# Aatrick/LightDiffusion

Hardware: AMD Instinct MI355X
Metric: UNet denoise steps/sec at 512x512 (higher is better)
Workload: dtype f16 (fp32 accumulate); 1 GPU; SD1.5 512x512 UNet CFG step, euler_ancestral / normal-30, batch 8/GPU (UNet batch 16), latent 64x64; global_batch=8, parallelism=dp1 (replicas, RCCL cond broadcast), hip_graph=True, setup_before_warmup=hipGraph capture + one untimed schedule pass per workload

## Files before the change

include/ld_mi355x.h:

```cpp
#ifndef LD_MI355X_H
#define LD_MI355X_H

#include <stddef.h>
#include <stdint.h>

#ifdef __cplusplus
extern "C" {
#endif

#define LD_OK 0
#define LD_ERR_ARG 1
#define LD_ERR_SHAPE 2
#define LD_ERR_HIP 3
#define LD_ERR_STATE 4

#define LD_F16 0
#define LD_F32 1

const char* ld_version(void);
const char* ld_status_string(int status);

typedef struct {
    int in_channels, out_channels, model_channels;
    int num_levels;
    int channel_mult[8];
    int num_res_blocks[8];
    int transformer_depth[16];
    int transformer_depth_output[24];
    int transformer_depth_middle;
    int context_dim, num_heads;
} ld_unet_config;

typedef struct ld_unet ld_unet;

int ld_unet_create(const ld_unet_config* cfg, ld_unet** out);
void ld_unet_destroy(ld_unet* u);
int ld_unet_param_count(const ld_unet* u);
int ld_unet_param_info(const ld_unet* u, int index, const char** name, int* ndim, int64_t shape[4]);
int ld_unet_load_param(ld_unet* u, const char* name, const void* dev_src, int dtype, void* stream);
int ld_unet_reserve(ld_unet* u, int max_n, int max_h, int max_w, int max_ctx_tokens);
size_t ld_unet_workspace_bytes(const ld_unet* u);
size_t ld_unet_weight_bytes(const ld_unet* u);
int ld_unet_set_context(ld_unet* u, const void* ctx, int dtype, int n, int tokens, void* stream);
int ld_unet_forward(ld_unet* u, const float* x, const float* sigma, float* out, int n, int h, int w, int eps_only, void* stream);
int ld_unet_forward_pair(ld_unet* u, const float* x, const float* sigma, float* out, int nb, int h, int w, void* stream);
int ld_unet_profile(ld_unet* u, const float* x, const float* sigma, float* out, int n, int h, int w, void* stream, double ms[6],
                    double flops[6], int launches[6]);
int ld_unet_profile_pair(ld_unet* u, const float* x, const float* sigma, float* out, int nb, int h, int w, void* stream, double ms[6],
                         double flops[6], int launches[6]);
int ld_unet_profile_kernels(const ld_unet* u, char* buf, size_t buf_bytes);
int ld_unet_profile_launches(const ld_unet* u, char* buf, size_t buf_bytes);
int ld_unet_last_launches(const ld_unet* u);
double ld_unet_last_flops(const ld_unet* u);

typedef struct {
    int z_channels, ch, num_levels;
    int ch_mult[8];
    int num_res_blocks, out_ch;
    int with_encoder;
} ld_vae_config;

typedef struct ld_vae ld_vae;

int ld_vae_create(const ld_vae_config* cfg, ld_vae** out);
void ld_vae_destroy(ld_vae* v);
int ld_vae_param_count(const ld_vae* v);
int ld_vae_param_info(const ld_vae* v, int index, const char** name, int* ndim, int64_t shape[4]);
int ld_vae_load_param(ld_vae* v, const char* name, const void* dev_src, int dtype, void* stream);
int ld_vae_reserve(ld_vae* v, int max_b, int max_h, int max_w);
size_t ld_vae_workspace_bytes(const ld_vae* v);
size_t ld_vae_plan_bytes(ld_vae* v, int b, int h, int w);
int ld_vae_decode(ld_vae* v, const float* z, float* out, int b, int h, int w, void* stream);
int ld_vae_encode(ld_vae* v, const float* pixels_nchw, float* moments, int b, int h, int w, void* stream);
int ld_vae_profile(ld_vae* v, const float* z, float* out, int b, int h, int w, void* stream);
int ld_vae_profile_launches(const ld_vae* v, char* buf, size_t buf_bytes);
int ld_vae_last_launches(const ld_vae* v);
double ld_vae_last_flops(const ld_vae* v);

int ld_op_linear(const void* x, const void* w, const void* bias, const void* residual, void* y, int M, int N, int K,
                 float alpha, int act, void* ws, size_t ws_bytes, void* stream);
int ld_op_conv(const void* x1, int c1, const void* x2, int c2, int n, int h, int w, int hv, int wv, int stride, int ksize,
               const void* wt, const void* bias, const void* rowvec, const void* residual, void* y, int cout,
               void* ws, size_t ws_bytes, void* stream);
size_t ld_op_groupnorm_conv_ws_bytes(int c1, int c2, int n, int h, int w, int cout);
int ld_op_groupnorm_conv(const void* x1, int c1, const void* x2, int c2, int n, int h, int w, const void* gamma, const void* beta, float eps,
                         const void* wt, const void* bias, const void* rowvec, const void* residual, void* y, int cout, void* ws,
                         size_t ws_bytes, void* stream);
int ld_op_repack_conv(const void* src_oihw, int dtype, int cout, int cin, void* dst, void* stream);
size_t ld_op_conv_skip_ws_bytes(int c, int sc1, int sc2, int cout);
int ld_op_conv_skip(const void* x, int c, int n, int h, int w, const void* wt, const void* bias, const void* s1, int sc1, const void* s2, int sc2,
                    const void* wskip, const void* bskip, const void* rowvec, void* y, int cout, void* ws, size_t ws_bytes, void* stream);
int ld_op_upconv2x_fold(const void* wt, int cout, int cin, void* wfold, void* stream);
int ld_op_upconv2x(const void* x, int c, int n, int h, int w, int hv, int wv, const void* wt, const void* wfold, const void* bias, void* y, int cout,
                   void* ws, size_t ws_bytes, void* stream);
size_t ld_op_conv_gn_partials_floats(int n, int hw);
int ld_op_conv_gn_partials(const void* x, int c, int n, int h, int w, int hv, int wv, const void* wt, const void* bias,
                           const void* residual, void* y, int cout, float* part, int* chunks, void* ws, size_t ws_bytes, void* stream);
size_t ld_op_groupnorm_ws_bytes(int n, int hw);
int ld_op_groupnorm(const void* x1, int c1, const void* x2, int c2, int n, int hw, const void* gamma, const void* beta,
                    float eps, int silu, void* y, void* ws, void* stream);
int ld_op_layernorm(const void* x, const void* gamma, const void* beta, void* y, int rows, int c, float eps, void* stream);
int ld_op_attention(const void* q, int ldq, const void* k, int ldk, const void* vt, int ldvt, void* o, int ldo, int b,
                    int heads, int lq, int lk, int d, float scale, int causal, void* stream);
int ld_op_attention_rowv(const void* q, int ldq, const void* k, int ldk, const void* v, int ldv, void* o, int ldo, int b,
                         int heads, int lq, int lk, int d, float scale, int causal, void* stream);
int ld_op_softmax_rows(void* s, int rows, int cols, void* stream);
int ld_op_timestep_embed(const float* sigma, const float* log_sigmas, int n_sigmas, int n, int dim, void* out_f16, float* t_out,
                         void* stream);
int ld_op_cfg_combine(const float* den2, float* out, float cfg, size_t n_half, void* stream);
int ld_op_axpby(float* x, float a, const float* y, float b, const float* z, float c, size_t n, void* stream);
int ld_op_hook_check(const void* a, const void* b, size_t words_ab, const void* x, size_t half_words_x, const void* sigma, int half_sigma,
                     int* flags, int epoch, void* stream);

int ld_op_linear_ln(const void* x, const void* w_prod, const void* b_prod, const void* gamma, const void* beta, const void* w,
                    const void* bias, void* t_out, void* y, int M, int C, int N, float eps, void* ws, size_t ws_bytes, void* stream);
int ld_op_linear_ln_geglu(const void* x, const void* w_prod, const void* b_prod, const void* gamma, const void* beta, const void* w,
                          const void* bias, void* t_out, void* y, int M, int C, int N, float eps, void* ws, size_t ws_bytes, void* stream);
int ld_op_bislerp(const float* x, float* tmp, float* y, int n, int c, int h, int w, int h_new, int w_new, void* stream);
const char* ld_op_last_kernel(void);

#ifdef __cplusplus
}
#endif
#endif
```

lightdiffusion_amd/_lib.py:

```python
from __future__ import annotations

import ctypes as C
import os

_HERE = os.path.dirname(os.path.abspath(__file__))
LIB_PATH = os.environ.get("LD_MI355X_LIB") or os.path.join(_HERE, "libld_mi355x.so")

OK, ERR_ARG, ERR_SHAPE, ERR_HIP, ERR_STATE = 0, 1, 2, 3, 4
F16, F32 = 0, 1


class UNetConfig(C.Structure):
    _fields_ = [("in_channels", C.c_int), ("out_channels", C.c_int), ("model_channels", C.c_int), ("num_levels", C.c_int),
                ("channel_mult", C.c_int * 8), ("num_res_blocks", C.c_int * 8), ("transformer_depth", C.c_int * 16),
                ("transformer_depth_output", C.c_int * 24), ("transformer_depth_middle", C.c_int),
                ("context_dim", C.c_int), ("num_heads", C.c_int)]


class VAEConfig(C.Structure):
    _fields_ = [("z_channels", C.c_int), ("ch", C.c_int), ("num_levels", C.c_int), ("ch_mult", C.c_int * 8),
                ("num_res_blocks", C.c_int), ("out_ch", C.c_int), ("with_encoder", C.c_int)]


class LDError(RuntimeError):
    def __init__(self, status: int, where: str):
        self.status = status
        msg = lib().ld_status_string(status).decode() if _lib is not None else str(status)
        super().__init__(f"{where}: {msg} (status {status})")


_lib = None
_P, _I, _F, _Z = C.c_void_p, C.c_int, C.c_float, C.c_size_t

SIGNATURES = {
    "ld_version": (C.c_char_p, []),
    "ld_status_string": (C.c_char_p, [_I]),
    "ld_unet_create": (_I, [C.POINTER(UNetConfig), C.POINTER(_P)]),
    "ld_unet_destroy": (None, [_P]),
    "ld_unet_param_count": (_I, [_P]),
    "ld_unet_param_info": (_I, [_P, _I, C.POINTER(C.c_char_p), C.POINTER(_I), C.POINTER(C.c_int64)]),
    "ld_unet_load_param": (_I, [_P, C.c_char_p, _P, _I, _P]),
    "ld_unet_reserve": (_I, [_P, _I, _I, _I, _I]),
    "ld_unet_workspace_bytes": (_Z, [_P]),
    "ld_unet_weight_bytes": (_Z, [_P]),
    "ld_unet_set_context": (_I, [_P, _P, _I, _I, _I, _P]),
    "ld_unet_forward": (_I, [_P, _P, _P, _P, _I, _I, _I, _I, _P]),
    "ld_unet_forward_pair": (_I, [_P, _P, _P, _P, _I, _I, _I, _P]),
    "ld_unet_profile_pair": (_I, [_P, _P, _P, _P, _I, _I, _I, _P, C.POINTER(C.c_double), C.POINTER(C.c_double), C.POINTER(_I)]),
    "ld_unet_profile": (_I, [_P, _P, _P, _P, _I, _I, _I, _P, C.POINTER(C.c_double), C.POINTER(C.c_double), C.POINTER(_I)]),
    "ld_unet_profile_kernels": (_I, [_P, C.c_char_p, _Z]),
    "ld_unet_profile_launches": (_I, [_P, C.c_char_p, _Z]),
    "ld_unet_last_launches": (_I, [_P]),
    "ld_unet_last_flops": (C.c_double, [_P]),
    "ld_vae_create": (_I, [C.POINTER(VAEConfig), C.POINTER(_P)]),
    "ld_vae_destroy": (None, [_P]),
    "ld_vae_param_count": (_I, [_P]),
    "ld_vae_param_info": (_I, [_P, _I, C.POINTER(C.c_char_p), C.POINTER(_I), C.POINTER(C.c_int64)]),
    "ld_vae_load_param": (_I, [_P, C.c_char_p, _P, _I, _P]),
    "ld_vae_reserve": (_I, [_P, _I, _I, _I]),
    "ld_vae_workspace_bytes": (_Z, [_P]),
    "ld_vae_plan_bytes": (_Z, [_P, _I, _I, _I]),
    "ld_vae_decode": (_I, [_P, _P, _P, _I, _I, _I, _P]),
    "ld_vae_encode": (_I, [_P, _P, _P, _I, _I, _I, _P]),
    "ld_vae_profile": (_I, [_P, _P, _P, _I, _I, _I, _P]),
    "ld_vae_profile_launches": (_I, [_P, C.c_char_p, _Z]),
    "ld_vae_last_launches": (_I, [_P]),
    "ld_vae_last_flops": (C.c_double, [_P]),
    "ld_op_linear": (_I, [_P, _P, _P, _P, _P, _I, _I, _I, _F, _I, _P, _Z, _P]),
    "ld_op_conv": (_I, [_P, _I, _P, _I, _I, _I, _I, _I, _I, _I, _I, _P, _P, _P, _P, _P, _I, _P, _Z, _P]),
    "ld_op_groupnorm_conv_ws_bytes": (_Z, [_I, _I, _I, _I, _I, _I]),
    "ld_op_groupnorm_conv": (_I, [_P, _I, _P, _I, _I, _I, _I, _P, _P, _F, _P, _P, _P, _P, _P, _I, _P, _Z, _P]),
    "ld_op_repack_conv": (_I, [_P, _I, _I, _I, _P, _P]),
    "ld_op_upconv2x_fold": (_I, [_P, _I, _I, _P, _P]),
    "ld_op_upconv2x": (_I, [_P, _I, _I, _I, _I, _I, _I, _P, _P, _P, _P, _I, _P, _Z, _P]),
    "ld_op_conv_skip_ws_bytes": (_Z, [_I, _I, _I, _I]),
    "ld_op_conv_skip": (_I, [_P, _I, _I, _I, _I, _P, _P, _P, _I, _P, _I, _P, _P, _P, _P, _I, _P, _Z, _P]),
    "ld_op_groupnorm_ws_bytes": (_Z, [_I, _I]),
    "ld_op_groupnorm": (_I, [_P, _I, _P, _I, _I, _I, _P, _P, _F, _I, _P, _P, _P]),
    "ld_op_layernorm": (_I, [_P, _P, _P, _P, _I, _I, _F, _P]),
    "ld_op_attention": (_I, [_P, _I, _P, _I, _P, _I, _P, _I, _I, _I, _I, _I, _I, _F, _I, _P]),
    "ld_op_conv_gn_partials_floats": (_Z, [_I, _I]),
    "ld_op_conv_gn_partials": (_I, [_P, _I, _I, _I, _I, _I, _I, _P, _P, _P, _P, _I, _P, _P, _P, _Z, _P]),
    "ld_op_attention_rowv": (_I, [_P, _I, _P, _I, _P, _I, _P, _I, _I, _I, _I, _I, _I, _F, _I, _P]),
    "ld_op_softmax_rows": (_I, [_P, _I, _I, _P]),
    "ld_op_timestep_embed": (_I, [_P, _P, _I, _I, _I, _P, _P, _P]),
    "ld_op_cfg_combine": (_I, [_P, _P, _F, _Z, _P]),
    "ld_op_axpby": (_I, [_P, _F, _P, _F, _P, _F, _Z, _P]),
    "ld_op_hook_check": (_I, [_P, _P, _Z, _P, _Z, _P, _I, _P, _I, _P]),
    "ld_op_linear_ln": (_I, [_P, _P, _P, _P, _P, _P, _P, _P, _P, _I, _I, _I, _F, _P, _Z, _P]),
    "ld_op_linear_ln_geglu": (_I, [_P, _P, _P, _P, _P, _P, _P, _P, _P, _I, _I, _I, _F, _P, _Z, _P]),
    "ld_op_bislerp": (_I, [_P, _P, _P, _I, _I, _I, _I, _I, _I, _P]),
    "ld_op_last_kernel": (C.c_char_p, []),
}


def lib() -> C.CDLL:
    global _lib
    if _lib is None:
        if not os.path.exists(LIB_PATH):
            raise ImportError(f"{LIB_PATH} not found — build it with `python -c 'import __graft_entry__ as g; g.build()'` "
                              f"or `make -C lightdiffusion_amd/csrc`.  There is no CPU / PyTorch fallback for the hot path.")
        try:
            import torch
        except ImportError:
            pass
        l = C.CDLL(LIB_PATH)
        missing = []
        for name, (res, args) in SIGNATURES.items():
            if not hasattr(l, name):
                if not os.environ.get("LD_MI355X_LIB"):
                    raise AttributeError(f"{LIB_PATH} does not export {name}: header and library out of sync — rebuild it")
                missing.append(name)
                setattr(l, name, _missing_symbol(name))
                continue
            fn = getattr(l, name)
            fn.restype = res
            fn.argtypes = args
        l._ld_missing = tuple(missing)
        _lib = l
    return _lib


def _missing_symbol(name: str):
    def fail(*_a, **_k):
        raise RuntimeError(f"{LIB_PATH} (LD_MI355X_LIB) does not export {name}: it was built from a commit without this entry point")
    return fail


def check(status: int, where: str) -> None:
    if status != OK:
        raise LDError(status, where)
```

lightdiffusion_amd/csrc/capi.hip:

```cpp
#include <string>

#include "kernels.h"
#include "../../include/ld_mi355x.h"

namespace {
inline size_t align256(size_t v) { return (v + 255) / 256 * 256; }

thread_local std::string t_op_kernels;
inline void op_begin() { t_op_kernels.clear(); }
inline int noted(int st, const char* name) {
    if (name != nullptr && *name != '\0') {
        if (!t_op_kernels.empty()) t_op_kernels += ';';
        t_op_kernels += name;
    }
    return st;
}
inline int gemm_op(const GemmParams& p, hipStream_t s) { return noted(gemm_launch(p, s), gemm_last_kernel_name()); }
inline int gemm_op(const GemmParams& p, const GemmPlan& plan, hipStream_t s) { return noted(gemm_run(p, plan, s), gemm_last_kernel_name()); }

constexpr size_t kSyncBytes = LD_SYNC_INTS * sizeof(int);
inline size_t conv8_scratch_head(int cout, int cin) { return kSyncBytes + (conv8_weight_eligible(cout, cin) ? align256(conv8_weight_bytes(cout, cin)) : 0); }
inline void conv8_scratch(GemmParams& p, void* ws, size_t partial_bytes) {
    const int cin = p.C1 + p.C2;
    p.sync = (int*)ws;
    p.W8 = conv8_weight_eligible(p.N, cin) ? (const half_t*)((char*)ws + kSyncBytes) : nullptr;
    p.partial = (float*)((char*)ws + conv8_scratch_head(p.N, cin));
    p.partial_bytes = partial_bytes;
}
inline int conv8_scratch_op(const GemmParams& p, const GemmPlan& plan, const void* wt, hipStream_t stream) {
    if (plan.route == GR_CONV8) {
        if (hipMemsetAsync(p.sync, 0, kSyncBytes, stream) != hipSuccess) return LD_ERR_HIP;
        const int st = conv8_repack_launch((const half_t*)wt, p.N, p.C1 + p.C2, const_cast<half_t*>(p.W8), stream);
        if (st != LD_OK) return st;
    }
    return gemm_op(p, plan, stream);
}
inline int attn_op(const AttnParams& a, hipStream_t s) { return noted(attention_launch(a, s), attention_last_kernel_name()); }
}

extern "C" {

const char* ld_version(void) { return "ld_mi355x 0.1 (gfx950)"; }

const char* ld_op_last_kernel(void) { return t_op_kernels.c_str(); }

const char* ld_status_string(int s) {
    switch (s) {
        case LD_OK: return "ok";
        case LD_ERR_ARG: return "invalid argument";
        case LD_ERR_SHAPE: return "unsupported shape or alignment";
        case LD_ERR_HIP: return "HIP runtime error";
        case LD_ERR_STATE: return "invalid call order (weights / reserve / context missing)";
        default: return "unknown status";
    }
}

int ld_op_linear(const void* x, const void* w, const void* bias, const void* residual, void* y, int M, int N, int K, float alpha,
                 int act, void* ws, size_t ws_bytes, void* stream_) {
    op_begin();
    hipStream_t stream = (hipStream_t)stream_;
    GemmParams p;
    p.A = (const half_t*)x; p.lda = K;
    p.W = (const half_t*)w; p.ldw = K;
    p.M = M; p.N = N; p.K = K;
    p.alpha = alpha;
    p.bias_n = (const half_t*)bias;
    p.R = (const half_t*)residual;
    p.act = act;
    p.C = (half_t*)y;
    p.ldc = p.ldr = (act == 2 ? N / 2 : N);
    char* wsp = (char*)ws;
    if (act == 2) {
        if (bias == nullptr || (N & 15)) return LD_ERR_ARG;
        const int bn = gemm_pick_bn(N);
        if (N % bn) return LD_ERR_SHAPE;
        const size_t wb = align256((size_t)N * K * sizeof(half_t)), bb = align256((size_t)N * sizeof(half_t));
        if (ws == nullptr || ws_bytes < wb + bb) return LD_ERR_ARG;
        half_t* w2 = (half_t*)wsp;
        half_t* b2 = (half_t*)(wsp + wb);
        int st = repack_rows_launch(w, 0, N, K, w2, bn, stream);
        if (st != LD_OK) return st;
        st = repack_rows_launch(bias, 0, N, 1, b2, bn, stream);
        if (st != LD_OK) return st;
        p.W = w2;
        p.bias_n = b2;
        p.bn = bn;
        wsp += wb + bb;
        ws_bytes -= wb + bb;
    }
    p.partial = (float*)wsp;
    p.partial_bytes = ws ? ws_bytes : 0;
    if (ws == nullptr) p.partial = nullptr;
    return gemm_op(p, stream);
}

static int op_conv(const void* x1, int c1, const void* x2, int c2, int n, int h, int w, int hv, int wv, int stride, int ksize,
                   const void* wt, const void* bias, const void* rowvec, const void* residual, void* y, int cout, void* ws,
                   size_t ws_bytes, void* stream, float* gn_part, int* gn_chunks, const void* wup = nullptr) {
    if (stride < 1 || (ksize != 1 && ksize != 3)) return LD_ERR_ARG;
    GemmParams p;
    if (gn_part != nullptr) {
        const int HW = (ksize == 3 ? (hv - 1) / stride + 1 : hv) * (ksize == 3 ? (wv - 1) / stride + 1 : wv);
        p.gn_part = gn_part;
        p.gn_P = gn_num_chunks(n, HW);
        p.gn_HW = HW;
        p.gn_ppb = (HW + p.gn_P - 1) / p.gn_P;
        p.gn_part_done = gn_chunks;
    }
    p.conv = 1;
    p.ksize = ksize;
    p.A = (const half_t*)x1; p.A2 = (const half_t*)x2; p.C1 = c1; p.C2 = c2;
    p.Hs = h; p.Ws = w; p.Hv = hv; p.Wv = wv; p.stride = stride;
    p.Ho = ksize == 3 ? (hv - 1) / stride + 1 : hv;
    p.Wo = ksize == 3 ? (wv - 1) / stride + 1 : wv;
    p.K = ksize * ksize * (c1 + c2);
    p.W = (const half_t*)wt; p.ldw = p.K;
    p.Wup = (const half_t*)wup;
    p.M = n * p.Ho * p.Wo; p.N = cout;
    p.bias_n = (const half_t*)bias;
    p.rowvec = (const half_t*)rowvec; p.rows_per_vec = p.Ho * p.Wo; p.ldrv = cout;
    p.R = (const half_t*)residual; p.ldr = cout;
    p.C = (half_t*)y; p.ldc = cout;
    p.partial = (float*)ws;
    p.partial_bytes = ws ? ws_bytes : 0;
    const size_t head = conv8_scratch_head(cout, c1 + c2);
    if (ws != nullptr && ksize == 3 && conv8_weight_eligible(cout, c1 + c2) && ws_bytes > head + ((size_t)8 << 20)) {
        GemmParams c8 = p;
        conv8_scratch(c8, ws, ws_bytes - head);
        if (const GemmPlan plan = gemm_plan(c8); plan.route == GR_CONV8) return conv8_scratch_op(c8, plan, wt, (hipStream_t)stream);
    }
    return gemm_op(p, (hipStream_t)stream);
}

int ld_op_conv(const void* x1, int c1, const void* x2, int c2, int n, int h, int w, int hv, int wv, int stride, int ksize,
               const void* wt, const void* bias, const void* rowvec, const void* residual, void* y, int cout, void* ws,
               size_t ws_bytes, void* stream) {
    op_begin();
    return op_conv(x1, c1, x2, c2, n, h, w, hv, wv, stride, ksize, wt, bias, rowvec, residual, y, cout, ws, ws_bytes, stream, nullptr, nullptr);
}

int ld_op_upconv2x_fold(const void* wt, int cout, int cin, void* wfold, void* stream) {
    op_begin();
    return upconv_fold_launch((const half_t*)wt, cout, cin, (half_t*)wfold, (hipStream_t)stream);
}

int ld_op_upconv2x(const void* x, int c, int n, int h, int w, int hv, int wv, const void* wt, const void* wfold, const void* bias, void* y, int cout,
                   void* ws, size_t ws_bytes, void* stream) {
    op_begin();
    if (wfold == nullptr) return LD_ERR_ARG;
    return op_conv(x, c, nullptr, 0, n, h, w, hv, wv, 1, 3, wt, bias, nullptr, nullptr, y, cout, ws, ws_bytes, stream, nullptr, nullptr, wfold);
}

size_t ld_op_conv_gn_partials_floats(int n, int hw) {
    op_begin();
    return groupnorm_workspace_bytes(n, hw) / sizeof(float);
}

int ld_op_conv_gn_partials(const void* x, int c, int n, int h, int w, int hv, int wv, const void* wt, const void* bias, const void* residual,
                           void* y, int cout, float* part, int* chunks, void* ws, size_t ws_bytes, void* stream) {
    op_begin();
    if (part == nullptr || chunks == nullptr) return LD_ERR_ARG;
    *chunks = 0;
    return op_conv(x, c, nullptr, 0, n, h, w, hv, wv, 1, 3, wt, bias, nullptr, residual, y, cout, ws, ws_bytes, stream, part, chunks);
}

size_t ld_op_groupnorm_conv_ws_bytes(int c1, int c2, int n, int h, int w, int cout) {
    op_begin();
    const size_t C = (size_t)c1 + c2, HW = (size_t)h * w;
    return align256(groupnorm_workspace_bytes(n, (int)HW)) + 2 * align256((size_t)n * C * sizeof(float)) + align256((size_t)n * HW * C * sizeof(half_t)) +
           conv8_scratch_head(cout, c1 + c2) + ((size_t)96 << 20);
}

int ld_op_groupnorm_conv(const void* x1, int c1, const void* x2, int c2, int n, int h, int w, const void* gamma, const void* beta, float eps,
                         const void* wt, const void* bias, const void* rowvec, const void* residual, void* y, int cout, void* ws, size_t ws_bytes,
                         void* stream_) {
    op_begin();
    if (x1 == nullptr || gamma == nullptr || beta == nullptr || wt == nullptr || y == nullptr || ws == nullptr) return LD_ERR_ARG;
    if (ws_bytes < ld_op_groupnorm_conv_ws_bytes(c1, c2, n, h, w, cout)) return LD_ERR_ARG;
    hipStream_t stream = (hipStream_t)stream_;
    const int C = c1 + c2, HW = h * w;
    char* q = (char*)ws;
    float* part = (float*)q; q += align256(groupnorm_workspace_bytes(n, HW));
    float* scale = (float*)q; q += align256((size_t)n * C * sizeof(float));
    float* shift = (float*)q; q += align256((size_t)n * C * sizeof(float));
    half_t* g = (half_t*)q; q += align256((size_t)n * HW * C * sizeof(half_t));
    GemmParams p;
    p.conv = 1; p.ksize = 3;
    p.A = (const half_t*)x1; p.A2 = (const half_t*)x2; p.C1 = c1; p.C2 = c2;
    p.Hs = p.Hv = p.Ho = h; p.Ws = p.Wv = p.Wo = w; p.stride = 1;
    p.K = 9 * C; p.W = (const half_t*)wt; p.ldw = p.K;
    p.M = n * HW; p.N = cout;
    p.bias_n = (const half_t*)bias;
    p.rowvec = (const half_t*)rowvec; p.rows_per_vec = HW; p.ldrv = cout;
    p.R = (const half_t*)residual; p.ldr = cout;
    p.C = (half_t*)y; p.ldc = cout;
    conv8_scratch(p, q, (size_t)96 << 20);
    const GemmPlan fused = gemm_plan(p, true);
    if (fused.can_fuse_groupnorm) {
        int st = groupnorm_scale_shift_launch((const half_t*)x1, c1, (const half_t*)x2, c2, n, HW, (const half_t*)gamma, (const half_t*)beta, eps, part,
                                              scale, shift, stream);
        if (st != LD_OK) return st;
        p.gn_scale = scale; p.gn_shift = shift; p.gn_silu = 1;
        return gemm_op(p, fused, stream);
    }
    int st = groupnorm_launch((const half_t*)x1, c1, (const half_t*)x2, c2, n, HW, (const half_t*)gamma, (const half_t*)beta, eps, 1, g, part, stream);
    if (st != LD_OK) return st;
    p.A = g; p.A2 = nullptr; p.C1 = C; p.C2 = 0;
    return conv8_scratch_op(p, gemm_plan(p), (const half_t*)wt, stream);
}

size_t ld_op_conv_skip_ws_bytes(int c, int sc1, int sc2, int cout) {
    op_begin();
    return align256((size_t)cout * (9 * (size_t)c + sc1 + sc2) * sizeof(half_t)) + align256((size_t)cout * sizeof(half_t)) + ((size_t)96 << 20);
}

int ld_op_conv_skip(const void* x, int c, int n, int h, int w, const void* wt, const void* bias, const void* s1, int sc1, const void* s2, int sc2,
                    const void* wskip, const void* bskip, const void* rowvec, void* y, int cout, void* ws, size_t ws_bytes, void* stream_) {
    op_begin();
    if (x == nullptr || wt == nullptr || bias == nullptr || s1 == nullptr || wskip == nullptr || bskip == nullptr || y == nullptr || ws == nullptr) return LD_ERR_ARG;
    if (c <= 0 || sc1 <= 0 || sc2 < 0 || (sc2 > 0 && s2 == nullptr) || cout <= 0 || n <= 0 || h <= 0 || w <= 0) return LD_ERR_ARG;
    if (ws_bytes < ld_op_conv_skip_ws_bytes(c, sc1, sc2, cout)) return LD_ERR_ARG;
    hipStream_t stream = (hipStream_t)stream_;
    const int K9 = 9 * c, SC = sc1 + sc2;
    char* q = (char*)ws;
    half_t* wf = (half_t*)q; q += align256((size_t)cout * (K9 + SC) * sizeof(half_t));
    half_t* bf = (half_t*)q; q += align256((size_t)cout * sizeof(half_t));
    int st = skip_fold_launch((const half_t*)wt, (const half_t*)wskip, (const half_t*)bias, (const half_t*)bskip, cout, K9, SC, wf, bf, stream);
    if (st != LD_OK) return st;
    GemmParams p;
    p.conv = 1; p.ksize = 3;
    p.A = (const half_t*)x; p.C1 = c;
    p.Hs = p.Hv = p.Ho = h; p.Ws = p.Wv = p.Wo = w; p.stride = 1;
    p.S1 = (const half_t*)s1; p.SC1 = sc1; p.S2 = (const half_t*)s2; p.SC2 = sc2;
    p.K = K9 + SC; p.W = wf; p.ldw = p.K;
    p.M = n * h * w; p.N = cout;
    p.bias_n = bf;
    p.rowvec = (const half_t*)rowvec; p.rows_per_vec = h * w; p.ldrv = cout;
    p.C = (half_t*)y; p.ldc = cout;
    p.partial = (float*)q; p.partial_bytes = (size_t)96 << 20;
    return gemm_op(p, stream);
}

int ld_op_repack_conv(const void* src, int dtype, int cout, int cin, void* dst, void* stream) {
    op_begin();
    return repack_conv3x3_launch(src, dtype == LD_F32, cout, cin, (half_t*)dst, (hipStream_t)stream);
}

size_t ld_op_groupnorm_ws_bytes(int n, int hw) {
    op_begin();
    return groupnorm_workspace_bytes(n, hw);
}

int ld_op_groupnorm(const void* x1, int c1, const void* x2, int c2, int n, int hw, const void* gamma, const void* beta, float eps,
                    int silu, void* y, void* ws, void* stream) {
    op_begin();
    return groupnorm_launch((const half_t*)x1, c1, (const half_t*)x2, c2, n, hw, (const half_t*)gamma, (const half_t*)beta, eps,
                            silu, (half_t*)y, (float*)ws, (hipStream_t)stream);
}

int ld_op_layernorm(const void* x, const void* gamma, const void* beta, void* y, int rows, int c, float eps, void* stream) {
    op_begin();
    return layernorm_launch((const half_t*)x, (const half_t*)gamma, (const half_t*)beta, (half_t*)y, rows, c, eps, (hipStream_t)stream);
}

int ld_op_attention(const void* q, int ldq, const void* k, int ldk, const void* vt, int ldvt, void* o, int ldo, int b, int heads,
                    int lq, int lk, int d, float scale, int causal, void* stream) {
    op_begin();
    AttnParams a;
    a.Q = (const half_t*)q; a.ldq = ldq; a.sQ = (long long)lq * ldq;
    a.K = (const half_t*)k; a.ldk = ldk; a.sK = (long long)lk * ldk;
    a.Vt = (const half_t*)vt; a.ldvt = ldvt; a.sV = (long long)heads * d * ldvt;
    a.O = (half_t*)o; a.ldo = ldo; a.sO = (long long)lq * ldo;
    a.B = b; a.H = heads; a.Lq = lq; a.Lk = lk; a.d = d; a.scale = scale; a.causal = causal;
    return attn_op(a, (hipStream_t)stream);
}

int ld_op_attention_rowv(const void* q, int ldq, const void* k, int ldk, const void* v, int ldv, void* o, int ldo, int b, int heads,
                         int lq, int lk, int d, float scale, int causal, void* stream) {
    op_begin();
    const char *qb = (const char*)q, *kb = (const char*)k, *vb = (const char*)v;
    const long long rowb = (long long)ldq * 2;
    const bool fused = ldq == ldk && ldk == ldv && rowb > 0 && (kb - qb >= 0 ? kb - qb : qb - kb) < rowb && (vb - qb >= 0 ? vb - qb : qb - vb) < rowb;
    if (fused && lq != lk) return LD_ERR_SHAPE;
    AttnParams a;
    a.Q = (const half_t*)q; a.ldq = ldq; a.sQ = (long long)lq * ldq;
    a.K = (const half_t*)k; a.ldk = ldk; a.sK = (long long)lk * ldk;
    a.V = (const half_t*)v; a.ldv = ldv; a.sV = (long long)lk * ldv;
    a.O = (half_t*)o; a.ldo = ldo; a.sO = (long long)lq * ldo;
    a.B = b; a.H = heads; a.Lq = lq; a.Lk = lk; a.d = d; a.scale = scale; a.causal = causal;
    return attn_op(a, (hipStream_t)stream);
}

int ld_op_softmax_rows(void* s, int rows, int cols, void* stream) {
    op_begin();
    return softmax_rows_launch((half_t*)s, rows, cols, cols, (hipStream_t)stream);
}

int ld_op_timestep_embed(const float* sigma, const float* log_sigmas, int n_sigmas, int n, int dim, void* out, float* t_out, void* stream) {
    op_begin();
    return timestep_embed_launch(sigma, log_sigmas, n_sigmas, n, dim, (half_t*)out, t_out, (hipStream_t)stream);
}

int ld_op_cfg_combine(const float* den2, float* out, float cfg, size_t n_half, void* stream) {
    op_begin();
    return cfg_combine_launch(den2, out, cfg, n_half, (hipStream_t)stream);
}

int ld_op_hook_check(const void* a, const void* b, size_t words_ab, const void* x, size_t half_words_x, const void* sigma, int half_sigma,
                     int* flags, int epoch, void* stream) {
    op_begin();
    return hook_check_launch(a, b, words_ab, x, half_words_x, sigma, half_sigma, flags, epoch, (hipStream_t)stream);
}

int ld_op_axpby(float* x, float a, const float* y, float b, const float* z, float c, size_t n, void* stream) {
    op_begin();
    return axpby_launch(x, a, y, b, z, c, n, (hipStream_t)stream);
}

// ... 92 lines not shown
```

lightdiffusion_amd/csrc/gemm.h:

```cpp
#pragma once
#include "common.h"

struct GemmParams {
    const half_t* A = nullptr;
    const half_t* A2 = nullptr;
    int lda = 0;
    int conv = 0;
    int ksize = 3;
    int pad = -1;
    int Hs = 0, Ws = 0;
    int Hv = 0, Wv = 0;
    int Ho = 0, Wo = 0, stride = 1;
    int C1 = 0, C2 = 0;
    const half_t* S1 = nullptr;
    const half_t* S2 = nullptr;
    int SC1 = 0, SC2 = 0;
    const half_t* W = nullptr;
    int ldw = 0;
    int M = 0, N = 0, K = 0;
    int n_valid = 0;
    int batch = 1;
    long long sA = 0, sW = 0, sC = 0, sR = 0;
    float alpha = 1.0f;
    const half_t* bias_n = nullptr;
    const half_t* bias_m = nullptr;
    const half_t* rowvec = nullptr;
    int rows_per_vec = 1, ldrv = 0;
    const half_t* R = nullptr;
    int ldr = 0;
    int act = 0;
    half_t* C = nullptr;
    int ldc = 0;
    int bm = 0, bn = 0;
    int splitk = 0;
    int m_fastest = -1;
    int xcd_gm = 0;
    float* partial = nullptr;
    size_t partial_bytes = 0;
    float* stat_out = nullptr;
    int* stat_parts_out = nullptr;
    const float* ln_stat = nullptr;
    int ln_parts = 0;
    int ln_rows = 0;
    int ln_zrows = 0;
    float ln_inv_c = 0.f, ln_eps = 0.f;
    const float* ln_wsum = nullptr;
    int ln_swapped = 0;
    const float* gn_scale = nullptr;
    const float* gn_shift = nullptr;
    int gn_silu = 0;
    float* gn_part = nullptr;
    int gn_P = 0, gn_ppb = 0, gn_HW = 0;
    int* gn_part_done = nullptr;
    const half_t* W8 = nullptr;
    int* sync = nullptr;
    int c8_S = 0;
    const half_t* Wup = nullptr;
    int dbg = 0;
};

enum GemmRoute { GR_NONE = 0, GR_CONV8, GR_CONV6, GR_GEMM7, GR_GEMM5, GR_GEMM3, GR_GEMM4, GR_UPCONV };
enum GemmReduce { GRD_NONE = 0, GRD_PLAIN, GRD_GROUPNORM, GRD_UPCONV };
struct GemmPlan {
    int status = LD_OK;
    int route = GR_NONE;
    bool conv = false, geglu = false;
    bool gn = false, up = false;
    bool ln = false;
    bool deep = false, two_wg = false;
    int bm = 0, bn = 0, wc = 0;
    int splitk = 1, c8_S = 0;
    int m_fastest = 0, xcd_gm = 0;
    unsigned grid_x = 0, grid_z = 1;
    int reduce = GRD_NONE;
    int stat_parts = 0;
    int gn_chunks = 0;
    bool halo_tile = false;
    bool can_fuse_groupnorm = false;
    bool takes_skip_segment = false;
    const char* kernel = "";
};
GemmPlan gemm_plan(const GemmParams& p, bool gn_offer = false);
int gemm_run(const GemmParams& p, const GemmPlan& plan, hipStream_t stream);
inline int gemm_launch(const GemmParams& p, hipStream_t stream) { return gemm_run(p, gemm_plan(p), stream); }
const char* gemm_last_kernel_name();

bool conv8_plan(const GemmParams& p, int* S_out);
int conv8_launch(const GemmParams& p, int S, hipStream_t stream);
bool conv8_weight_eligible(int N, int Cin);
size_t conv8_weight_bytes(int N, int Cin);
int conv8_repack_launch(const half_t* w_okki, int N, int Cin, half_t* dst, hipStream_t stream);
int upconv_reduce_launch(const GemmParams& p, hipStream_t stream);
#define LD_SYNC_INTS 1024

static inline int gemm_pick_bn(int N) { return (N % 160 == 0) ? 160 : 128; }
```

lightdiffusion_amd/csrc/gemm.hip:

```cpp
#include <cstdlib>
#include <mutex>
#include <set>
#include <string>
#include <type_traits>
#include <vector>

#include "gemm.h"

namespace {

constexpr int BK = 64;
constexpr int NT = 256;

__device__ __forceinline__ void epilogue_store8(const GemmParams& p, int z, int m, int n_out, int n_bias, float (&v)[8]) {
    const bool hb = p.bias_n != nullptr && p.act != 2, hv = p.rowvec != nullptr, hr = p.R != nullptr;
    const uint4 rb = hb ? ld16(p.bias_n + n_bias) : zero16();
    const uint4 rv = hv ? ld16(p.rowvec + (long long)(m / p.rows_per_vec) * p.ldrv + n_out) : zero16();
    const uint4 rr = hr ? ld16(p.R + (long long)z * p.sR + (long long)m * p.ldr + n_out) : zero16();
    const float bm = p.bias_m != nullptr ? (float)p.bias_m[m] : 0.f;
    float b[8], e[8], r[8];
    unpack8(rb, b);
    unpack8(rv, e);
    unpack8(rr, r);
#pragma unroll
    for (int j = 0; j < 8; ++j) v[j] = v[j] + b[j] + bm + e[j];
    if (p.act == 1) {
#pragma unroll
        for (int j = 0; j < 8; ++j) v[j] = silu_f(v[j]);
    } else if (p.act == 3) {
#pragma unroll
        for (int j = 0; j < 8; ++j) v[j] = quick_gelu_f(v[j]);
    }
#pragma unroll
    for (int j = 0; j < 8; ++j) v[j] += r[j];
    st16(p.C + (long long)z * p.sC + (long long)m * p.ldc + n_out, pack8(v));
}

template <int BM, int BN>
struct EpiPre {
    static constexpr int CPR = BN / 8, EIT = (BM * CPR + NT - 1) / NT, GRP = EIT > 5 ? (EIT + 1) / 2 : EIT;
    uint4 r[GRP];
    bool fast;
    bool bias_done;
};
template <int BM, int BN>
__device__ __forceinline__ EpiPre<BM, BN> epi_prefetch_residual(const GemmParams& p, int z, int m0, int n0, int tid, bool bias_done) {
    EpiPre<BM, BN> e;
    e.bias_done = bias_done;
    constexpr int CPR = EpiPre<BM, BN>::CPR, GRP = EpiPre<BM, BN>::GRP;
    e.fast = (BM * CPR) % NT == 0 && m0 + BM <= p.M && n0 + BN <= p.N && p.act == 0 && p.bias_m == nullptr && bias_done;
#pragma unroll
    for (int k = 0; k < GRP; ++k) e.r[k] = zero16();
    if (e.fast && p.R != nullptr) {
        const half_t* Rb = p.R + (long long)z * p.sR + (long long)m0 * p.ldr + n0;
#pragma unroll
        for (int k = 0; k < GRP; ++k) {
            const int q = tid + k * NT;
            const int row = q / CPR, cc = q - row * CPR;
            e.r[k] = ld16(Rb + (long long)row * p.ldr + cc * 8);
        }
    }
    return e;
}

template <int BM, int BN>
__device__ __forceinline__ void epilogue_tile(const GemmParams& p, const half_t* Cs, int z, int m0, int n0, int tid, float* lds_scratch, const half_t* bias_s,
                                              const EpiPre<BM, BN>& pre) {
    constexpr int CLD = BN + 8;
    if (p.act == 2) {
        constexpr int CPR = BN / 16;
        constexpr int EIT = (BM * CPR + NT - 1) / NT;
        if ((BM * CPR) % NT == 0 && m0 + BM <= p.M && n0 + BN <= p.N && pre.bias_done) {
            half_t* Cb = p.C + (long long)z * p.sC + (long long)m0 * p.ldc + n0 / 2;
            const bool hr = p.R != nullptr;
            const half_t* Rb = hr ? p.R + (long long)z * p.sR + (long long)m0 * p.ldr + n0 / 2 : nullptr;
            uint4 rres[EIT], ca[EIT], cg[EIT];
#pragma unroll
            for (int it = 0; it < EIT; ++it) {
                const int q = tid + it * NT;
                const int row = q / CPR, cc = q - row * CPR;
                rres[it] = hr ? ld16(Rb + (long long)row * p.ldr + cc * 8) : zero16();
                ca[it] = ld16(Cs + row * CLD + cc * 8);
                cg[it] = ld16(Cs + row * CLD + BN / 2 + cc * 8);
            }
#pragma unroll
            for (int it = 0; it < EIT; ++it) {
                const int q = tid + it * NT;
                const int row = q / CPR, cc = q - row * CPR;
                float g[8];
                unpack8(cg[it], g);
                const unsigned aw[4] = {ca[it].x, ca[it].y, ca[it].z, ca[it].w};
                const f32x2 gp[4] = {{g[0], g[1]}, {g[2], g[3]}, {g[4], g[5]}, {g[6], g[7]}};
                unsigned ow[4];
                geglu8_staged(aw, gp, ow);
                uint4 packed = make_uint4(ow[0], ow[1], ow[2], ow[3]);
                if (hr) packed = add8h(packed, rres[it]);
                st16(Cb + (long long)row * p.ldc + cc * 8, packed);
            }
            return;
        }
        uint4 rba[EIT], rbg[EIT], rres[EIT];
#pragma unroll
        for (int it = 0; it < EIT; ++it) {
            const int q = tid + it * NT;
            const int row = q / CPR, cc = q - row * CPR;
            const int m = m0 + row, nv = n0 + cc * 8, ng = nv + BN / 2;
            const bool ok = q < BM * CPR && m < p.M && ng < p.N;
            rba[it] = (ok && !pre.bias_done) ? ld16(p.bias_n + nv) : zero16();
            rbg[it] = (ok && !pre.bias_done) ? ld16(p.bias_n + ng) : zero16();
            rres[it] = (ok && p.R != nullptr) ? ld16(p.R + (long long)z * p.sR + (long long)m * p.ldr + n0 / 2 + cc * 8) : zero16();
        }
#pragma unroll
        for (int it = 0; it < EIT; ++it) {
            const int q = tid + it * NT;
            const int row = q / CPR, cc = q - row * CPR;
            const int m = m0 + row, ng = n0 + cc * 8 + BN / 2;
            if (q < BM * CPR && m < p.M && ng < p.N) {
                float a[8], g[8], ba[8], bg[8], r[8];
                unpack8(ld16(Cs + row * CLD + cc * 8), a);
                unpack8(ld16(Cs + row * CLD + BN / 2 + cc * 8), g);
                unpack8(rba[it], ba);
                unpack8(rbg[it], bg);
                unpack8(rres[it], r);
#pragma unroll
                for (int j = 0; j < 8; ++j) a[j] = (a[j] + ba[j]) * gelu_f(g[j] + bg[j]) + r[j];
                st16(p.C + (long long)z * p.sC + (long long)m * p.ldc + n0 / 2 + cc * 8, pack8(a));
            }
        }
    } else {
        constexpr int CPR = BN / 8;
        constexpr int EIT = (BM * CPR + NT - 1) / NT;
        constexpr int GRP = EIT > 5 ? (EIT + 1) / 2 : EIT;
        const bool hb = p.bias_n != nullptr && !pre.bias_done, hv = p.rowvec != nullptr, hr = p.R != nullptr;
        if (pre.fast) {
            static_assert(GRP == EpiPre<BM, BN>::GRP, "group size");
            half_t* Cb = p.C + (long long)z * p.sC + (long long)m0 * p.ldc + n0;
            const half_t* Rb = hr ? p.R + (long long)z * p.sR + (long long)m0 * p.ldr + n0 : nullptr;
            uint4 rnext[GRP];
#pragma unroll
            for (int k = 0; k < GRP; ++k) rnext[k] = pre.r[k];
#pragma unroll
            for (int g0 = 0; g0 < EIT; g0 += GRP) {
                uint4 rv[GRP], rres[GRP], cv[GRP];
#pragma unroll
                for (int k = 0; k < GRP; ++k) rres[k] = rnext[k];
#pragma unroll
                for (int k = 0; k < GRP; ++k) {
                    if (g0 + GRP + k >= EIT) continue;
                    const int q = tid + (g0 + GRP + k) * NT;
                    const int row = q / CPR, cc = q - row * CPR;
                    rnext[k] = hr ? ld16(Rb + (long long)row * p.ldr + cc * 8) : zero16();
                }
#pragma unroll
                for (int k = 0; k < GRP; ++k) {
                    if (g0 + k >= EIT) continue;
                    const int q = tid + (g0 + k) * NT;
                    const int row = q / CPR, cc = q - row * CPR;
                    rv[k] = hv ? ld16(p.rowvec + (long long)((m0 + row) / p.rows_per_vec) * p.ldrv + n0 + cc * 8) : zero16();
                    cv[k] = ld16(Cs + row * CLD + cc * 8);
                }
#pragma unroll
                for (int k = 0; k < GRP; ++k) {
                    if (g0 + k >= EIT) continue;
                    const int q = tid + (g0 + k) * NT;
                    const int row = q / CPR, cc = q - row * CPR;
                    uint4 packed = cv[k];
                    if (hv) packed = add8h(packed, rv[k]);
                    if (hr) packed = add8h(packed, rres[k]);
                    st16(Cb + (long long)row * p.ldc + cc * 8, packed);
                    if (lds_scratch != nullptr) {
                        const half2v one2 = {(half_t)1.f, (half_t)1.f};
                        const half2v h0 = __builtin_bit_cast(half2v, packed.x), h1 = __builtin_bit_cast(half2v, packed.y);
                        const half2v h2 = __builtin_bit_cast(half2v, packed.z), h3 = __builtin_bit_cast(half2v, packed.w);
                        float s1 = __builtin_amdgcn_fdot2(h1, one2, __builtin_amdgcn_fdot2(h0, one2, 0.f, false), false);
                        float s2 = __builtin_amdgcn_fdot2(h1, h1, __builtin_amdgcn_fdot2(h0, h0, 0.f, false), false);
                        s1 = __builtin_amdgcn_fdot2(h3, one2, __builtin_amdgcn_fdot2(h2, one2, s1, false), false);
                        s2 = __builtin_amdgcn_fdot2(h3, h3, __builtin_amdgcn_fdot2(h2, h2, s2, false), false);
                        *reinterpret_cast<float2*>(lds_scratch + q * 2) = make_float2(s1, s2);
                    }
                }
            }
            if (lds_scratch != nullptr) {
                __syncthreads();
                if (tid < BM) {
                    float s1 = 0.f, s2 = 0.f;
#pragma unroll 4
                    for (int c = 0; c < CPR; ++c) {
                        const float2 t = *reinterpret_cast<const float2*>(lds_scratch + (tid * CPR + c) * 2);
                        s1 += t.x;
// ... 1896 lines not shown
                for (int j = 0; j < 8; ++j) {
                    a[j] += base[nv + j];
                    g[j] += base[ng + j];
                }
            }
            float ba[8], bg[8];
            unpack8(ld16(p.bias_n + nv), ba);
            unpack8(ld16(p.bias_n + ng), bg);
#pragma unroll
            for (int j = 0; j < 8; ++j) v[j] = (a[j] + ba[j]) * gelu_f(g[j] + bg[j]);
            epilogue_store8(p, 0, m, no, 0, v);
        } else {
            const int n = cc * 8;
#pragma unroll
            for (int j = 0; j < 8; ++j) v[j] = 0.f;
            const float* base = p.partial + (long long)m * p.N + n;
            const long long slab = (long long)p.M * p.N;
            int s = 0;
            for (; s + 4 <= p.splitk; s += 4) {
                f32x4 x0[4], x1[4];
#pragma unroll
                for (int u = 0; u < 4; ++u) {
                    x0[u] = *reinterpret_cast<const f32x4*>(base + (s + u) * slab);
                    x1[u] = *reinterpret_cast<const f32x4*>(base + (s + u) * slab + 4);
                }
#pragma unroll
                for (int u = 0; u < 4; ++u)
#pragma unroll
                    for (int j = 0; j < 4; ++j) {
                        v[j] += x0[u][j];
                        v[4 + j] += x1[u][j];
                    }
            }
            for (; s < p.splitk; ++s) {
                const f32x4 x0 = *reinterpret_cast<const f32x4*>(base + s * slab), x1 = *reinterpret_cast<const f32x4*>(base + s * slab + 4);
#pragma unroll
                for (int j = 0; j < 4; ++j) {
                    v[j] += x0[j];
                    v[4 + j] += x1[j];
                }
            }
            epilogue_store8(p, 0, m, n, n, v);
        }
    }
}

__global__ __launch_bounds__(256) void splitk_reduce_gn_kernel(const GemmParams p) {
    __shared__ float csum[2048], csq[2048];
    const int C = p.N, cpg = C / 32;
    const int CS = C / 4, CHS = CS >> 3;
    const int n = blockIdx.y, pc = blockIdx.x, slab = blockIdx.z, tid = threadIdx.x;
    const int rows_par = 256 / CHS;
    const int cc = tid % CHS, prow = tid / CHS;
    const int c0 = slab * CS + cc * 8;
    const int p_begin = pc * p.gn_ppb, p_end = min(p.gn_HW, p_begin + p.gn_ppb);
    const long long slab_stride = (long long)p.M * p.N;
    if (prow < rows_par) {
        float s[8], ss[8];
#pragma unroll
        for (int j = 0; j < 8; ++j) s[j] = ss[j] = 0.f;
        for (int pix = p_begin + prow; pix < p_end; pix += rows_par) {
            const int m = n * p.gn_HW + pix;
            const float* base = p.partial + (long long)m * p.N + c0;
            float v[8];
#pragma unroll
            for (int j = 0; j < 8; ++j) v[j] = 0.f;
            int sp = 0;
            for (; sp + 4 <= p.splitk; sp += 4) {
                f32x4 x0[4], x1[4];
#pragma unroll
                for (int u = 0; u < 4; ++u) {
                    x0[u] = *reinterpret_cast<const f32x4*>(base + (sp + u) * slab_stride);
                    x1[u] = *reinterpret_cast<const f32x4*>(base + (sp + u) * slab_stride + 4);
                }
#pragma unroll
                for (int u = 0; u < 4; ++u)
#pragma unroll
                    for (int j = 0; j < 4; ++j) {
                        v[j] += x0[u][j];
                        v[4 + j] += x1[u][j];
                    }
            }
            for (; sp < p.splitk; ++sp) {
                const f32x4 x0 = *reinterpret_cast<const f32x4*>(base + sp * slab_stride), x1 = *reinterpret_cast<const f32x4*>(base + sp * slab_stride + 4);
#pragma unroll
                for (int j = 0; j < 4; ++j) {
                    v[j] += x0[j];
                    v[4 + j] += x1[j];
                }
            }
            epilogue_store8(p, 0, m, c0, c0, v);
            float f[8];
            unpack8(pack8(v), f);
#pragma unroll
            for (int j = 0; j < 8; ++j) {
                s[j] += f[j];
                ss[j] += f[j] * f[j];
            }
        }
#pragma unroll
        for (int j = 0; j < 8; ++j) {
            csum[prow * CS + cc * 8 + j] = s[j];
            csq[prow * CS + cc * 8 + j] = ss[j];
        }
    }
    __syncthreads();
    {
        const int g = tid >> 5, sub = tid & 31;
        const int cnt = rows_par * cpg;
        float a = 0.f, b = 0.f;
        for (int i = sub; i < cnt; i += 32) {
            const int pr = i / cpg, c = g * cpg + (i - pr * cpg);
            a += csum[pr * CS + c];
            b += csq[pr * CS + c];
        }
#pragma unroll
        for (int o = 1; o < 32; o <<= 1) {
            a += __shfl_xor(a, o, 64);
            b += __shfl_xor(b, o, 64);
        }
        if (sub == 0) {
            float* o = p.gn_part + (((long long)n * p.gn_P + pc) * 32 + slab * 8 + g) * 2;
            o[0] = a;
            o[1] = b;
        }
    }
}

constexpr int V4_MAX_BLOCKS = 256;

thread_local const char* t_last_kernel = "";

const char* plan_kernel_name(const GemmPlan& pl) {
    typedef unsigned long long u64;
    const u64 key = (u64)pl.route | (u64)pl.reduce << 3 | (u64)pl.conv << 5 | (u64)pl.geglu << 6 | (u64)pl.gn << 7 | (u64)pl.up << 8 | (u64)pl.ln << 9 |
                    (u64)pl.deep << 10 | (u64)pl.two_wg << 11 | (u64)pl.bm << 12 | (u64)pl.bn << 24 | (u64)pl.wc << 36;
    thread_local std::vector<std::pair<u64, const char*>> seen;
    for (const auto& e : seen)
        if (e.first == key) return e.second;
    const std::string tile = std::to_string(pl.bm) + "," + std::to_string(pl.bn);
    std::string s;
    switch (pl.route) {
        case GR_UPCONV: s = "upconv_kernel<256,320>"; break;
        case GR_CONV8: s = "conv8_kernel<W" + std::to_string(pl.wc) + (pl.up ? ",up>" : ">"); break;
        case GR_CONV6:
            s = "conv6_kernel<W" + std::to_string(pl.wc) + ",halo" + (pl.gn ? "+groupnorm" : "") +
                (pl.bn == V5_BN ? "" : "," + std::to_string(pl.bn) + (pl.bm == V5_BM ? "" : "x" + std::to_string(pl.bm))) + (pl.up ? ",up" : "") + ">";
            break;
        case GR_GEMM7: s = std::string("gemm7_kernel<256,K320,") + (pl.geglu ? "geglu" : "plain") + (pl.ln ? ",ln>" : ">"); break;
        case GR_GEMM5: s = std::string("gemm5_kernel<256,320,") + (pl.conv ? "conv" : pl.geglu ? "geglu" : pl.ln ? "lnfold" : "plain") + ">"; break;
        case GR_GEMM4: s = "gemm4_kernel<" + tile + (pl.conv ? ",conv" : ",plain") + (pl.two_wg ? ",2wg>" : ">"); break;
        default: s = "gemm3_kernel<" + tile + (pl.conv ? ",conv" : ",plain") + (pl.deep ? ",deep>" : ">"); break;
    }
    if (pl.reduce != GRD_NONE) s += pl.reduce == GRD_GROUPNORM ? "+splitk_reduce_gn_kernel" : pl.reduce == GRD_UPCONV ? "+upconv_reduce_kernel" : "+splitk_reduce_kernel";
    static std::mutex mu; static std::set<std::string> pool;
    std::lock_guard<std::mutex> lock(mu);
    const char* name = pool.insert(s).first->c_str();
    seen.push_back({key, name});
    return name;
}

template <int BM, int BN>
void launch_cfg(const GemmParams& p, const GemmPlan& pl, dim3 grid, hipStream_t s) {
    if (pl.route == GR_GEMM4) {
        if constexpr (BM == 64 && BN == 64) {
            if (pl.two_wg) {
                if (!pl.conv) hipLaunchKernelGGL((gemm4_kernel<64, 64, false, 4, 4>), grid, dim3(2 * NT), 0, s, p);
                else hipLaunchKernelGGL((gemm4_kernel<64, 64, true, 4, 4>), grid, dim3(2 * NT), 0, s, p);
                return;
            }
        }
        hipLaunchKernelGGL((gemm4_kernel<BM, BN, false>), grid, dim3(2 * NT), 0, s, p);
    } else if (pl.conv) {
        if constexpr (BM == 64 && BN == 160) {
            if (pl.deep) {
                hipLaunchKernelGGL((gemm3_kernel<BM, BN, true, 4>), grid, dim3(NT), 0, s, p);
                return;
            }
        }
        hipLaunchKernelGGL((gemm3_kernel<BM, BN, true, 2>), grid, dim3(NT), 0, s, p);
    } else {
        hipLaunchKernelGGL((gemm3_kernel<BM, BN, false, 2>), grid, dim3(NT), 0, s, p);
    }
}

template <int W, bool GN, int BN, int BM, bool UP>
void launch_conv6_w(const GemmParams& p, dim3 grid, hipStream_t s) { hipLaunchKernelGGL((conv6_kernel<W, GN, BN, BM, UP>), grid, dim3(512), 0, s, p); }
template <bool GN, int BN = V5_BN, int BM = V5_BM, bool UP = false>
void launch_conv6(int wc, const GemmParams& p, dim3 grid, hipStream_t s) {
    if constexpr (BN == V5_BN) {
        if (wc == 16) return launch_conv6_w<16, GN, BN, BM, UP>(p, grid, s);
        if (wc == 32) return launch_conv6_w<32, GN, BN, BM, UP>(p, grid, s);
    }
    if constexpr (BN == V5_BN || (BN == 256 && !GN)) {
        if (wc == 64) return launch_conv6_w<64, GN, BN, BM, UP>(p, grid, s);
    }
    launch_conv6_w<128, GN, BN, BM, UP>(p, grid, s);
}

}

#ifdef LD_AB_BUILD
static int g_force_bm = 0, g_force_sk = 0;
static int g_shape_ovr[5] = {0, 0, 0, 0, 0};
extern "C" void ld_debug_gemm_shape_override(int M, int N, int K, int bm, int splitk) {
    g_shape_ovr[0] = M; g_shape_ovr[1] = N; g_shape_ovr[2] = K; g_shape_ovr[3] = bm; g_shape_ovr[4] = splitk;
}
extern "C" void ld_debug_gemm_override(int bm, int splitk) {
    g_force_bm = bm;
    g_force_sk = splitk;
}
#endif

const char* gemm_last_kernel_name() { return t_last_kernel; }

static void plan_reduce(const GemmParams& p, GemmPlan* pl) {
    if (pl->splitk <= 1) return;
    const bool gn = p.gn_part != nullptr && p.act != 2 && p.batch == 1 && p.gn_P > 0 && p.gn_HW > 0 && p.M % p.gn_HW == 0 && p.N % 32 == 0 && p.N <= 8192 && p.N >= 256 &&
                    p.ldc == p.N && (p.N / 4) % 8 == 0 && p.N / 32 <= 256;
    pl->reduce = gn ? GRD_GROUPNORM : GRD_PLAIN;
    if (gn) pl->gn_chunks = p.gn_P;
}

static bool upconv_plan(const GemmParams& p, GemmPlan* out) {
    if (!(p.conv && p.ksize == 3 && p.stride == 1 && p.pad == 1 && p.Hv == 2 * p.Hs && p.Wv == 2 * p.Ws && p.Ho == p.Hv && p.Wo == p.Wv && p.C2 == 0 &&
          p.SC1 == 0 && p.C1 % V5_BK == 0 && p.N % V5_BN == 0 && p.n_valid == p.N && p.bm == 0 && p.bn == 0 && p.splitk == 0 && p.batch == 1 && p.act == 0 &&
          p.alpha == 1.0f && p.rowvec == nullptr && p.R == nullptr && p.bias_m == nullptr && p.stat_out == nullptr && p.ln_stat == nullptr && p.ldc == p.N))
        return false;
    if ((long long)p.M * 4 > 0x7fffffffll) return false;
    if (p.M / (p.Ho * p.Wo) <= 2) return false;
    const int Ms = p.M / 4, K = 4 * p.C1;
    const long long tiles = (long long)((Ms + V5_BM - 1) / V5_BM) * (4 * p.N / V5_BN);
    int sk = 1;
    if (tiles < 192 && p.partial != nullptr) {
        sk = (int)((256 + tiles - 1) / tiles);
        const int cap = K / 640 < 1 ? 1 : K / 640;
        if (sk > cap) sk = cap;
        while (sk > 1 && (size_t)sk * Ms * 4 * p.N * sizeof(float) > p.partial_bytes) --sk;
    }
    out->bm = V5_BM; out->bn = V5_BN; out->splitk = sk; out->up = true;
    out->grid_x = (unsigned)(tiles * sk); out->grid_z = 1;
    out->reduce = sk > 1 ? GRD_UPCONV : GRD_NONE;
    return true;
}

static bool v6_plan(const GemmParams& p, bool gn, GemmPlan* out) {
    const bool same = p.Hv == p.Hs && p.Wv == p.Ws;
    const bool up = p.Hv == 2 * p.Hs && p.Wv == 2 * p.Ws;
    if (!(p.conv && p.ksize == 3 && p.stride == 1 && (p.pad < 0 || p.pad == 1) && (same || up) && p.Ho == p.Hv && p.Wo == p.Wv &&
          p.C1 % 32 == 0 && p.C2 % 32 == 0 && p.bm == 0 && p.bn == 0 && p.splitk == 0 && p.batch == 1 && p.act != 2))
        return false;
    if (up && (p.C2 != 0 || gn)) return false;
    if (p.SC1 > 0) return false;
    const int wc = (p.Wo == 16 || p.Wo == 32 || p.Wo == 64 || p.Wo == 128) ? p.Wo : (p.Wo > 128 && p.Wo % 128 == 0) ? 128 : 0;
    if (wc == 0) return false;
    int bn = 0, bm = V5_BM;
    if (p.N % V5_BN == 0) {
        bn = V5_BN;
    } else if (p.N % 256 == 0 && wc >= 64 && (!gn || (p.N == 256 && wc == 128 && !up))) {
        bn = 256;
    } else if (p.N % 128 == 0 && wc == 128 && !up && (!gn || p.N == 128)) {
        bn = 128;
        bm = 512;
    } else if (p.N == 32 && wc == 128 && !gn && !up) {
        bn = 32;
        bm = 512;
    } else {
        return false;
    }
    if (p.Ho % (bm / wc) != 0 || p.M % bm != 0) return false;
    const long long tm = p.M / bm;
    const long long t6 = tm * (p.N / bn);
    const int NS = (p.C1 + p.C2) / 32;
    int sk6 = 1;
    if (t6 < 192 && p.partial != nullptr && p.K >= 8640) {
        sk6 = (int)((256 + t6 - 1) / t6);
        const int cap = p.K / 2560;
        if (sk6 > cap) sk6 = cap;
        if (sk6 > NS) sk6 = NS;
        while (sk6 > 1 && (size_t)sk6 * p.M * p.N * sizeof(float) > p.partial_bytes) --sk6;
    }
#ifdef LD_AB_BUILD
    if (p.partial != nullptr && bn == V5_BN) {
        static const char* names[4] = {"LD_V6_SK_W16", "LD_V6_SK_W32", "LD_V6_SK_W64", "LD_V6_SK_W128"};
        const char* e = getenv(names[wc == 16 ? 0 : wc == 32 ? 1 : wc == 64 ? 2 : 3]);
        if (e != nullptr) {
            int want = atoi(e);
            if (want < 1) want = 1;
            if (want > NS) want = NS;
            while (want > 1 && (size_t)want * p.M * p.N * sizeof(float) > p.partial_bytes) --want;
            sk6 = want;
        }
    }
#endif
    out->splitk = sk6; out->bn = bn; out->bm = bm; out->wc = wc; out->up = up;
    out->grid_x = (unsigned)(t6 * sk6);
    return t6 * sk6 >= 192;
}

GemmPlan gemm_plan(const GemmParams& pin, bool gn_offer) {
    GemmPlan pl;
    GemmParams p = pin;
    const bool gn = gn_offer || p.gn_scale != nullptr;
    const auto fail = [](int st) { GemmPlan f; f.status = st; return f; };
    const auto done = [&pl](int route) { pl.route = route; pl.kernel = plan_kernel_name(pl); return pl; };
#ifdef LD_AB_BUILD
    if (g_force_bm) p.bm = g_force_bm;
    if (g_force_sk) p.splitk = g_force_sk;
    if (g_shape_ovr[0] == p.M && g_shape_ovr[1] == p.N && g_shape_ovr[2] == p.K && p.batch == 1 && !gn) {
        p.bm = g_shape_ovr[3];
        p.splitk = g_shape_ovr[4];
    }
#endif
    if (p.M <= 0 || p.N <= 0 || p.K <= 0 || p.A == nullptr || p.W == nullptr || p.C == nullptr) return fail(LD_ERR_ARG);
    if ((p.N & 7) || (p.K & 7) || (p.ldw & 7) || (p.ldc & 7)) return fail(LD_ERR_SHAPE);
    if (p.conv) {
        const int Cin = p.C1 + p.C2;
        if (p.ksize != 1 && p.ksize != 3) return fail(LD_ERR_ARG);
        if (p.pad < 0) p.pad = p.ksize >> 1;
        if (p.SC1 < 0 || p.SC2 < 0 || (p.SC1 == 0 && p.SC2 != 0)) return fail(LD_ERR_ARG);
        if (Cin <= 0 || (p.C1 % 64) || (p.C2 % 64) || (p.SC1 % 64) || (p.SC2 % 64) || p.K != p.ksize * p.ksize * Cin + p.SC1 + p.SC2) return fail(LD_ERR_SHAPE);
        if (p.SC1 > 0) {
            if (p.S1 == nullptr || (p.SC2 > 0 && p.S2 == nullptr)) return fail(LD_ERR_ARG);
            if (p.stride != 1 || p.Hv != p.Hs || p.Wv != p.Ws || p.Ho != p.Hv || p.Wo != p.Wv || p.pad != p.ksize / 2 || p.SC1 > 32768 || p.SC2 > 32768) return fail(LD_ERR_SHAPE);
        }
        if (p.C1 > 32768 || p.C2 > 32768) return fail(LD_ERR_SHAPE);
        if (p.C2 > 0 && p.A2 == nullptr) return fail(LD_ERR_ARG);
        if (p.M % (p.Ho * p.Wo)) return fail(LD_ERR_SHAPE);
        if (p.batch != 1) return fail(LD_ERR_ARG);
    } else if (p.lda & 7) {
        return fail(LD_ERR_SHAPE);
    }
    if (p.act == 2 && (p.bias_n == nullptr || (p.N & 15))) return fail(LD_ERR_ARG);
    if (p.R != nullptr && (p.ldr & 7)) return fail(LD_ERR_SHAPE);
    if (p.n_valid <= 0 || p.n_valid > p.N) p.n_valid = p.N;
    pl.conv = p.conv != 0; pl.geglu = p.act == 2;

    if (!gn && conv8_plan(p, &pl.c8_S)) {
        pl.wc = p.Wo; pl.up = p.Hv == 2 * p.Hs;
        if (p.gn_part != nullptr) pl.gn_chunks = p.Wo * p.Wo / 16;
        return done(GR_CONV8);
    }
    if (p.Wup != nullptr && !gn && upconv_plan(p, &pl)) return done(GR_UPCONV);
    if (GemmPlan v6 = pl; v6_plan(p, gn, &v6)) {
        pl = v6;
        const int bn6 = pl.bn, wc = pl.wc;
        if (gn) {
            if ((p.gn_scale != nullptr && p.gn_shift == nullptr) || pl.up) return fail(LD_ERR_ARG);
            if (bn6 != V5_BN && (wc != 128 || p.N != bn6 || !((bn6 == 256 && pl.bm == V5_BM) || (bn6 == 128 && pl.bm == 512)))) return fail(LD_ERR_ARG);
            pl.can_fuse_groupnorm = bn6 != V5_BN || p.N == V5_BN;
            if (gn_offer && !pl.can_fuse_groupnorm) return fail(LD_ERR_ARG);
            pl.gn = true;
        }
        if (pl.splitk == 1 && p.gn_part != nullptr) {
            const int cpg = p.N / 32, tiles_img = (p.Ho / (pl.bm / wc)) * (p.Wo / wc);
            const bool ok = (bn6 == 256 || bn6 == 128) && p.N % 32 == 0 && (p.N == 128 || cpg % 8 == 0) && bn6 % cpg == 0 && p.act == 0;
            if (ok) pl.gn_chunks = tiles_img;
        }
        plan_reduce(p, &pl);
        pl.halo_tile = true;
        return done(GR_CONV6);
    }
    if (gn) return fail(LD_ERR_ARG);
    pl.takes_skip_segment = p.conv && p.ksize == 3 && p.stride == 1 && p.Hv == p.Hs && p.Wv == p.Ws && p.SC1 == 0;
    if (!p.conv && p.K == V7_K && p.batch == 1 && !p.ln_swapped && p.bias_m == nullptr && p.rowvec == nullptr && p.bm == 0 && (p.bn == 0 || p.bn == 160) &&
        p.splitk == 0 && (p.n_valid <= 0 || p.n_valid >= p.N) && p.N % (p.act == 2 ? 160 : V7_NB) == 0 && (p.M + V7_BM - 1) / V7_BM >= 192 &&
        (p.act == 0 || (p.act == 2 && p.bias_n != nullptr && p.stat_out == nullptr && p.R == nullptr))) {
        pl.stat_parts = p.N / V7_NB;
        pl.grid_x = (unsigned)((p.M + V7_BM - 1) / V7_BM); pl.ln = p.ln_stat != nullptr;
        return done(GR_GEMM7);
    }
    {
        const bool conv3 = p.conv && p.ksize == 3;
        const bool shape_ok = !p.ln_swapped && p.bm == 0 && (p.bn == 0 || p.bn == 160) && p.N % V5_BN == 0 && p.K % V5_BK == 0 &&
                              p.K >= (p.act == 2 ? 1280 : conv3 ? 640 : 2560) && (p.n_valid == p.N || p.n_valid <= 0 || p.n_valid > p.N) &&
                              p.splitk == 0 && p.M >= 1024;
        const int tm5 = (p.M + V5_BM - 1) / V5_BM, tn5 = p.N / V5_BN;
        if (shape_ok && (long long)tm5 * tn5 * p.batch >= 192 && !(p.act == 2 && p.stat_out != nullptr)) {
            pl.ln = p.ln_stat != nullptr || p.stat_out != nullptr;
            if (p.conv && (pl.ln || p.act == 2)) return fail(LD_ERR_ARG);
            pl.stat_parts = 2 * tn5;
            pl.bm = V5_BM; pl.bn = V5_BN;
            pl.grid_x = (unsigned)(tm5 * tn5); pl.grid_z = (unsigned)p.batch;
            pl.xcd_gm = p.xcd_gm;
            if (!p.conv) {
                pl.xcd_gm = 0;
                if (p.batch == 1 && (tm5 * tn5) % 8 == 0 && p.M % V5_BM == 0) {
                    double best = 0;
                    for (int gm = 1; gm <= 8; gm <<= 1) {
                        const int gn5 = 8 / gm;
                        if (tm5 % gm || tn5 % gn5) continue;
                        const double cost = (double)p.M * gn5 + (double)p.N * gm;
                        if (pl.xcd_gm == 0 || cost < best) {
                            best = cost;
                            pl.xcd_gm = gm;
                        }
                    }
                }
            }
            return done(GR_GEMM5);
        }
    }
    int bn = p.bn ? p.bn : gemm_pick_bn(p.N);
    constexpr int skinny_max = 256;
    const bool skinny_ok = !p.conv && p.act != 2 && p.bn == 0 && p.bm == 0 && (p.N % 64) == 0;
    if (skinny_ok) {
        const long long t160 = (long long)((p.M + 63) / 64) * ((p.N + bn - 1) / bn) * p.batch;
        if (t160 <= skinny_max && (p.N + bn - 1) / bn <= 8) bn = 64;
    }
    bool skinny_conv1 = false;
    if (p.conv && p.ksize == 1 && p.act == 0 && p.bn == 0 && p.bm == 0 && p.splitk == 0 && p.batch == 1 && (p.N % 64) == 0 && p.SC1 == 0) {
        const long long t64 = (long long)((p.M + 63) / 64) * (p.N / 64);
        if (t64 > 128 && t64 <= 512 && p.K >= 1280 && p.K <= 3200) {
            bn = 64;
            skinny_conv1 = true;
        }
    }
    if (bn != 128 && bn != 160 && bn != 64) return fail(LD_ERR_ARG);
    if (p.act == 2 && (p.N % bn)) return fail(LD_ERR_SHAPE);
    const int tiles_n = (p.N + bn - 1) / bn;
    const int KT = (p.K + BK - 1) / BK;
    const int tiles128 = ((p.M + 127) / 128) * tiles_n * p.batch;
    const bool can_split = p.batch == 1 && p.partial != nullptr;
    const int sk_cap = p.K / 640 < 1 ? 1 : (p.K / 640 > 16 ? 16 : p.K / 640);
    int bm = p.bm, sk = p.splitk;
    if (bm == 0) {
        if (tiles128 >= 512) bm = 128;
        else if (p.K >= 4096 && can_split && (tiles128 >= 128 || (p.K >= 8192 && tiles128 >= 64))) bm = 128;
        else if (!p.conv && tiles128 >= 256) bm = 128;
        else bm = 64;
    }
    if (bn == 64) bm = 64;
    if (skinny_conv1) sk = 1;
    if (bm != 64 && bm != 128) return fail(LD_ERR_ARG);
    const int tiles = ((p.M + bm - 1) / bm) * tiles_n;
    const bool deep = p.conv && bm == 64 && bn == 160 && p.batch == 1 && p.splitk == 0 && (tiles <= 32 || (tiles >= 256 && tiles < 512));
    if (sk == 0) {
        sk = 1;
        if (can_split && tiles * p.batch < 512) {
            sk = ((deep ? 256 : 512) + tiles - 1) / tiles;
            if (sk > sk_cap) sk = sk_cap;
        }
    }
    if (sk > 1) {
        if (p.batch != 1 || p.partial == nullptr) return fail(LD_ERR_ARG);
        while (sk > 1 && (size_t)sk * p.M * p.N * sizeof(float) > p.partial_bytes) --sk;
        if (sk > KT) sk = KT;
    }
    if (p.stat_out != nullptr || p.ln_stat != nullptr) {
        if (p.act == 2 && p.stat_out != nullptr) return fail(LD_ERR_ARG);
        sk = 1;
        pl.stat_parts = tiles_n;
    }
    if (sk < 1) sk = 1;
    pl.bm = bm; pl.bn = bn; pl.splitk = sk;
    pl.grid_x = (unsigned)(tiles * sk); pl.grid_z = (unsigned)p.batch;
    pl.m_fastest = p.m_fastest;
    if (p.m_fastest < 0) {
        const int tiles_m = (p.M + bm - 1) / bm;
        pl.m_fastest = (!p.conv && p.batch == 1 && tiles_m >= 2 && tiles_m <= 8 && (long long)p.N * p.K * 2 >= (8ll << 20)) ? 1 : 0;
    }
    plan_reduce(p, &pl);
    const long long blocks = (long long)tiles * sk * p.batch;
    {
        const bool plain_2wg = bn == 64 && !p.conv && blocks > V4_MAX_BLOCKS && blocks <= 512 && p.K >= 640;
        const bool conv1_2wg = bn == 64 && p.conv && p.ksize == 1 && sk <= 1 && (long long)tiles * p.batch <= 512;
        pl.two_wg = plain_2wg || conv1_2wg;
        if (pl.two_wg) return done(GR_GEMM4);
    }
    if (!p.conv && blocks <= V4_MAX_BLOCKS) return done(GR_GEMM4);
    pl.deep = deep;
    return done(GR_GEMM3);
}

int gemm_run(const GemmParams& pin, const GemmPlan& pl, hipStream_t stream) {
    t_last_kernel = "";
    if (pl.status != LD_OK) return pl.status;
    if (pl.gn != (pin.gn_scale != nullptr) || (pl.gn && pin.gn_shift == nullptr)) return LD_ERR_ARG;
    GemmParams p = pin;
    if (p.stat_parts_out != nullptr) *p.stat_parts_out = pl.stat_parts;
    if (p.gn_part_done != nullptr) *p.gn_part_done = pl.gn_chunks;
    if (p.conv && p.pad < 0) p.pad = p.ksize >> 1;
    if (p.n_valid <= 0 || p.n_valid > p.N) p.n_valid = p.N;
    const dim3 grid(pl.grid_x, 1, pl.grid_z);
    t_last_kernel = pl.kernel;
    switch (pl.route) {
        case GR_CONV8:
            if (const int st = conv8_launch(p, pl.c8_S, stream); st != LD_OK) return st;
            break;
        case GR_CONV6:
            p.splitk = pl.splitk;
            if (pl.bn != 32) p.n_valid = p.N;
            if (pl.splitk == 1 && p.gn_part != nullptr) {
                if (pl.gn_chunks > 0) p.gn_P = pl.gn_chunks;
                else p.gn_part = nullptr;
            }
            if (pl.gn) {
                if (pl.bn == 256) launch_conv6<true, 256>(pl.wc, p, grid, stream);
                else if (pl.bn == 128) launch_conv6<true, 128, 512>(pl.wc, p, grid, stream);
                else launch_conv6<true>(pl.wc, p, grid, stream);
            } else if (pl.bn == 128) {
                launch_conv6<false, 128, 512>(pl.wc, p, grid, stream);
            } else if (pl.bn == 32) {
                launch_conv6<false, 32, 512>(pl.wc, p, grid, stream);
            } else if (pl.bn == 256) {
                if (pl.up) launch_conv6<false, 256, V5_BM, true>(pl.wc, p, grid, stream);
                else launch_conv6<false, 256>(pl.wc, p, grid, stream);
            } else {
                if (pl.up) launch_conv6<false, V5_BN, V5_BM, true>(pl.wc, p, grid, stream);
                else launch_conv6<false>(pl.wc, p, grid, stream);
            }
            break;
        case GR_UPCONV: {
            p.W = p.Wup; p.K = 4 * p.C1; p.ldw = p.K; p.M = pin.M / 4; p.N = 4 * pin.N; p.n_valid = p.N;
            p.splitk = pl.splitk; p.bn = 160; p.xcd_gm = 0;
            hipLaunchKernelGGL((gemm5_kernel<true, 0, true>), grid, dim3(512), 0, stream, p);
            if (pl.reduce == GRD_UPCONV) {
                if (const int st = upconv_reduce_launch(p, stream); st != LD_OK) return st;
            }
            return hipGetLastError() == hipSuccess ? LD_OK : LD_ERR_HIP;
        }
        case GR_GEMM7:
            if (pl.geglu && pl.ln) hipLaunchKernelGGL((gemm7_kernel<true, true>), grid, dim3(512), 0, stream, p);
            else if (pl.geglu) hipLaunchKernelGGL((gemm7_kernel<true, false>), grid, dim3(512), 0, stream, p);
            else if (pl.ln) hipLaunchKernelGGL((gemm7_kernel<false, true>), grid, dim3(512), 0, stream, p);
            else hipLaunchKernelGGL((gemm7_kernel<false, false>), grid, dim3(512), 0, stream, p);
            break;
        case GR_GEMM5:
            p.splitk = 1; p.bn = 160; p.xcd_gm = pl.xcd_gm;
            if (pl.conv) hipLaunchKernelGGL((gemm5_kernel<true, 0>), grid, dim3(512), 0, stream, p);
            else if (pl.geglu) hipLaunchKernelGGL((gemm5_kernel<false, 2>), grid, dim3(512), 0, stream, p);
            else if (pl.ln) hipLaunchKernelGGL((gemm5_kernel<false, 1>), grid, dim3(512), 0, stream, p);
            else hipLaunchKernelGGL((gemm5_kernel<false, 0>), grid, dim3(512), 0, stream, p);
            break;
        default:
            p.splitk = pl.splitk; p.bn = pl.bn; p.m_fastest = pl.m_fastest;
            if (pl.bn == 64) launch_cfg<64, 64>(p, pl, grid, stream);
            else if (pl.bm == 128 && pl.bn == 160) launch_cfg<128, 160>(p, pl, grid, stream);
            else if (pl.bm == 128 && pl.bn == 128) launch_cfg<128, 128>(p, pl, grid, stream);
            else if (pl.bm == 64 && pl.bn == 160) launch_cfg<64, 160>(p, pl, grid, stream);
            else launch_cfg<64, 128>(p, pl, grid, stream);
            break;
    }
    if (pl.reduce == GRD_GROUPNORM) {
        hipLaunchKernelGGL(splitk_reduce_gn_kernel, dim3(p.gn_P, p.M / p.gn_HW, 4), dim3(256), 0, stream, p);
    } else if (pl.reduce == GRD_PLAIN) {
        const int out_n = p.act == 2 ? p.N / 2 : p.N;
        const long long total = (long long)p.M * (out_n / 8);
        int blocks = (int)((total + 255) / 256);
        if (blocks > 2048) blocks = 2048;
        hipLaunchKernelGGL(splitk_reduce_kernel, dim3(blocks), dim3(256), 0, stream, p, pl.route == GR_CONV6 ? 160 : pl.bn);
    }
    return hipGetLastError() == hipSuccess ? LD_OK : LD_ERR_HIP;
}
```

lightdiffusion_amd/csrc/norm.hip:

```cpp
#include "kernels.h"

namespace {

constexpr int GN_THREADS = 256;
__host__ __device__ inline int gn_slabs(int C) { return C >= 256 ? 4 : C >= 128 ? 2 : 1; }

struct GnArgs {
    const half_t* x1;
    const half_t* x2;
    int C1, C2, HW, P, ppb;
    int Pstat;
    int slabs;
    float* partial;
    const half_t* gamma;
    const half_t* beta;
    half_t* y;
    float eps;
    int silu;
};

__device__ __forceinline__ const half_t* gn_src(const GnArgs& a, int n, int pix, int c) {
    return c < a.C1 ? a.x1 + ((long long)n * a.HW + pix) * a.C1 + c
                    : a.x2 + ((long long)n * a.HW + pix) * a.C2 + (c - a.C1);
}
// ... 34 lines not shown
            float v[8];
            unpack8(ld16(src), v);
#pragma unroll
            for (int j = 0; j < 8; ++j) {
                s[j] += v[j];
                ss[j] += v[j] * v[j];
            }
        }
#pragma unroll
        for (int j = 0; j < 8; ++j) {
            csum[prow * CS + cc * 8 + j] = s[j];
            csq[prow * CS + cc * 8 + j] = ss[j];
        }
    }
    __syncthreads();
    {
        const int g = tid / lpg, sub = tid - g * lpg;
        const int cnt = rows_par * cpg;
        float s = 0.f, ss = 0.f;
        for (int i = sub; i < cnt; i += lpg) {
            const int pr = i / cpg, c = g * cpg + (i - pr * cpg);
            s += csum[pr * CS + c];
            ss += csq[pr * CS + c];
        }
        for (int o = 1; o < lpg; o <<= 1) {
            s += __shfl_xor(s, o, 64);
            ss += __shfl_xor(ss, o, 64);
        }
        if (sub == 0) {
            float* o = a.partial + (((long long)n * a.P + pc) * 32 + slab * gps + g) * 2;
            o[0] = s;
            o[1] = ss;
        }
    }
}

__global__ __launch_bounds__(GN_THREADS) void gn_apply_kernel(const GnArgs a) {
    __shared__ float mean[32], rstd[32];
    const int C = a.C1 + a.C2, cpg = C / 32;
    const int CS = C / a.slabs, CHS = CS >> 3;
    const int gps = 32 / a.slabs, lpg = GN_THREADS / gps;
    const int n = blockIdx.y, pc = blockIdx.x, slab = blockIdx.z, tid = threadIdx.x;
    {
        const int g = tid / lpg, sub = tid - g * lpg;
        float s = 0.f, ss = 0.f;
        const float* pp = a.partial + ((long long)n * a.Pstat * 32 + slab * gps + g) * 2;
        for (int i = sub; i < a.Pstat; i += 4 * lpg) {
            float2 v[4];
#pragma unroll
            for (int u = 0; u < 4; ++u) {
                const int iu = i + u * lpg;
                v[u] = *reinterpret_cast<const float2*>(pp + (long long)(iu < a.Pstat ? iu : sub) * 64);
                if (iu >= a.Pstat) v[u] = make_float2(0.f, 0.f);
            }
#pragma unroll
            for (int u = 0; u < 4; ++u) {
                s += v[u].x;
                ss += v[u].y;
            }
        }
        for (int o = 1; o < lpg; o <<= 1) {
            s += __shfl_xor(s, o, 64);
            ss += __shfl_xor(ss, o, 64);
        }
        if (sub == 0) {
            const float cnt = (float)cpg * (float)a.HW;
            const float mu = s / cnt;
            const float var = fmaxf(ss / cnt - mu * mu, 0.f);
            mean[g] = mu;
            rstd[g] = rsqrtf(var + a.eps);
        }
    }
    __syncthreads();
    const int rows_par = GN_THREADS / CHS;
    const int cc = tid % CHS, prow = tid / CHS;
    if (prow >= rows_par) return;
    const int c0 = slab * CS + cc * 8;
    const int p_begin = pc * a.ppb, p_end = min(a.HW, p_begin + a.ppb);
    float ga[8], be[8], sc[8], sh[8];
    unpack8(ld16(a.gamma + c0), ga);
    unpack8(ld16(a.beta + c0), be);
#pragma unroll
    for (int j = 0; j < 8; ++j) {
        const int g = (cc * 8 + j) / cpg;
        sc[j] = rstd[g] * ga[j];
        sh[j] = be[j] - mean[g] * sc[j];
    }
    const half_t* src = gn_src(a, n, p_begin + prow, c0);
    const long long pstep = (long long)rows_par * (c0 < a.C1 ? a.C1 : a.C2);
    half_t* dst = a.y + ((long long)n * a.HW + p_begin + prow) * C + c0;
    const long long dstep = (long long)rows_par * C;
    auto norm8 = [&](uint4 raw) {
        float v[8];
        unpack8(raw, v);
#pragma unroll
        for (int j = 0; j < 8; ++j) {
            v[j] = v[j] * sc[j] + sh[j];
            if (a.silu) v[j] = silu_f(v[j]);
        }
        return pack8(v);
    };
    int pix = p_begin + prow;
    for (; pix + 3 * rows_par < p_end; pix += 4 * rows_par, src += 4 * pstep, dst += 4 * dstep) {
        uint4 r[4];
#pragma unroll
        for (int u = 0; u < 4; ++u) r[u] = ld16(src + u * pstep);
#pragma unroll
        for (int u = 0; u < 4; ++u) st16(dst + u * dstep, norm8(r[u]));
    }
    for (; pix < p_end; pix += rows_par, src += pstep, dst += dstep) st16(dst, norm8(ld16(src)));
}

__global__ __launch_bounds__(GN_THREADS) void gn_finalize_kernel(const GnArgs a, float* __restrict__ scale, float* __restrict__ shift) {
    __shared__ float mean[32], rstd[32];
    const int C = a.C1 + a.C2, cpg = C / 32, CS = C / a.slabs;
    const int gps = 32 / a.slabs, lpg = GN_THREADS / gps;
    const int n = blockIdx.x, slab = blockIdx.y, tid = threadIdx.x;
    {
        const int g = tid / lpg, sub = tid - g * lpg;
        float s = 0.f, ss = 0.f;
        const float* pp = a.partial + ((long long)n * a.Pstat * 32 + slab * gps + g) * 2;
        for (int i = sub; i < a.Pstat; i += 4 * lpg) {
            float2 v[4];
#pragma unroll
            for (int u = 0; u < 4; ++u) {
                const int iu = i + u * lpg;
                v[u] = *reinterpret_cast<const float2*>(pp + (long long)(iu < a.Pstat ? iu : sub) * 64);
                if (iu >= a.Pstat) v[u] = make_float2(0.f, 0.f);
            }
#pragma unroll
            for (int u = 0; u < 4; ++u) {
                s += v[u].x;
                ss += v[u].y;
            }
        }
        for (int o = 1; o < lpg; o <<= 1) {
            s += __shfl_xor(s, o, 64);
            ss += __shfl_xor(ss, o, 64);
        }
        if (sub == 0) {
            const float cnt = (float)cpg * (float)a.HW;
            const float mu = s / cnt;
            const float var = fmaxf(ss / cnt - mu * mu, 0.f);
            mean[g] = mu;
            rstd[g] = rsqrtf(var + a.eps);
        }
    }
    __syncthreads();
    for (int c = tid; c < CS; c += GN_THREADS) {
        const int g = c / cpg, cg = slab * CS + c;
        const float sc = rstd[g] * (float)a.gamma[cg];
        scale[(long long)n * C + cg] = sc;
        shift[(long long)n * C + cg] = (float)a.beta[cg] - mean[g] * sc;
    }
}

__global__ __launch_bounds__(256) void layernorm_kernel(const half_t* __restrict__ x, const half_t* __restrict__ gamma,
                                                         const half_t* __restrict__ beta, half_t* __restrict__ y,
                                                         int rows, int C, float eps) {
    const int lane = threadIdx.x & 63;
    const int row = blockIdx.x * 4 + (threadIdx.x >> 6);
    if (row >= rows) return;
    const int CH = C >> 3;
    float v[4][8];
    float s = 0.f;
#pragma unroll
    for (int i = 0; i < 4; ++i) {
        const int cc = lane + i * 64;
        if (cc < CH) {
            unpack8(ld16(x + (long long)row * C + cc * 8), v[i]);
#pragma unroll
            for (int j = 0; j < 8; ++j) s += v[i][j];
        }
    }
    const float mu = wave_sum(s) / (float)C;
    float ss = 0.f;
#pragma unroll
    for (int i = 0; i < 4; ++i) {
        const int cc = lane + i * 64;
        if (cc < CH) {
#pragma unroll
            for (int j = 0; j < 8; ++j) {
                const float d = v[i][j] - mu;
                ss += d * d;
            }
        }
    }
    const float rs = rsqrtf(wave_sum(ss) / (float)C + eps);
#pragma unroll
    for (int i = 0; i < 4; ++i) {
        const int cc = lane + i * 64;
        if (cc < CH) {
            float ga[8], be[8];
            unpack8(ld16(gamma + cc * 8), ga);
            unpack8(ld16(beta + cc * 8), be);
#pragma unroll
            for (int j = 0; j < 8; ++j) v[i][j] = (v[i][j] - mu) * rs * ga[j] + be[j];
            st16(y + (long long)row * C + cc * 8, pack8(v[i]));
        }
    }
}

__global__ __launch_bounds__(256) void softmax_rows_kernel(half_t* __restrict__ s, int cols, int valid, long long ld) {
    __shared__ float red[4];
    half_t* row = s + (long long)blockIdx.x * ld;
    const int tid = threadIdx.x, lane = tid & 63, wid = tid >> 6;
    const int CH = cols >> 3;
    float mx = -INFINITY;
    for (int c = tid; c < CH; c += 256) {
        float v[8];
        unpack8(ld16(row + c * 8), v);
#pragma unroll
        for (int j = 0; j < 8; ++j) mx = fmaxf(mx, c * 8 + j < valid ? v[j] : -INFINITY);
    }
    mx = wave_max(mx);
    if (lane == 0) red[wid] = mx;
    __syncthreads();
    mx = fmaxf(fmaxf(red[0], red[1]), fmaxf(red[2], red[3]));
    __syncthreads();
    float sum = 0.f;
    for (int c = tid; c < CH; c += 256) {
        float v[8];
        unpack8(ld16(row + c * 8), v);
#pragma unroll
        for (int j = 0; j < 8; ++j) sum += c * 8 + j < valid ? __expf(v[j] - mx) : 0.f;
    }
    sum = wave_sum(sum);
    if (lane == 0) red[wid] = sum;
    __syncthreads();
    const float inv = 1.0f / (red[0] + red[1] + red[2] + red[3]);
    for (int c = tid; c < CH; c += 256) {
        float v[8];
        unpack8(ld16(row + c * 8), v);
#pragma unroll
        for (int j = 0; j < 8; ++j) v[j] = c * 8 + j < valid ? __expf(v[j] - mx) * inv : 0.f;
        st16(row + c * 8, pack8(v));
    }
}

}

size_t groupnorm_workspace_bytes(int n_img, int HW) {
    int P = gn_num_chunks(n_img, HW);
    const int p8 = HW / 16 < 256 ? HW / 16 : 256;
    if (p8 > P) P = p8;
    if (HW / 256 > P) P = HW / 256;
    return (size_t)n_img * P * 32 * 2 * sizeof(float);
}

int groupnorm_stats_launch(const half_t* x1, int C1, const half_t* x2, int C2, int n_img, int HW, float* partial, hipStream_t stream) {
    const int C = C1 + C2;
    if (x1 == nullptr || partial == nullptr) return LD_ERR_ARG;
    if (C % 32 || C1 % 8 || C2 % 8 || C > 8192 || C1 <= 0 || (C2 > 0 && x2 == nullptr)) return LD_ERR_SHAPE;
    GnArgs a;
    a.x1 = x1; a.x2 = x2; a.C1 = C1; a.C2 = C2; a.HW = HW;
    a.P = a.Pstat = gn_num_chunks(n_img, HW);
    a.ppb = (HW + a.P - 1) / a.P;
    a.partial = partial; a.gamma = nullptr; a.beta = nullptr; a.y = nullptr; a.eps = 0.f; a.silu = 0;
    a.slabs = gn_slabs(C);
    hipLaunchKernelGGL(gn_stats_kernel, dim3(a.P, n_img, a.slabs), dim3(GN_THREADS), 0, stream, a);
    return hipGetLastError() == hipSuccess ? LD_OK : LD_ERR_HIP;
}

int groupnorm_launch(const half_t* x1, int C1, const half_t* x2, int C2, int n_img, int HW, const half_t* gamma,
                     const half_t* beta, float eps, int silu, half_t* y, float* partial, hipStream_t stream, int stats_ready) {
    const int C = C1 + C2;
    if (x1 == nullptr || y == nullptr || partial == nullptr || gamma == nullptr || beta == nullptr) return LD_ERR_ARG;
    if (C % 32 || C1 % 8 || C2 % 8 || C > 8192 || C1 <= 0 || (C2 > 0 && x2 == nullptr)) return LD_ERR_SHAPE;
    GnArgs a;
    a.x1 = x1; a.x2 = x2; a.C1 = C1; a.C2 = C2; a.HW = HW;
    a.P = gn_num_chunks(n_img, HW);
    a.Pstat = stats_ready > 0 ? stats_ready : a.P;
    a.ppb = (HW + a.P - 1) / a.P;
    a.partial = partial; a.gamma = gamma; a.beta = beta; a.y = y; a.eps = eps; a.silu = silu;
    a.slabs = gn_slabs(C);
    dim3 grid(a.P, n_img, a.slabs);
    if (!stats_ready) hipLaunchKernelGGL(gn_stats_kernel, grid, dim3(GN_THREADS), 0, stream, a);
    hipLaunchKernelGGL(gn_apply_kernel, grid, dim3(GN_THREADS), 0, stream, a);
    return hipGetLastError() == hipSuccess ? LD_OK : LD_ERR_HIP;
}

int groupnorm_scale_shift_launch(const half_t* x1, int C1, const half_t* x2, int C2, int n_img, int HW, const half_t* gamma, const half_t* beta,
                                 float eps, float* partial, float* scale, float* shift, hipStream_t stream, int stats_ready) {
    const int C = C1 + C2;
    if (x1 == nullptr || partial == nullptr || gamma == nullptr || beta == nullptr || scale == nullptr || shift == nullptr) return LD_ERR_ARG;
    if (C % 32 || C1 % 8 || C2 % 8 || C > 8192 || C1 <= 0 || (C2 > 0 && x2 == nullptr)) return LD_ERR_SHAPE;
    GnArgs a;
    a.x1 = x1; a.x2 = x2; a.C1 = C1; a.C2 = C2; a.HW = HW;
    a.P = gn_num_chunks(n_img, HW);
    a.Pstat = stats_ready > 0 ? stats_ready : a.P;
    a.ppb = (HW + a.P - 1) / a.P;
    a.partial = partial; a.gamma = gamma; a.beta = beta; a.y = nullptr; a.eps = eps; a.silu = 0;
    a.slabs = gn_slabs(C);
    if (!stats_ready) hipLaunchKernelGGL(gn_stats_kernel, dim3(a.P, n_img, a.slabs), dim3(GN_THREADS), 0, stream, a);
    hipLaunchKernelGGL(gn_finalize_kernel, dim3(n_img, a.slabs), dim3(GN_THREADS), 0, stream, a, scale, shift);
    return hipGetLastError() == hipSuccess ? LD_OK : LD_ERR_HIP;
}

int layernorm_launch(const half_t* x, const half_t* gamma, const half_t* beta, half_t* y, int rows, int C, float eps,
                     hipStream_t stream) {
    if (x == nullptr || y == nullptr || gamma == nullptr || beta == nullptr) return LD_ERR_ARG;
    if (C % 8 || C > 2048 || rows <= 0) return LD_ERR_SHAPE;
    hipLaunchKernelGGL(layernorm_kernel, dim3((rows + 3) / 4), dim3(256), 0, stream, x, gamma, beta, y, rows, C, eps);
    return hipGetLastError() == hipSuccess ? LD_OK : LD_ERR_HIP;
}

int softmax_rows_launch(half_t* s, int rows, int cols, long long ld, hipStream_t stream, int valid) {
    if (s == nullptr || rows <= 0 || cols % 8 || ld % 8 || valid > cols) return LD_ERR_SHAPE;
    hipLaunchKernelGGL(softmax_rows_kernel, dim3(rows), dim3(256), 0, stream, s, cols, valid > 0 ? valid : cols, ld);
    return hipGetLastError() == hipSuccess ? LD_OK : LD_ERR_HIP;
}
```

lightdiffusion_amd/csrc/runtime.h:

```cpp
#pragma once
#include <cstdio>
#include <cstdlib>
#include <string>
#include <unordered_map>
#include <vector>

#include "kernels.h"

enum ParamKind { PK_VEC = 0, PK_MAT = 1, PK_CONV3 = 2, PK_GEGLU_W = 3, PK_GEGLU_B = 4 };

struct ParamSlot {
    std::string name;
    int ndim = 0;
    int64_t shape[4] = {0, 0, 0, 0};
    int kind = PK_VEC;
    int geglu_bn = 0;
    size_t elems = 0, offset = 0;
    bool loaded = false;
};

struct ParamTable {
    std::vector<ParamSlot> slots;
    std::unordered_map<std::string, int> index;
    size_t bytes = 0;
// ... 46 lines not shown
            case PK_GEGLU_B: st = repack_rows_launch(src, f32, (int)s.shape[0], 1, dst, s.geglu_bn, stream); break;
            case PK_MAT: st = repack_rows_launch(src, f32, (int)s.shape[0], (int)(s.elems / s.shape[0]), dst, 0, stream); break;
            default: st = repack_rows_launch(src, f32, 1, (int)s.elems, dst, 0, stream); break;
        }
        if (st == LD_OK) s.loaded = true;
        return st;
    }
};

struct Arena {
    char* base = nullptr;
    size_t cap = 0, off = 0, peak = 0;
    void* alloc(size_t bytes) {
        off = (off + 255) / 256 * 256;
        void* p = base + off;
        off += bytes;
        if (off > peak) peak = off;
        return p;
    }
    half_t* halfs(size_t n) { return reinterpret_cast<half_t*>(alloc(n * sizeof(half_t))); }
    size_t mark() const { return off; }
    void release(size_t m) { off = m; }
};

enum KClass { KC_CONV3 = 0, KC_GEMM = 1, KC_ATTN = 2, KC_GNORM = 3, KC_LNORM = 4, KC_MISC = 5, KC_COUNT = 6 };

struct Timing {
    std::vector<hipEvent_t> ev;
    std::vector<int> cls;
    std::vector<std::string> desc;
    std::vector<const char*> kname;
    std::vector<double> kflops;
    struct PerKernel {
        double ms = 0, flops = 0;
        int launches = 0;
    };
    std::vector<std::pair<std::string, PerKernel>> per_kernel;
    struct Launch {
        const char* what = "";
        long long a = 0, b = 0, d = 0, e = 0;
        float us = 0.f;
    };
    std::vector<Launch> rec;
    bool verbose = false;
    size_t used = 0;
    double ms[KC_COUNT] = {0}, flops[KC_COUNT] = {0};
    int launches[KC_COUNT] = {0};
    hipEvent_t next() {
        if (used == ev.size()) {
            hipEvent_t e;
            (void)hipEventCreate(&e);
            ev.push_back(e);
        }
        return ev[used++];
    }
    void reset() {
        used = 0;
        cls.clear();
        desc.clear();
        kname.clear();
        kflops.clear();
        per_kernel.clear();
        rec.clear();
        verbose = getenv("LD_PROFILE_DUMP") != nullptr;
        for (int i = 0; i < KC_COUNT; ++i) ms[i] = flops[i] = 0, launches[i] = 0;
    }
    void collect() {
        for (size_t i = 0; i + 1 < used; i += 2) {
            float t = 0.f;
            (void)hipEventElapsedTime(&t, ev[i], ev[i + 1]);
            ms[cls[i / 2]] += t;
            const char* kn = i / 2 < kname.size() && kname[i / 2] ? kname[i / 2] : "?";
            size_t j = 0;
            while (j < per_kernel.size() && per_kernel[j].first != kn) ++j;
            if (j == per_kernel.size()) per_kernel.push_back({kn, PerKernel()});
            per_kernel[j].second.ms += t;
            per_kernel[j].second.flops += i / 2 < kflops.size() ? kflops[i / 2] : 0.0;
            per_kernel[j].second.launches += 1;
            if (i / 2 < rec.size()) rec[i / 2].us = t * 1e3f;
            if (verbose && i / 2 < desc.size()) fprintf(stderr, "[ld_profile] %8.1f us  %s  %s\n", t * 1e3, desc[i / 2].c_str(), kn);
        }
    }
    void destroy() {
        for (hipEvent_t e : ev) (void)hipEventDestroy(e);
        ev.clear();
    }
    int format_launches(char* buf, size_t buf_bytes) const {
        if (buf == nullptr || buf_bytes == 0) return LD_ERR_ARG;
        size_t off = 0;
        buf[0] = 0;
        for (size_t i = 0; i < rec.size(); ++i) {
            const Launch& r = rec[i];
            const int w = snprintf(buf + off, buf_bytes - off, "%s\t%lld\t%lld\t%lld\t%lld\t%.0f\t%.2f\t%s\n", r.what, r.a, r.b, r.d, r.e,
                                   i < kflops.size() ? kflops[i] : 0.0, r.us, i < kname.size() && kname[i] ? kname[i] : "?");
            if (w < 0 || (size_t)w >= buf_bytes - off) return LD_ERR_ARG;
            off += (size_t)w;
        }
        return LD_OK;
    }
};

struct Exec {
    Timing* timing = nullptr;
    hipStream_t stream = nullptr;
    bool dry = false;
    Arena* arena = nullptr;
    int status = LD_OK;
    int launches = 0;
    double flops = 0.0;
    float* splitk_ws = nullptr;
    size_t splitk_bytes = 0;
    int* sync_ws = nullptr;

    void note(int st) {
        if (st != LD_OK && status == LD_OK) status = st;
    }
    bool overflow() const { return !dry && arena->peak > arena->cap; }

    void t_begin(int c, double fl, int nl, const char* what = "", long long a = 0, long long b = 0, long long d = 0, long long e = 0) {
        if (timing == nullptr || dry) return;
        timing->cls.push_back(c);
        if (timing->verbose) {
            char buf[160];
            snprintf(buf, sizeof buf, "%-10s %8lld %6lld %6lld %4lld  %.2f GFLOP", what, a, b, d, e, fl * 1e-9);
            timing->desc.push_back(buf);
        }
        timing->flops[c] += fl;
        timing->launches[c] += nl;
        timing->kflops.push_back(fl);
        Timing::Launch r;
        r.what = what;
        r.a = a; r.b = b; r.d = d; r.e = e;
        timing->rec.push_back(r);
        (void)hipEventRecord(timing->next(), stream);
    }
    void t_end(const char* kernel_name = "misc") {
        if (timing == nullptr || dry) return;
        (void)hipEventRecord(timing->next(), stream);
        timing->kname.push_back(kernel_name);
    }

    void with_scratch(GemmParams& p) const {
        if (p.batch != 1) return;
        p.partial = splitk_ws; p.partial_bytes = splitk_bytes; p.sync = sync_ws;
    }
    void gemm(GemmParams p, const GemmPlan* plan = nullptr) {
        const double fl = 2.0 * p.M * (double)p.N * p.K * p.batch;
        flops += fl;
        with_scratch(p);
        launches += 1;
        if (dry || status != LD_OK) return;
        t_begin(p.conv && p.ksize == 3 ? KC_CONV3 : KC_GEMM, fl, 1, p.conv ? (p.ksize == 3 ? "conv3" : "conv1") : (p.act == 2 ? "geglu" : "gemm"),
                p.M, p.N, p.K, p.batch);
        note(plan != nullptr ? gemm_run(p, *plan, stream) : gemm_launch(p, stream));
        t_end(gemm_last_kernel_name());
    }
    bool conv_takes_skip_segment(GemmParams p) const {
        with_scratch(p);
        return gemm_plan(p).takes_skip_segment;
    }
    void groupnorm(const half_t* x1, int C1, const half_t* x2, int C2, int n, int HW, const half_t* g, const half_t* b, float eps,
                   int silu, half_t* y, float* ready = nullptr, int ready_P = 0) {
        const size_t m = arena->mark();
        if (ready_P <= 0) ready = nullptr;
        float* ws = ready != nullptr ? ready : reinterpret_cast<float*>(arena->alloc(groupnorm_workspace_bytes(n, HW)));
        const int nl = ready != nullptr ? 1 : 2;
        launches += nl;
        t_begin(KC_GNORM, 0.0, nl, "groupnorm", n, HW, C1 + C2, silu);
        if (!dry && status == LD_OK) note(groupnorm_launch(x1, C1, x2, C2, n, HW, g, b, eps, silu, y, ws, stream, ready != nullptr ? ready_P : 0));
        t_end(ready != nullptr ? "gn_apply_kernel" : "gn_stats_kernel+gn_apply_kernel");
        arena->release(m);
    }
    void gn_silu_conv(GemmParams p, int n_img, int HW, const half_t* gamma, const half_t* beta, float eps, half_t* g, float* ready = nullptr, int ready_P = 0) {
        with_scratch(p);
        if (ready_P <= 0) ready = nullptr;
        const GemmPlan fused = gemm_plan(p, true);
        if (fused.can_fuse_groupnorm) {
            const int C = p.C1 + p.C2;
            const size_t m = arena->mark();
            float* ws = ready != nullptr ? ready : reinterpret_cast<float*>(arena->alloc(groupnorm_workspace_bytes(n_img, HW)));
            float* scale = reinterpret_cast<float*>(arena->alloc((size_t)n_img * C * sizeof(float)));
            float* shift = reinterpret_cast<float*>(arena->alloc((size_t)n_img * C * sizeof(float)));
            const int nl = ready != nullptr ? 1 : 2;
            launches += nl;
            t_begin(KC_GNORM, 0.0, nl, "gn_stats", n_img, HW, C, 1);
            if (!dry && status == LD_OK)
                note(groupnorm_scale_shift_launch(p.A, p.C1, p.A2, p.C2, n_img, HW, gamma, beta, eps, ws, scale, shift, stream, ready != nullptr ? ready_P : 0));
            t_end(ready != nullptr ? "gn_finalize_kernel" : "gn_stats_kernel+gn_finalize_kernel");
            p.gn_scale = scale;
            p.gn_shift = shift;
            p.gn_silu = 1;
            gemm(p, &fused);
            arena->release(m);
            return;
        }
        groupnorm(p.A, p.C1, p.A2, p.C2, n_img, HW, gamma, beta, eps, 1, g, ready, ready_P);
        p.A = g;
        p.A2 = nullptr;
        p.C1 = p.C1 + p.C2;
        p.C2 = 0;
        gemm(p);
    }
    void attention(const AttnParams& p) {
        const double fl = 4.0 * p.B * p.H * (double)p.Lq * p.Lk * p.d;
        flops += fl;
        launches += 1;
        t_begin(KC_ATTN, fl, 1, "attention", (long long)p.B * p.H, p.Lq, p.Lk, p.d);
        if (!dry && status == LD_OK) note(attention_launch(p, stream));
        t_end(attention_last_kernel_name());
    }
};
```

lightdiffusion_amd/csrc/unet.hip:

```cpp
#include <cstring>

#include "runtime.h"
#include "../../include/ld_mi355x.h"

namespace {

struct ResW {
    std::string prefix;
    int cin = 0, cout = 0, emb_off = 0;
    int gn1_g, gn1_b, c1_w, c1_b, emb_w, emb_b, gn2_g, gn2_b, c2_w, c2_b, sk_w = -1, sk_b = -1;
    size_t f_c2_w = 0, f_c2_b = 0;
};
struct StW {
    int c = 0, bn = 0, ctx_slot = 0;
    size_t f_qk_w = 0, f_q2_w = 0, f_ff1_w = 0, f_qk_b = 0, f_q2_b = 0, f_ff1_b = 0, f_qk_s = 0, f_q2_s = 0,
           f_ff1_s = 0;
    size_t f_mo_w = 0, f_mo_b = 0;
    int gn_g, gn_b, pin_w, pin_b, ln1_g, ln1_b, q1_w, k1_w, v1_w, o1_w, o1_b, ln2_g, ln2_b, q2_w, k2_w, v2_w, o2_w, o2_b, ln3_g,
        ln3_b, ff1_w, ff1_b, ff2_w, ff2_b, pout_w, pout_b;
};
struct ConvW {
    int cin = 0, cout = 0, w = -1, b = -1;
    long long f_up = -1;
};
enum LayerKind { L_CONV_IN, L_RES, L_ST, L_DOWN, L_UP };
struct Layer {
    int kind, idx;
};
struct Feat {
    half_t* p;
    int C, H, W;
    float* gn = nullptr;
    int gnP = 0;
};

}

struct ld_unet {
    ld_unet_config cfg;
    ParamTable pt;
    std::vector<ResW> res;
    std::vector<StW> st;
    std::vector<ConvW> convs;
    std::vector<std::vector<Layer>> in_blocks, out_blocks;
    std::vector<Layer> mid_block;
    int te0_w, te0_b, te2_w, te2_b, outn_g, outn_b, outc_w, outc_b;
    int emb_total = 0, ted = 0;
    Arena arena;
    char* ws_base = nullptr;
    size_t ws_bytes = 0;
    float* splitk_ws = nullptr;
    size_t splitk_bytes = 0;
    float* log_sigmas = nullptr;
    int max_n = 0, max_h = 0, max_w = 0, max_tok = 0;
    half_t* ctx16 = nullptr;
    std::vector<half_t*> ctx_k, ctx_vt;
    int ctx_n = 0, ctx_tok = 0, ctx_tpad = 0;
    int plan_n = 0, plan_h = 0, plan_w = 0, plan_pair = 0;
    int last_launches = 0;
    double last_flops = 0.0;
    int* sync_ws = nullptr;
    struct W8 { int slot, N, Cin; size_t off; };
    std::vector<W8> w8_list;
    std::vector<long long> w8_of_slot;
    char* w8_base = nullptr;
    size_t w8_bytes = 0;
    const half_t* w8(int slot) const {
        return (w8_base != nullptr && slot >= 0 && slot < (int)w8_of_slot.size() && w8_of_slot[slot] >= 0) ? reinterpret_cast<const half_t*>(w8_base + w8_of_slot[slot]) : nullptr;
    }
    void want_w8(int slot, int N, int Cin) {
        if (!conv8_weight_eligible(N, Cin)) return;
        w8_list.push_back({slot, N, Cin, w8_bytes});
        w8_bytes += (conv8_weight_bytes(N, Cin) + 255) / 256 * 256;
    }
    Timing timing;
    bool want_timing = false;
    char* fold_base = nullptr;
    size_t fold_bytes = 0;
    bool fold_dirty = true;
};

namespace {

std::string S(const char* fmt, int a = 0, int b = 0) {
    char buf[160];
    snprintf(buf, sizeof buf, fmt, a, b);
    return buf;
}

int add_res(ld_unet* u, const std::string& p, int cin, int cout) {
    ParamTable& t = u->pt;
    ResW r;
    r.prefix = p;
    r.cin = cin;
    r.cout = cout;
    r.gn1_g = t.add(p + ".in_layers.0.weight", PK_VEC, {cin});
    r.gn1_b = t.add(p + ".in_layers.0.bias", PK_VEC, {cin});
    r.c1_w = t.add(p + ".in_layers.2.weight", PK_CONV3, {cout, cin, 3, 3});
    r.c1_b = t.add(p + ".in_layers.2.bias", PK_VEC, {cout});
    u->want_w8(r.c1_w, cout, cin);
    r.gn2_g = t.add(p + ".out_layers.0.weight", PK_VEC, {cout});
    r.gn2_b = t.add(p + ".out_layers.0.bias", PK_VEC, {cout});
    r.c2_w = t.add(p + ".out_layers.3.weight", PK_CONV3, {cout, cout, 3, 3});
    r.c2_b = t.add(p + ".out_layers.3.bias", PK_VEC, {cout});
    u->want_w8(r.c2_w, cout, cout);
    if (cin != cout) {
        r.sk_w = t.add(p + ".skip_connection.weight", PK_MAT, {cout, cin, 1, 1});
        r.sk_b = t.add(p + ".skip_connection.bias", PK_VEC, {cout});
        size_t& fb = u->fold_bytes;
        r.f_c2_w = fb;
        fb += ((size_t)cout * (9 * cout + cin) * sizeof(half_t) + 255) / 256 * 256;
        r.f_c2_b = fb;
        fb += ((size_t)cout * sizeof(half_t) + 255) / 256 * 256;
    }
    r.emb_off = u->emb_total;
    u->emb_total += cout;
    u->res.push_back(r);
    return (int)u->res.size() - 1;
}

int add_st(ld_unet* u, const std::string& p, int c) {
    ParamTable& t = u->pt;
    const int ctx = u->cfg.context_dim;
    StW s;
    s.c = c;
    s.bn = gemm_pick_bn(8 * c);
    s.ctx_slot = (int)u->st.size();
    s.gn_g = t.add(p + ".norm.weight", PK_VEC, {c});
    s.gn_b = t.add(p + ".norm.bias", PK_VEC, {c});
    s.pin_w = t.add(p + ".proj_in.weight", PK_MAT, {c, c, 1, 1});
    s.pin_b = t.add(p + ".proj_in.bias", PK_VEC, {c});
    const std::string b = p + ".transformer_blocks.0";
    s.ln1_g = t.add(b + ".norm1.weight", PK_VEC, {c});
    s.ln1_b = t.add(b + ".norm1.bias", PK_VEC, {c});
    s.q1_w = t.add(b + ".attn1.to_q.weight", PK_MAT, {c, c});
    s.k1_w = t.add(b + ".attn1.to_k.weight", PK_MAT, {c, c}, 16);
    s.v1_w = t.add(b + ".attn1.to_v.weight", PK_MAT, {c, c}, 16);
    s.o1_w = t.add(b + ".attn1.to_out.0.weight", PK_MAT, {c, c});
    s.o1_b = t.add(b + ".attn1.to_out.0.bias", PK_VEC, {c});
    s.ln2_g = t.add(b + ".norm2.weight", PK_VEC, {c});
    s.ln2_b = t.add(b + ".norm2.bias", PK_VEC, {c});
    s.q2_w = t.add(b + ".attn2.to_q.weight", PK_MAT, {c, c});
    s.k2_w = t.add(b + ".attn2.to_k.weight", PK_MAT, {c, ctx});
    s.v2_w = t.add(b + ".attn2.to_v.weight", PK_MAT, {c, ctx});
    s.o2_w = t.add(b + ".attn2.to_out.0.weight", PK_MAT, {c, c});
    s.o2_b = t.add(b + ".attn2.to_out.0.bias", PK_VEC, {c});
    s.ln3_g = t.add(b + ".norm3.weight", PK_VEC, {c});
    s.ln3_b = t.add(b + ".norm3.bias", PK_VEC, {c});
    s.ff1_w = t.add(b + ".ff.net.0.proj.weight", PK_GEGLU_W, {8 * c, c}, 256, s.bn);
    s.ff1_b = t.add(b + ".ff.net.0.proj.bias", PK_GEGLU_B, {8 * c}, 256, s.bn);
    s.ff2_w = t.add(b + ".ff.net.2.weight", PK_MAT, {c, 4 * c});
    s.ff2_b = t.add(b + ".ff.net.2.bias", PK_VEC, {c});
    s.pout_w = t.add(p + ".proj_out.weight", PK_MAT, {c, c, 1, 1});
    s.pout_b = t.add(p + ".proj_out.bias", PK_VEC, {c});
    {
        size_t& fb = u->fold_bytes;
        auto take = [&](size_t bytes) {
            const size_t o = fb;
            fb += (bytes + 255) / 256 * 256;
            return o;
        };
        const size_t C = (size_t)c;
        s.f_qk_w = take(3 * C * C * sizeof(half_t));
        s.f_q2_w = take(C * C * sizeof(half_t));
        s.f_ff1_w = take(8 * C * C * sizeof(half_t));
        s.f_qk_b = take(3 * C * sizeof(half_t));
        s.f_q2_b = take(C * sizeof(half_t));
        s.f_ff1_b = take(8 * C * sizeof(half_t));
        s.f_qk_s = take(3 * C * sizeof(float));
        s.f_q2_s = take(C * sizeof(float));
        s.f_ff1_s = take(8 * C * sizeof(float));
        s.f_mo_w = take(5 * C * C * sizeof(half_t));
        s.f_mo_b = take(C * sizeof(half_t));
    }
    u->st.push_back(s);
    return (int)u->st.size() - 1;
}

int add_conv(ld_unet* u, const std::string& p, int cin, int cout) {
    ConvW c;
    c.cin = cin;
    c.cout = cout;
    c.w = u->pt.add(p + ".weight", PK_CONV3, {cout, cin, 3, 3});
    c.b = u->pt.add(p + ".bias", PK_VEC, {cout});
    u->convs.push_back(c);
    return (int)u->convs.size() - 1;
}

int build(ld_unet* u) {
    const ld_unet_config& c = u->cfg;
    if (c.num_levels < 1 || c.num_levels > 8 || c.model_channels % 32 || c.num_heads < 1) return LD_ERR_ARG;
    const int mc = c.model_channels;
    u->ted = mc * 4;
    ParamTable& t = u->pt;
    u->te0_w = t.add("time_embed.0.weight", PK_MAT, {u->ted, mc});
    u->te0_b = t.add("time_embed.0.bias", PK_VEC, {u->ted});
    u->te2_w = t.add("time_embed.2.weight", PK_MAT, {u->ted, u->ted});
    u->te2_b = t.add("time_embed.2.bias", PK_VEC, {u->ted});
    u->in_blocks.push_back({{L_CONV_IN, add_conv(u, "input_blocks.0.0", c.in_channels, mc)}});
    int ch = mc, idx = 1, td = 0;
    std::vector<int> chans{mc};
    for (int lvl = 0; lvl < c.num_levels; ++lvl) {
        for (int r = 0; r < c.num_res_blocks[lvl]; ++r) {
            std::vector<Layer> L;
            L.push_back({L_RES, add_res(u, S("input_blocks.%d.0", idx), ch, c.channel_mult[lvl] * mc)});
            ch = c.channel_mult[lvl] * mc;
            if (c.transformer_depth[td++] > 0) L.push_back({L_ST, add_st(u, S("input_blocks.%d.1", idx), ch)});
            u->in_blocks.push_back(L);
            chans.push_back(ch);
            ++idx;
        }
        if (lvl != c.num_levels - 1) {
            u->in_blocks.push_back({{L_DOWN, add_conv(u, S("input_blocks.%d.0.op", idx), ch, ch)}});
            chans.push_back(ch);
            ++idx;
        }
    }
    u->mid_block.push_back({L_RES, add_res(u, "middle_block.0", ch, ch)});
    if (c.transformer_depth_middle > 0) u->mid_block.push_back({L_ST, add_st(u, "middle_block.1", ch)});
    u->mid_block.push_back({L_RES, add_res(u, "middle_block.2", ch, ch)});
    int n_out = 0;
    for (int lvl = 0; lvl < c.num_levels; ++lvl) n_out += c.num_res_blocks[lvl] + 1;
    int tdo = n_out;
    idx = 0;
    for (int lvl = c.num_levels - 1; lvl >= 0; --lvl) {
        for (int i = 0; i <= c.num_res_blocks[lvl]; ++i) {
            const int ich = chans.back();
            chans.pop_back();
            std::vector<Layer> L;
            L.push_back({L_RES, add_res(u, S("output_blocks.%d.0", idx), ch + ich, mc * c.channel_mult[lvl])});
            ch = mc * c.channel_mult[lvl];
            int j = 1;
            if (c.transformer_depth_output[--tdo] > 0) {
                L.push_back({L_ST, add_st(u, S("output_blocks.%d.%d", idx, j), ch)});
                ++j;
            }
            if (lvl && i == c.num_res_blocks[lvl]) {
                L.push_back({L_UP, add_conv(u, S("output_blocks.%d.%d.conv", idx, j), ch, ch)});
                u->want_w8(u->convs.back().w, ch, ch);
                u->convs.back().f_up = (long long)u->fold_bytes;
                u->fold_bytes += (16 * (size_t)ch * ch * sizeof(half_t) + 255) / 256 * 256;
            }
            u->out_blocks.push_back(L);
            ++idx;
        }
    }
    u->outn_g = t.add("out.0.weight", PK_VEC, {ch});
    u->outn_b = t.add("out.0.bias", PK_VEC, {ch});
    u->outc_w = t.add("out.2.weight", PK_CONV3, {c.out_channels, mc, 3, 3});
    u->outc_b = t.add("out.2.bias", PK_VEC, {c.out_channels});
    for (size_t i = 0; i < u->res.size(); ++i)
        u->res[i].emb_w = t.add(u->res[i].prefix + ".emb_layers.1.weight", PK_MAT, {u->res[i].cout, u->ted}, i == 0 ? 256 : 16);
    for (size_t i = 0; i < u->res.size(); ++i)
        u->res[i].emb_b = t.add(u->res[i].prefix + ".emb_layers.1.bias", PK_VEC, {u->res[i].cout}, i == 0 ? 256 : 16);
    return t.finalize();
}

struct Run {
    ld_unet* u;
    Exec ex;
    int n;
    int n_alloc = 0;
    bool pair_pending = false;
    const half_t* emb_all;
    half_t* P(int slot) const { return u->pt.ptr(slot); }
    int na() const { return n_alloc > 0 ? n_alloc : n; }
    void dup(void* base, size_t half_bytes) {
        ex.launches += 1;
        ex.t_begin(KC_MISC, 0.0, 1, "dup", (long long)half_bytes, 0, 0, 1);
        if (!ex.dry && ex.status == LD_OK &&
            hipMemcpyAsync(static_cast<char*>(base) + half_bytes, base, half_bytes, hipMemcpyDeviceToDevice, ex.stream) != hipSuccess)
            ex.note(LD_ERR_HIP);
        ex.t_end("hipMemcpyAsync(pair)");
    }

    void want_stats(GemmParams& p, float* buf, int HW, int* done) {
        p.gn_part = buf;
        p.gn_P = gn_num_chunks(n, HW);
        p.gn_HW = HW;
        p.gn_ppb = (HW + p.gn_P - 1) / p.gn_P;
        p.gn_part_done = done;
    }

    half_t* conv3(const half_t* x1, int C1, const half_t* x2, int C2, int Hs, int Ws, int Hv, int Wv, int stride, int wslot, int bslot,
                  int cout, const half_t* rowvec, int ldrv, const half_t* R, half_t* out, int* Ho_, int* Wo_, int ksize = 3, float* stats = nullptr,
                  int* stats_done = nullptr, const half_t* wup = nullptr) {
        const int Ho = ksize == 3 ? (Hv - 1) / stride + 1 : Hv, Wo = ksize == 3 ? (Wv - 1) / stride + 1 : Wv;
        GemmParams p;
        p.conv = 1;
        p.ksize = ksize;
        p.A = x1; p.A2 = x2; p.C1 = C1; p.C2 = C2;
        p.Hs = Hs; p.Ws = Ws; p.Hv = Hv; p.Wv = Wv; p.Ho = Ho; p.Wo = Wo; p.stride = stride;
        p.W = P(wslot); p.ldw = ksize * ksize * (C1 + C2);
        p.W8 = ksize == 3 ? u->w8(wslot) : nullptr;
        p.Wup = wup;
        p.M = n * Ho * Wo; p.N = cout; p.K = ksize * ksize * (C1 + C2);
        p.bias_n = P(bslot);
        p.rowvec = rowvec; p.rows_per_vec = Ho * Wo; p.ldrv = ldrv;
        p.R = R; p.ldr = cout;
        p.C = out; p.ldc = cout;
        if (stats != nullptr) want_stats(p, stats, Ho * Wo, stats_done);
        ex.gemm(p);
        if (Ho_) *Ho_ = Ho;
        if (Wo_) *Wo_ = Wo;
        return out;
    }

    void linear(const half_t* x, int lda, int wslot, int bslot, const half_t* R, half_t* y, int M, int N, int K, int act = 0, int bn = 0) {
        GemmParams p;
        p.A = x; p.lda = lda;
        p.W = P(wslot); p.ldw = K;
        p.M = M; p.N = N; p.K = K;
        p.bias_n = bslot >= 0 ? P(bslot) : nullptr;
        p.R = R; p.ldr = (act == 2 ? N / 2 : N);
        p.act = act; p.bn = bn;
        p.C = y; p.ldc = (act == 2 ? N / 2 : N);
        ex.gemm(p);
    }

    Feat resblock(const ResW& r, const half_t* x1, int C1, const half_t* x2, int C2, int H, int W, float* in_stats = nullptr, int in_P = 0) {
        Arena& ar = *ex.arena;
        const size_t M = (size_t)na() * H * W;
        half_t* out = ar.halfs(M * r.cout);
        float* gno = reinterpret_cast<float*>(ar.alloc(groupnorm_workspace_bytes(na(), H * W)));
        int gno_done = 0;
        if (C2 != 0) in_stats = nullptr;
        const size_t mk = ar.mark();
        auto conv_params = [&](const half_t* a1, int c1, const half_t* a2, int c2, int wslot, int bslot, const half_t* rowvec, int ldrv, const half_t* R,
                               half_t* dst) {
            GemmParams p;
            p.conv = 1; p.ksize = 3;
            p.A = a1; p.A2 = a2; p.C1 = c1; p.C2 = c2;
            p.Hs = H; p.Ws = W; p.Hv = H; p.Wv = W; p.Ho = H; p.Wo = W; p.stride = 1;
            p.W = P(wslot); p.ldw = 9 * (c1 + c2);
            p.W8 = u->w8(wslot);
            p.M = n * H * W; p.N = r.cout; p.K = 9 * (c1 + c2);
            p.bias_n = P(bslot);
            p.rowvec = rowvec; p.rows_per_vec = H * W; p.ldrv = ldrv;
            p.R = R; p.ldr = r.cout;
            p.C = dst; p.ldc = r.cout;
            return p;
        };
        half_t* g1 = ar.halfs(M * r.cin);
        half_t* h1 = ar.halfs(M * r.cout);
        const half_t* skip = x1;
        bool fold_skip = false;
        if (r.sk_w >= 0) {
            fold_skip = u->fold_base != nullptr && ex.conv_takes_skip_segment(conv_params(h1, r.cout, nullptr, 0, r.c2_w, r.c2_b, nullptr, 0, nullptr, out));
            half_t* sk = (!fold_skip || ex.dry) ? ar.halfs(M * r.cout) : nullptr;
            if (!fold_skip) {
                conv3(x1, C1, x2, C2, H, W, H, W, 1, r.sk_w, r.sk_b, r.cout, nullptr, 0, nullptr, sk, nullptr, nullptr, 1);
                skip = sk;
            }
        }
        float* gnp = reinterpret_cast<float*>(ar.alloc(groupnorm_workspace_bytes(na(), H * W)));
        int gnp_done = 0;
        {
            GemmParams c1 = conv_params(x1, C1, x2, C2, r.c1_w, r.c1_b, emb_all + r.emb_off, u->emb_total, nullptr, h1);
            want_stats(c1, gnp, H * W, &gnp_done);
            ex.gn_silu_conv(c1, n, H * W, P(r.gn1_g), P(r.gn1_b), 1e-5f, g1, in_stats, in_P);
        }
        half_t* g2 = g1;
        if (r.cout > r.cin) g2 = ar.halfs(M * r.cout);
        {
            GemmParams c2 = conv_params(h1, r.cout, nullptr, 0, r.c2_w, r.c2_b, nullptr, 0, skip, out);
            if (fold_skip) {
                c2.S1 = x1; c2.SC1 = C1; c2.S2 = x2; c2.SC2 = C2;
                c2.W = reinterpret_cast<const half_t*>(u->fold_base + r.f_c2_w);
                c2.K = 9 * r.cout + r.cin; c2.ldw = c2.K;
                c2.bias_n = reinterpret_cast<const half_t*>(u->fold_base + r.f_c2_b);
                c2.R = nullptr;
                c2.W8 = nullptr;
            }
            want_stats(c2, gno, H * W, &gno_done);
            ex.gn_silu_conv(c2, n, H * W, P(r.gn2_g), P(r.gn2_b), 1e-5f, g2, gnp_done ? gnp : nullptr, gnp_done);
        }
        ar.release(mk);
        return {out, r.cout, H, W, gno_done ? gno : nullptr, gno_done};
    }

    Feat transformer(const StW& s, const half_t* x, int H, int W, float* in_stats = nullptr, int in_P = 0) {
        Arena& ar = *ex.arena;
        const int C = s.c, L = H * W, heads = u->cfg.num_heads, d = C / heads;
        int M = n * L;
        const size_t Ma = (size_t)na() * L;
        half_t* out = ar.halfs(Ma * C);
        float* gno = reinterpret_cast<float*>(ar.alloc(groupnorm_workspace_bytes(na(), L)));
        int gno_done = 0;
        const size_t mk = ar.mark();
        half_t* g = ar.halfs(Ma * C);
        ex.groupnorm(x, C, nullptr, 0, n, L, P(s.gn_g), P(s.gn_b), 1e-6f, 0, g, in_stats, in_P);
        half_t* t = ar.halfs(Ma * C);
        half_t* qkv = ar.halfs(Ma * 3 * C);
        half_t* ao = ar.halfs(Ma * C);
        half_t* ff = nullptr;
        float* stat = reinterpret_cast<float*>(ar.alloc((size_t)((C + 63) / 64) * Ma * 2 * sizeof(float)));
        int parts = 0;
        char* fb = u->fold_base;
        auto producer = [&](const half_t* x_, int lda, int wslot, int bslot, const half_t* R, int K) {
            GemmParams p;
            p.A = x_; p.lda = lda;
            p.W = P(wslot); p.ldw = K;
            p.M = M; p.N = C; p.K = K;
            p.bias_n = P(bslot);
            p.R = R; p.ldr = C;
            p.C = t; p.ldc = C;
            p.stat_out = stat;
            p.stat_parts_out = &parts;
            ex.gemm(p);
        };
        auto ln_args = [&](GemmParams& p, size_t wsum_off) {
            p.ln_stat = stat; p.ln_parts = parts; p.ln_rows = M;
            p.ln_inv_c = 1.0f / (float)C; p.ln_eps = 1e-5f;
            p.ln_wsum = reinterpret_cast<const float*>(fb + wsum_off);
        };
        producer(g, C, s.pin_w, s.pin_b, nullptr, C);
        {
            GemmParams p;
            p.A = t; p.lda = C;
            p.W = reinterpret_cast<const half_t*>(fb + s.f_qk_w); p.ldw = C;
            p.M = M; p.N = 3 * C; p.K = C;
            p.C = qkv; p.ldc = 3 * C;
            p.bias_n = reinterpret_cast<const half_t*>(fb + s.f_qk_b);
            ln_args(p, s.f_qk_s);
            ex.gemm(p);
        }
        {
            AttnParams a;
            a.Q = qkv; a.ldq = 3 * C; a.sQ = (long long)L * 3 * C;
            a.K = qkv + C; a.ldk = 3 * C; a.sK = (long long)L * 3 * C;
            a.V = qkv + 2 * C; a.ldv = 3 * C; a.sV = (long long)L * 3 * C;
            a.O = ao; a.ldo = C; a.sO = (long long)L * C;
            a.B = n; a.H = heads; a.Lq = L; a.Lk = L; a.d = d;
            a.scale = 1.0f / sqrtf((float)d);
            ex.attention(a);
        }
        const bool split_here = pair_pending;
        producer(ao, C, s.o1_w, s.o1_b, t, C);
        half_t* q2 = qkv;
        {
            GemmParams p;
            p.A = t; p.lda = C;
            p.W = reinterpret_cast<const half_t*>(fb + s.f_q2_w); p.ldw = C;
            p.M = M; p.N = C; p.K = C;
            p.C = q2; p.ldc = C;
            p.bias_n = reinterpret_cast<const half_t*>(fb + s.f_q2_b);
            ln_args(p, s.f_q2_s);
            ex.gemm(p);
        }
        if (split_here) {
            const size_t hb = (size_t)M * C * sizeof(half_t);
            DupArgs da;
            da.count = 3;
            da.base[0] = reinterpret_cast<char*>(t); da.base[1] = reinterpret_cast<char*>(q2); da.base[2] = reinterpret_cast<char*>(const_cast<half_t*>(x));
            da.bytes[0] = da.bytes[1] = da.bytes[2] = hb;
            ex.launches += 1;
            ex.t_begin(KC_MISC, 0.0, 1, "dup3", (long long)hb, 0, 0, 1);
            if (!ex.dry && ex.status == LD_OK) ex.note(dup_halves_launch(da, ex.stream));
            ex.t_end("dup_halves_kernel");
            pair_pending = false;
            n = n_alloc;
            M = n * L;
        }
        {
            const int Tp = u->ctx_tpad;
            AttnParams a;
            a.Q = q2; a.ldq = C; a.sQ = (long long)L * C;
            a.K = u->ctx_k[s.ctx_slot]; a.ldk = C; a.sK = (long long)Tp * C;
            a.Vt = u->ctx_vt[s.ctx_slot]; a.ldvt = Tp; a.sV = (long long)C * Tp;
            a.O = ao; a.ldo = C; a.sO = (long long)L * C;
            a.B = n; a.H = heads; a.Lq = L; a.Lk = u->ctx_tok; a.d = d;
            a.scale = 1.0f / sqrtf((float)d);
            ex.attention(a);
        }
        producer(ao, C, s.o2_w, s.o2_b, t, C);
        ff = ar.halfs(Ma * 4 * C);
        {
            GemmParams p;
            p.A = t; p.lda = C;
            p.W = reinterpret_cast<const half_t*>(fb + s.f_ff1_w); p.ldw = C;
            p.M = M; p.N = 8 * C; p.K = C;
            p.bias_n = reinterpret_cast<const half_t*>(fb + s.f_ff1_b);
            p.act = 2; p.bn = s.bn;
            p.C = ff; p.ldc = 4 * C; p.ldr = 4 * C;
            ln_args(p, s.f_ff1_s);
            ex.gemm(p);
        }
        {
            GemmParams p;
            p.conv = 1; p.ksize = 1;
            p.A = ff; p.A2 = t; p.C1 = 4 * C; p.C2 = C;
            p.Hs = p.Hv = p.Ho = H; p.Ws = p.Wv = p.Wo = W; p.stride = 1;
            p.W = reinterpret_cast<const half_t*>(fb + s.f_mo_w); p.ldw = 5 * C;
            p.M = M; p.N = C; p.K = 5 * C;
            p.bias_n = reinterpret_cast<const half_t*>(fb + s.f_mo_b);
            p.R = x; p.ldr = C;
            p.C = out; p.ldc = C;
            want_stats(p, gno, L, &gno_done);
            ex.gemm(p);
        }
        ar.release(mk);
        return {out, C, H, W, gno_done ? gno : nullptr, gno_done};
    }
};

int fold_layernorms(ld_unet* u, hipStream_t stream) {
    for (const StW& s : u->st) {
        const int C = s.c;
        char* fb = u->fold_base;
        auto H = [&](size_t off) { return reinterpret_cast<half_t*>(fb + off); };
        auto F = [&](size_t off) { return reinterpret_cast<float*>(fb + off); };
        const half_t* P_q1 = u->pt.ptr(s.q1_w);
        int st = ln_fold_launch(P_q1, 3 * C, C, u->pt.ptr(s.ln1_g), u->pt.ptr(s.ln1_b), nullptr, H(s.f_qk_w), H(s.f_qk_b), F(s.f_qk_s), stream);
        if (st == LD_OK) st = ln_fold_launch(u->pt.ptr(s.q2_w), C, C, u->pt.ptr(s.ln2_g), u->pt.ptr(s.ln2_b), nullptr, H(s.f_q2_w), H(s.f_q2_b), F(s.f_q2_s), stream);
        if (st == LD_OK) st = ln_fold_launch(u->pt.ptr(s.ff1_w), 8 * C, C, u->pt.ptr(s.ln3_g), u->pt.ptr(s.ln3_b), u->pt.ptr(s.ff1_b), H(s.f_ff1_w), H(s.f_ff1_b), F(s.f_ff1_s), stream);
        if (st == LD_OK) st = mlp_out_fold_launch(u->pt.ptr(s.pout_w), u->pt.ptr(s.ff2_w), u->pt.ptr(s.ff2_b), u->pt.ptr(s.pout_b), C, H(s.f_mo_w), H(s.f_mo_b), stream);
        if (st != LD_OK) return st;
    }
    for (const ResW& r : u->res) {
        if (r.sk_w < 0) continue;
        const int st = skip_fold_launch(u->pt.ptr(r.c2_w), u->pt.ptr(r.sk_w), u->pt.ptr(r.c2_b), u->pt.ptr(r.sk_b), r.cout, 9 * r.cout, r.cin,
                                        reinterpret_cast<half_t*>(u->fold_base + r.f_c2_w), reinterpret_cast<half_t*>(u->fold_base + r.f_c2_b), stream);
        if (st != LD_OK) return st;
    }
    for (const ConvW& c : u->convs) {
        if (c.f_up < 0) continue;
        const int st = upconv_fold_launch(u->pt.ptr(c.w), c.cout, c.cin, reinterpret_cast<half_t*>(u->fold_base + c.f_up), stream);
        if (st != LD_OK) return st;
    }
    u->fold_dirty = false;
    return LD_OK;
}

int derive_conv8_weights(ld_unet* u, hipStream_t stream) {
    for (const ld_unet::W8& w : u->w8_list) {
        const int st = conv8_repack_launch(u->pt.ptr(w.slot), w.N, w.Cin, reinterpret_cast<half_t*>(u->w8_base + w.off), stream);
        if (st != LD_OK) return st;
    }
    return LD_OK;
}

int run_forward(ld_unet* u, bool dry, const float* x, const float* sigma, float* out, int n, int h, int w, int eps_only, hipStream_t stream,
                size_t* dry_peak = nullptr, bool pair = false) {
    if (!dry && u->fold_dirty) {
        if (u->w8_base != nullptr) {
            const int st = derive_conv8_weights(u, stream);
            if (st != LD_OK) return st;
        }
        {
            const int st = fold_layernorms(u, stream);
            if (st != LD_OK) return st;
        }
        u->fold_dirty = false;
    }
    if (pair && (n & 1)) return LD_ERR_SHAPE;
    Run R;
    R.u = u;
    R.n = n;
    R.n_alloc = n;
    Exec& ex = R.ex;
    ex.stream = stream;
    ex.dry = dry;
    Arena plan;
    ex.arena = dry ? &plan : &u->arena;
    ex.splitk_ws = u->splitk_ws;
    ex.splitk_bytes = u->splitk_bytes;
    ex.sync_ws = u->sync_ws;
    if (u->want_timing && !dry) {
        u->timing.reset();
        ex.timing = &u->timing;
    }
    Arena& ar = *ex.arena;
    ar.release(0);
    const ld_unet_config& c = u->cfg;
    const int mc = c.model_channels, ted = u->ted;
    const int in_mod = pair ? n / 2 : 0;
    if (pair) R.pair_pending = true;

    half_t* temb = ar.halfs((size_t)n * mc);
    ex.launches += 1;
    ex.t_begin(KC_MISC, 0.0, 1);
    if (!dry) ex.note(timestep_embed_launch(sigma, u->log_sigmas, 1000, n, mc, temb, nullptr, stream, in_mod));
    ex.t_end("timestep_embed_kernel");
    half_t* e1 = ar.halfs((size_t)n * ted);
    R.linear(temb, mc, u->te0_w, u->te0_b, nullptr, e1, n, ted, mc, 1);
    half_t* semb = ar.halfs((size_t)n * ted);
    R.linear(e1, ted, u->te2_w, u->te2_b, nullptr, semb, n, ted, ted, 1);
    half_t* emb_all = ar.halfs((size_t)n * u->emb_total);
    R.linear(semb, ted, u->res[0].emb_w, u->res[0].emb_b, nullptr, emb_all, n, u->emb_total, ted);
    R.emb_all = emb_all;

    auto run_layers = [&](const std::vector<Layer>& layers, Feat f, const half_t* x2, int C2, int outH, int outW) -> Feat {
        for (const Layer& L : layers) {
            switch (L.kind) {
                case L_RES: {
                    f = R.resblock(u->res[L.idx], f.p, f.C, x2, C2, f.H, f.W, f.gn, f.gnP);
                    x2 = nullptr;
                    C2 = 0;
                    break;
                }
                case L_ST: f = R.transformer(u->st[L.idx], f.p, f.H, f.W, f.gn, f.gnP); break;
                case L_DOWN: {
                    const ConvW& cw = u->convs[L.idx];
                    const int Ho = (f.H - 1) / 2 + 1, Wo = (f.W - 1) / 2 + 1;
                    if (R.pair_pending) {
                        R.dup(const_cast<half_t*>(f.p), (size_t)R.n * f.H * f.W * f.C * sizeof(half_t));
                        R.pair_pending = false;
                        R.n = n;
                    }
                    half_t* o = ar.halfs((size_t)n * Ho * Wo * cw.cout);
                    float* gno = reinterpret_cast<float*>(ar.alloc(groupnorm_workspace_bytes(n, Ho * Wo)));
                    int gno_done = 0;
                    R.conv3(f.p, f.C, nullptr, 0, f.H, f.W, f.H, f.W, 2, cw.w, cw.b, cw.cout, nullptr, 0, nullptr, o, nullptr, nullptr, 3, gno, &gno_done);
                    f = {o, cw.cout, Ho, Wo, gno_done ? gno : nullptr, gno_done};
                    break;
                }
                case L_UP: {
                    const ConvW& cw = u->convs[L.idx];
                    const int Hv = outH > 0 ? outH : f.H * 2, Wv = outW > 0 ? outW : f.W * 2;
                    half_t* o = ar.halfs((size_t)n * Hv * Wv * cw.cout);
                    const half_t* wup = (u->fold_base != nullptr && cw.f_up >= 0) ? reinterpret_cast<const half_t*>(u->fold_base + cw.f_up) : nullptr;
                    R.conv3(f.p, f.C, nullptr, 0, f.H, f.W, Hv, Wv, 1, cw.w, cw.b, cw.cout, nullptr, 0, nullptr, o, nullptr, nullptr, 3, nullptr, nullptr, wup);
                    f = {o, cw.cout, Hv, Wv};
                    break;
                }
                default: break;
            }
        }
        return f;
    };

    std::vector<Feat> hs;
    Feat f{nullptr, 0, h, w};
    {
        const ConvW& cw = u->convs[u->in_blocks[0][0].idx];
        half_t* o = ar.halfs((size_t)n * h * w * mc);
        if (R.pair_pending) R.n = n / 2;
        SmallConvInArgs a;
        a.x = x; a.scale_sigma = sigma; a.w = u->pt.ptr(cw.w); a.b = u->pt.ptr(cw.b); a.y = o;
        a.N = R.n; a.Cin = c.in_channels; a.H = h; a.W = w; a.Cout = mc;
        if (R.pair_pending) a.dup_off = (long long)R.n * h * w * mc;
        ex.launches += 1;
        ex.flops += 2.0 * R.n * h * w * mc * 9.0 * c.in_channels;
        ex.t_begin(KC_MISC, 2.0 * R.n * h * w * mc * 9.0 * c.in_channels, 1);
        if (!dry) ex.note(small_conv_in_launch(a, stream));
        ex.t_end("small_conv_in_kernel");
        f = {o, mc, h, w};
        hs.push_back(f);
    }
    for (size_t b = 1; b < u->in_blocks.size(); ++b) {
        f = run_layers(u->in_blocks[b], f, nullptr, 0, 0, 0);
        if (R.pair_pending && b == 1) {
            R.dup(const_cast<half_t*>(f.p), (size_t)R.n * f.H * f.W * f.C * sizeof(half_t));
            R.pair_pending = false;
            R.n = n;
            f.gn = nullptr;
            f.gnP = 0;
        }
        hs.push_back(f);
    }
    if (R.pair_pending) {
        R.pair_pending = false;
        R.n = n;
    }
    f = run_layers(u->mid_block, f, nullptr, 0, 0, 0);
    for (size_t b = 0; b < u->out_blocks.size(); ++b) {
        const Feat skip = hs.back();
        hs.pop_back();
        if (skip.H != f.H || skip.W != f.W) ex.note(LD_ERR_SHAPE);
        const int oh = hs.empty() ? 0 : hs.back().H, ow = hs.empty() ? 0 : hs.back().W;
        f = run_layers(u->out_blocks[b], f, skip.p, skip.C, oh, ow);
    }
    {
        half_t* g = ar.halfs((size_t)n * f.H * f.W * f.C);
        ex.groupnorm(f.p, f.C, nullptr, 0, n, f.H * f.W, u->pt.ptr(u->outn_g), u->pt.ptr(u->outn_b), 1e-5f, 1, g, f.gn, f.gnP);
        SmallConvOutArgs a;
        a.x = g; a.w = u->pt.ptr(u->outc_w); a.b = u->pt.ptr(u->outc_b);
        a.N = n; a.H = f.H; a.W = f.W; a.Cin = f.C; a.Cout = c.out_channels;
        a.mode = eps_only ? 2 : 0;
        a.x_in = x; a.sigma = sigma; a.out = out; a.in_mod = in_mod;
        ex.launches += 1;
        ex.flops += 2.0 * n * f.H * f.W * f.C * 9.0 * c.out_channels;
        ex.t_begin(KC_MISC, 2.0 * n * f.H * f.W * f.C * 9.0 * c.out_channels, 1);
        if (!dry) ex.note(small_conv_out_launch(a, stream));
        ex.t_end("small_conv_out_kernel");
    }
    u->last_launches = ex.launches;
    u->last_flops = ex.flops;
    if (dry_peak) *dry_peak = ar.peak;
    return ex.status;
}

}

extern "C" {

int ld_unet_create(const ld_unet_config* cfg, ld_unet** out) {
    if (cfg == nullptr || out == nullptr) return LD_ERR_ARG;
    ld_unet* u = new ld_unet();
    u->cfg = *cfg;
    const int st = build(u);
    if (st != LD_OK) {
        u->pt.destroy();
        delete u;
        return st;
    }
    std::vector<float> ls(1000);
    {
        const double b0 = sqrt(0.00085), b1 = sqrt(0.012);
        double ac = 1.0;
        for (int i = 0; i < 1000; ++i) {
            const double sb = b0 + (b1 - b0) * (double)i / 999.0;
            ac *= 1.0 - sb * sb;
            ls[i] = (float)log(sqrt((1.0 - ac) / ac));
        }
    }
    u->w8_of_slot.assign(u->pt.slots.size(), -1);
    for (const ld_unet::W8& w : u->w8_list) u->w8_of_slot[w.slot] = (long long)w.off;
    if (u->w8_bytes > 0 && hipMalloc((void**)&u->w8_base, u->w8_bytes) != hipSuccess) u->w8_base = nullptr;
    if (u->fold_bytes > 0 && hipMalloc((void**)&u->fold_base, u->fold_bytes) != hipSuccess) {
        u->pt.destroy();
        delete u;
        return LD_ERR_HIP;
    }
    if (hipMalloc((void**)&u->sync_ws, LD_SYNC_INTS * sizeof(int)) != hipSuccess || hipMemset(u->sync_ws, 0, LD_SYNC_INTS * sizeof(int)) != hipSuccess ||
        hipMalloc((void**)&u->log_sigmas, 1000 * sizeof(float)) != hipSuccess ||
        hipMemcpy(u->log_sigmas, ls.data(), 1000 * sizeof(float), hipMemcpyHostToDevice) != hipSuccess) {
        u->pt.destroy();
        delete u;
        return LD_ERR_HIP;
    }
    *out = u;
    return LD_OK;
}

void ld_unet_destroy(ld_unet* u) {
    if (u == nullptr) return;
    u->pt.destroy();
    u->timing.destroy();
    if (u->ws_base) (void)hipFree(u->ws_base);
    if (u->log_sigmas) (void)hipFree(u->log_sigmas);
    if (u->sync_ws) (void)hipFree(u->sync_ws);
    if (u->w8_base) (void)hipFree(u->w8_base);
    if (u->fold_base) (void)hipFree(u->fold_base);
    delete u;
}

int ld_unet_param_count(const ld_unet* u) { return u ? (int)u->pt.slots.size() : 0; }

int ld_unet_param_info(const ld_unet* u, int i, const char** name, int* ndim, int64_t shape[4]) {
    if (u == nullptr || i < 0 || i >= (int)u->pt.slots.size()) return LD_ERR_ARG;
    const ParamSlot& s = u->pt.slots[i];
    if (name) *name = s.name.c_str();
    if (ndim) *ndim = s.ndim;
    if (shape)
        for (int k = 0; k < 4; ++k) shape[k] = s.shape[k];
    return LD_OK;
}

int ld_unet_load_param(ld_unet* u, const char* name, const void* src, int dtype, void* stream) {
    if (u == nullptr || name == nullptr) return LD_ERR_ARG;
    u->fold_dirty = true;
    return u->pt.load(name, src, dtype, (hipStream_t)stream);
}

size_t ld_unet_workspace_bytes(const ld_unet* u) { return u ? u->ws_bytes : 0; }
size_t ld_unet_weight_bytes(const ld_unet* u) { return u ? u->pt.bytes + (u->fold_base ? u->fold_bytes : 0) + (u->w8_base ? u->w8_bytes : 0) : 0; }

int ld_unet_reserve(ld_unet* u, int max_n, int max_h, int max_w, int max_tok) {
    if (u == nullptr || max_n < 1 || max_h < 1 || max_w < 1 || max_tok < 1) return LD_ERR_ARG;
    if (u->ws_base) {
        (void)hipFree(u->ws_base);
        u->ws_base = nullptr;
    }
    u->arena = Arena();
    u->plan_n = u->plan_h = u->plan_w = u->plan_pair = 0;
    u->ctx_tok = max_tok;
    u->ctx_tpad = (max_tok + 7) & ~7;
    u->ctx_k.assign(u->st.size(), nullptr);
    u->ctx_vt.assign(u->st.size(), nullptr);
    size_t peak = 0;
    int st = run_forward(u, true, nullptr, nullptr, nullptr, max_n, max_h, max_w, 0, nullptr, &peak);
    if (st != LD_OK) return st;
    if (!(max_n & 1)) {
        size_t peak2 = 0;
        st = run_forward(u, true, nullptr, nullptr, nullptr, max_n, max_h, max_w, 0, nullptr, &peak2, true);
        if (st != LD_OK) return st;
        if (peak2 > peak) peak = peak2;
    }
    const size_t act = (peak + 4095) / 4096 * 4096;
    const size_t tpad = (size_t)u->ctx_tpad;
    size_t ctxb = ((size_t)max_n * tpad * u->cfg.context_dim * sizeof(half_t) + 255) / 256 * 256;
    for (const StW& s : u->st) ctxb += 2 * (((size_t)max_n * tpad * s.c * sizeof(half_t) + 255) / 256 * 256);
    u->splitk_bytes = (size_t)96 << 20;
    u->ws_bytes = act + ctxb + u->splitk_bytes + 4096;
    if (hipMalloc((void**)&u->ws_base, u->ws_bytes) != hipSuccess) {
        u->ws_base = nullptr;
        return LD_ERR_HIP;
    }
    char* p = u->ws_base;
    u->arena.base = p;
    u->arena.cap = act;
    u->arena.off = u->arena.peak = 0;
    p += act;
    u->splitk_ws = reinterpret_cast<float*>(p);
    p += u->splitk_bytes;
    u->ctx16 = reinterpret_cast<half_t*>(p);
    p += ((size_t)max_n * tpad * u->cfg.context_dim * sizeof(half_t) + 255) / 256 * 256;
    for (size_t i = 0; i < u->st.size(); ++i) {
        const size_t b = ((size_t)max_n * tpad * u->st[i].c * sizeof(half_t) + 255) / 256 * 256;
// ... 127 lines not shown
```

lightdiffusion_amd/ops.py:

```python
from __future__ import annotations

import math
from typing import Optional

import torch

from ._lib import F16, F32, check, lib


def _stream() -> int:
    return torch.cuda.current_stream().cuda_stream


def _p(t: Optional[torch.Tensor]) -> Optional[int]:
    if t is None:
        return None
    assert t.is_cuda and t.is_contiguous(), "device-resident contiguous tensors only"
    return t.data_ptr()


def last_kernel() -> str:
    return lib().ld_op_last_kernel().decode()


_WS = {}


def _ws(nbytes: int, device) -> torch.Tensor:
    d = torch.device(device)
    idx = d.index if d.index is not None else torch.cuda.current_device()
    n = max(nbytes, 256)
    if torch.cuda.is_current_stream_capturing():
        return torch.empty(n, dtype=torch.uint8, device=device)
    key = (idx, torch.cuda.current_stream(idx).cuda_stream)
    buf = _WS.get(key)
    if buf is None or buf.numel() < n:
        buf = torch.empty(n, dtype=torch.uint8, device=device)
        _WS[key] = buf
    return buf[:n]


def linear(x: torch.Tensor, weight: torch.Tensor, bias: Optional[torch.Tensor] = None, residual: Optional[torch.Tensor] = None,
           act: str = "none", alpha: float = 1.0) -> torch.Tensor:
    code = {"none": 0, "silu": 1, "geglu": 2, "quick_gelu": 3}[act]
    K = x.shape[-1]
    N = weight.shape[0]
    M = x.numel() // K
    y = torch.empty(*x.shape[:-1], N // 2 if code == 2 else N, dtype=torch.float16, device=x.device)
    ws = _ws(64 << 20, x.device)
    check(lib().ld_op_linear(_p(x), _p(weight), _p(bias), _p(residual), _p(y), M, N, K, alpha, code, _p(ws), ws.numel(), _stream()),
          "ld_op_linear")
    return y


def linear_ln(x: torch.Tensor, w_prod: torch.Tensor, b_prod: Optional[torch.Tensor], gamma: torch.Tensor, beta: torch.Tensor,
              weight: torch.Tensor, bias: Optional[torch.Tensor], eps: float = 1e-5):
    M, C = x.shape
    N = weight.shape[0]
    t = torch.empty(M, C, dtype=torch.float16, device=x.device)
    y = torch.empty(M, N, dtype=torch.float16, device=x.device)
    ws = _ws(2 * N * C + 8 * N + 8 * ((C + 63) // 64) * M + 4096, x.device)
    check(lib().ld_op_linear_ln(_p(x), _p(w_prod), _p(b_prod), _p(gamma), _p(beta), _p(weight), _p(bias), _p(t), _p(y), M, C, N, eps,
                                _p(ws), ws.numel(), _stream()), "ld_op_linear_ln")
    return t, y


def linear_ln_geglu(x: torch.Tensor, w_prod: torch.Tensor, b_prod: Optional[torch.Tensor], gamma: torch.Tensor, beta: torch.Tensor,
                    weight: torch.Tensor, bias: torch.Tensor, eps: float = 1e-5):
    M, C = x.shape
    N = weight.shape[0]
    t = torch.empty(M, C, dtype=torch.float16, device=x.device)
    y = torch.empty(M, N // 2, dtype=torch.float16, device=x.device)
    ws = _ws(4 * N * C + 12 * N + 8 * ((C + 63) // 64) * M + 4096, x.device)
    check(lib().ld_op_linear_ln_geglu(_p(x), _p(w_prod), _p(b_prod), _p(gamma), _p(beta), _p(weight), _p(bias), _p(t), _p(y), M, C, N, eps,
                                      _p(ws), ws.numel(), _stream()), "ld_op_linear_ln_geglu")
    return t, y


def repack_conv_weight(w_oihw: torch.Tensor) -> torch.Tensor:
    O, I, kh, kw = w_oihw.shape
    w_oihw = w_oihw.contiguous()
    out = torch.empty(O, kh * kw * I, dtype=torch.float16, device=w_oihw.device)
    if kh == 3:
        check(lib().ld_op_repack_conv(_p(w_oihw), F32 if w_oihw.dtype == torch.float32 else F16, O, I, _p(out), _stream()),
              "ld_op_repack_conv")
    else:
        out.copy_(w_oihw.reshape(O, I))
    return out


def conv2d(x: torch.Tensor, w_packed: torch.Tensor, bias: Optional[torch.Tensor], ksize: int = 3, stride: int = 1,
           x2: Optional[torch.Tensor] = None, out_hw: Optional[tuple] = None, rowvec: Optional[torch.Tensor] = None,
           residual: Optional[torch.Tensor] = None) -> torch.Tensor:
    n, h, w, c1 = x.shape
    c2 = 0 if x2 is None else x2.shape[-1]
    hv, wv = (h, w) if out_hw is None else out_hw
    cout = w_packed.shape[0]
    ho = (hv - 1) // stride + 1 if ksize == 3 else hv
    wo = (wv - 1) // stride + 1 if ksize == 3 else wv
    y = torch.empty(n, ho, wo, cout, dtype=torch.float16, device=x.device)
    ws = _ws(192 << 20, x.device)
    check(lib().ld_op_conv(_p(x), c1, _p(x2), c2, n, h, w, hv, wv, stride, ksize, _p(w_packed), _p(bias), _p(rowvec), _p(residual),
                           _p(y), cout, _p(ws), ws.numel(), _stream()), "ld_op_conv")
    return y


def upconv2x_fold(w_packed: torch.Tensor) -> torch.Tensor:
    O = w_packed.shape[0]
    I = w_packed.shape[1] // 9
    out = torch.empty(4, O, 4 * I, dtype=torch.float16, device=w_packed.device)
    check(lib().ld_op_upconv2x_fold(_p(w_packed), O, I, _p(out), _stream()), "ld_op_upconv2x_fold")
    return out


def upconv2x(x: torch.Tensor, w_packed: torch.Tensor, w_fold: torch.Tensor, bias: Optional[torch.Tensor], out_hw: Optional[tuple] = None) -> torch.Tensor:
    n, h, w, c = x.shape
    hv, wv = (2 * h, 2 * w) if out_hw is None else out_hw
    cout = w_packed.shape[0]
    y = torch.empty(n, hv, wv, cout, dtype=torch.float16, device=x.device)
    ws = _ws(192 << 20, x.device)
    check(lib().ld_op_upconv2x(_p(x), c, n, h, w, hv, wv, _p(w_packed), _p(w_fold), _p(bias), _p(y), cout, _p(ws), ws.numel(), _stream()),
          "ld_op_upconv2x")
    return y


def conv2d_skip(x: torch.Tensor, w_packed: torch.Tensor, bias: torch.Tensor, s1: torch.Tensor, s2: Optional[torch.Tensor], w_skip: torch.Tensor,
                b_skip: torch.Tensor, rowvec: Optional[torch.Tensor] = None) -> torch.Tensor:
    n, h, w, c = x.shape
    sc1 = s1.shape[-1]
    sc2 = 0 if s2 is None else s2.shape[-1]
    cout = w_packed.shape[0]
    y = torch.empty(n, h, w, cout, dtype=torch.float16, device=x.device)
    ws = _ws(lib().ld_op_conv_skip_ws_bytes(c, sc1, sc2, cout), x.device)
    check(lib().ld_op_conv_skip(_p(x), c, n, h, w, _p(w_packed), _p(bias), _p(s1), sc1, _p(s2), sc2, _p(w_skip), _p(b_skip), _p(rowvec), _p(y), cout,
                                _p(ws), ws.numel(), _stream()), "ld_op_conv_skip")
    return y


def conv2d_gn_partials(x: torch.Tensor, w_packed: torch.Tensor, bias: Optional[torch.Tensor], out_hw: Optional[tuple] = None,
                       residual: Optional[torch.Tensor] = None):
    import ctypes
    n, h, w, c = x.shape
    hv, wv = (h, w) if out_hw is None else out_hw
    cout = w_packed.shape[0]
    y = torch.empty(n, hv, wv, cout, dtype=torch.float16, device=x.device)
    part = torch.zeros(lib().ld_op_conv_gn_partials_floats(n, hv * wv), dtype=torch.float32, device=x.device)
    chunks = ctypes.c_int(0)
    ws = _ws(192 << 20, x.device)
    check(lib().ld_op_conv_gn_partials(_p(x), c, n, h, w, hv, wv, _p(w_packed), _p(bias), _p(residual), _p(y), cout, _p(part), ctypes.byref(chunks),
                                       _p(ws), ws.numel(), _stream()), "ld_op_conv_gn_partials")
    if chunks.value == 0:
        return y, None
    return y, part[: n * chunks.value * 64].view(n, chunks.value, 32, 2)


def group_norm_silu_conv2d(x: torch.Tensor, gamma: torch.Tensor, beta: torch.Tensor, eps: float, w_packed: torch.Tensor,
                           bias: Optional[torch.Tensor], x2: Optional[torch.Tensor] = None, rowvec: Optional[torch.Tensor] = None,
                           residual: Optional[torch.Tensor] = None) -> torch.Tensor:
    n, h, w, c1 = x.shape
    c2 = 0 if x2 is None else x2.shape[-1]
    cout = w_packed.shape[0]
    y = torch.empty(n, h, w, cout, dtype=torch.float16, device=x.device)
    ws = _ws(lib().ld_op_groupnorm_conv_ws_bytes(c1, c2, n, h, w, cout), x.device)
    check(lib().ld_op_groupnorm_conv(_p(x), c1, _p(x2), c2, n, h, w, _p(gamma), _p(beta), eps, _p(w_packed), _p(bias), _p(rowvec), _p(residual),
                                     _p(y), cout, _p(ws), ws.numel(), _stream()), "ld_op_groupnorm_conv")
    return y


def group_norm(x: torch.Tensor, gamma: torch.Tensor, beta: torch.Tensor, eps: float, silu: bool = False,
               x2: Optional[torch.Tensor] = None) -> torch.Tensor:
    n, c1 = x.shape[0], x.shape[-1]
    hw = x.numel() // (n * c1)
    c2 = 0 if x2 is None else x2.shape[-1]
    y = torch.empty(*x.shape[:-1], c1 + c2, dtype=torch.float16, device=x.device)
    ws = _ws(lib().ld_op_groupnorm_ws_bytes(n, hw), x.device)
    check(lib().ld_op_groupnorm(_p(x), c1, _p(x2), c2, n, hw, _p(gamma), _p(beta), eps, int(silu), _p(y), _p(ws), _stream()),
          "ld_op_groupnorm")
    return y


def layer_norm(x: torch.Tensor, gamma: torch.Tensor, beta: torch.Tensor, eps: float = 1e-5) -> torch.Tensor:
    c = x.shape[-1]
    y = torch.empty_like(x)
    check(lib().ld_op_layernorm(_p(x), _p(gamma), _p(beta), _p(y), x.numel() // c, c, eps, _stream()), "ld_op_layernorm")
    return y


def attention(q: torch.Tensor, k: torch.Tensor, v: torch.Tensor, heads: int, causal: bool = False) -> torch.Tensor:
    b, lq, c = q.shape
    lk = k.shape[1]
    d = c // heads
    lkp = (lk + 7) // 8 * 8
    vt = torch.zeros(b, c, lkp, dtype=torch.float16, device=q.device)
    vt[:, :, :lk] = v.transpose(1, 2)
    o = torch.empty_like(q)
    check(lib().ld_op_attention(_p(q), c, _p(k.contiguous()), c, _p(vt), lkp, _p(o), c, b, heads, lq, lk, d, 1.0 / math.sqrt(d), int(causal), _stream()),
          "ld_op_attention")
    return o


def attention_qkv(qkv: torch.Tensor, heads: int, causal: bool = False) -> torch.Tensor:
    b, l, c3 = qkv.shape
    c = c3 // 3
    d = c // heads
    o = torch.empty(b, l, c, dtype=torch.float16, device=qkv.device)
    base = qkv.data_ptr()
    check(lib().ld_op_attention_rowv(base, c3, base + 2 * c, c3, base + 4 * c, c3, _p(o), c, b, heads, l, l, d, 1.0 / math.sqrt(d), int(causal),
                                     _stream()), "ld_op_attention_rowv")
    return o


def attention_rowv(q: torch.Tensor, k: torch.Tensor, v: torch.Tensor, heads: int, causal: bool = False) -> torch.Tensor:
    b, lq, c = q.shape
    lk = k.shape[1]
    d = c // heads
    o = torch.empty_like(q)
    check(lib().ld_op_attention_rowv(_p(q), c, _p(k.contiguous()), c, _p(v.contiguous()), c, _p(o), c, b, heads, lq, lk, d, 1.0 / math.sqrt(d), int(causal),
                                     _stream()), "ld_op_attention_rowv")
    return o


def softmax_rows_(s: torch.Tensor) -> torch.Tensor:
    cols = s.shape[-1]
    check(lib().ld_op_softmax_rows(_p(s), s.numel() // cols, cols, _stream()), "ld_op_softmax_rows")
    return s


def timestep_embed(sigma: torch.Tensor, log_sigmas: torch.Tensor, dim: int):
    n = sigma.numel()
    out = torch.empty(n, dim, dtype=torch.float16, device=sigma.device)
    t = torch.empty(n, dtype=torch.float32, device=sigma.device)
    check(lib().ld_op_timestep_embed(_p(sigma), _p(log_sigmas), log_sigmas.numel(), n, dim, _p(out), _p(t), _stream()),
          "ld_op_timestep_embed")
    return out, t


def cfg_combine(den2: torch.Tensor, cfg: float) -> torch.Tensor:
    half = den2.shape[0] // 2
    out = torch.empty_like(den2[:half])
    check(lib().ld_op_cfg_combine(_p(den2), _p(out), float(cfg), out.numel(), _stream()), "ld_op_cfg_combine")
    return out


def axpby_(x: torch.Tensor, a: float, y: Optional[torch.Tensor] = None, b: float = 0.0, z: Optional[torch.Tensor] = None,
           c: float = 0.0) -> torch.Tensor:
    check(lib().ld_op_axpby(_p(x), float(a), _p(y), float(b), _p(z), float(c), x.numel(), _stream()), "ld_op_axpby")
    return x


def bislerp(samples: torch.Tensor, width: int, height: int) -> torch.Tensor:
    x = samples.float().contiguous()
    n, c, h, w = x.shape
    tmp = torch.empty(n, c, h, width, dtype=torch.float32, device=x.device)
    y = torch.empty(n, c, height, width, dtype=torch.float32, device=x.device)
    check(lib().ld_op_bislerp(_p(x), _p(tmp), _p(y), n, c, h, w, height, width, _stream()), "ld_op_bislerp")
    return y.to(samples.dtype)


import torch.nn as nn


def _to_f16_cl(x: torch.Tensor) -> torch.Tensor:
    return x.to(torch.float16).contiguous(memory_format=torch.channels_last)


class _NoInit:
    def reset_parameters(self):
        return None


class Linear(_NoInit, nn.Module):
    def __init__(self, in_features, out_features, bias=True, device=None, dtype=None):
        super().__init__()
        self.in_features, self.out_features = in_features, out_features
        self.weight = nn.Parameter(torch.empty(out_features, in_features, device=device, dtype=dtype), requires_grad=False)
        self.bias = nn.Parameter(torch.empty(out_features, device=device, dtype=dtype), requires_grad=False) if bias else None

    def forward(self, x):
        w = self.weight.to(x.device, torch.float16)
        b = None if self.bias is None else self.bias.to(x.device, torch.float16)
        return linear(x.to(torch.float16).contiguous(), w.contiguous(), b).to(x.dtype)


class Conv2d(_NoInit, nn.Module):
    def __init__(self, in_channels, out_channels, kernel_size, stride=1, padding=0, dilation=1, groups=1, bias=True,
                 padding_mode="zeros", device=None, dtype=None):
        super().__init__()
        k = kernel_size if isinstance(kernel_size, int) else kernel_size[0]
        st = stride if isinstance(stride, int) else stride[0]
        pd = padding if isinstance(padding, int) else padding[0]
        if k not in (1, 3) or pd != k // 2 or dilation not in (1, (1, 1)) or groups != 1 or padding_mode != "zeros":
            raise NotImplementedError("MI355X Conv2d: kernel 1 or 3 with padding k//2, no dilation / groups (all the SD1.x UNet and VAE use)")
        self.in_channels, self.out_channels, self.kernel_size, self.stride, self.padding = in_channels, out_channels, (k, k), (st, st), (pd, pd)
        self.weight = nn.Parameter(torch.empty(out_channels, in_channels, k, k, device=device, dtype=dtype), requires_grad=False)
        self.bias = nn.Parameter(torch.empty(out_channels, device=device, dtype=dtype), requires_grad=False) if bias else None
        self._packed = None

    def _weights(self, device):
        key = (self.weight.data_ptr(), self.weight._version, str(device))
        if self._packed is None or self._packed[0] != key:
            wp = repack_conv_weight(self.weight.detach().to(device))
            b = torch.zeros(self.out_channels, dtype=torch.float16, device=device) if self.bias is None else self.bias.detach().to(device, torch.float16)
            self._packed = (key, wp, b.contiguous())
        return self._packed[1], self._packed[2]

    def forward(self, x):
# ... 53 lines not shown
```

Baseline: 61.40 steps/s.

## Fuse split-K reduce with GroupNorm apply for next-layer normalized input

```diff
diff --git a/include/ld_mi355x.h b/include/ld_mi355x.h
--- a/include/ld_mi355x.h
+++ b/include/ld_mi355x.h
@@ -90,6 +90,10 @@
 size_t ld_op_conv_skip_ws_bytes(int c, int sc1, int sc2, int cout);
 int ld_op_conv_skip(const void* x, int c, int n, int h, int w, const void* wt, const void* bias, const void* s1, int sc1, const void* s2, int sc2,
                     const void* wskip, const void* bskip, const void* rowvec, void* y, int cout, void* ws, size_t ws_bytes, void* stream);
+int ld_op_conv_gn_finish(const void* x1, int c1, const void* x2, int c2, int n, int h, int w, int ksize, const void* wt, const void* bias,
+                         const void* rowvec, const void* residual, const void* s1, int sc1, const void* s2, int sc2, const void* gamma,
+                         const void* beta, float eps, int silu, const void* gn_x2, int gn_c2, void* y, void* yn, int cout, float* part, int* chunks,
+                         int* applied, int offer, void* ws, size_t ws_bytes, void* stream);
 int ld_op_upconv2x_fold(const void* wt, int cout, int cin, void* wfold, void* stream);
 int ld_op_upconv2x(const void* x, int c, int n, int h, int w, int hv, int wv, const void* wt, const void* wfold, const void* bias, void* y, int cout,
                    void* ws, size_t ws_bytes, void* stream);
diff --git a/lightdiffusion_amd/_lib.py b/lightdiffusion_amd/_lib.py
--- a/lightdiffusion_amd/_lib.py
+++ b/lightdiffusion_amd/_lib.py
@@ -80,6 +80,7 @@
     "ld_op_layernorm": (_I, [_P, _P, _P, _P, _I, _I, _F, _P]),
     "ld_op_attention": (_I, [_P, _I, _P, _I, _P, _I, _P, _I, _I, _I, _I, _I, _I, _F, _I, _P]),
     "ld_op_conv_gn_partials_floats": (_Z, [_I, _I]),
+    "ld_op_conv_gn_finish": (_I, [_P, _I, _P, _I, _I, _I, _I, _I, _P, _P, _P, _P, _P, _I, _P, _I, _P, _P, _F, _I, _P, _I, _P, _P, _I, _P, _P, _P, _I, _P, _Z, _P]),
     "ld_op_conv_gn_partials": (_I, [_P, _I, _I, _I, _I, _I, _I, _P, _P, _P, _P, _I, _P, _P, _P, _Z, _P]),
     "ld_op_attention_rowv": (_I, [_P, _I, _P, _I, _P, _I, _P, _I, _I, _I, _I, _I, _I, _F, _I, _P]),
     "ld_op_softmax_rows": (_I, [_P, _I, _I, _P]),
diff --git a/lightdiffusion_amd/csrc/capi.hip b/lightdiffusion_amd/csrc/capi.hip
--- a/lightdiffusion_amd/csrc/capi.hip
+++ b/lightdiffusion_amd/csrc/capi.hip
@@ -164,6 +164,50 @@
     return op_conv(x, c, nullptr, 0, n, h, w, hv, wv, 1, 3, wt, bias, nullptr, residual, y, cout, ws, ws_bytes, stream, part, chunks);
 }
 
+int ld_op_conv_gn_finish(const void* x1, int c1, const void* x2, int c2, int n, int h, int w, int ksize, const void* wt, const void* bias,
+                         const void* rowvec, const void* residual, const void* s1, int sc1, const void* s2, int sc2, const void* gamma,
+                         const void* beta, float eps, int silu, const void* gn_x2, int gn_c2, void* y, void* yn, int cout, float* part, int* chunks,
+                         int* applied, int offer, void* ws, size_t ws_bytes, void* stream_) {
+    op_begin();
+    if (part == nullptr || chunks == nullptr || applied == nullptr || gamma == nullptr || beta == nullptr || yn == nullptr || ws == nullptr) return LD_ERR_ARG;
+    if ((ksize != 1 && ksize != 3) || gn_c2 < 0 || (gn_c2 > 0 && gn_x2 == nullptr)) return LD_ERR_ARG;
+    hipStream_t stream = (hipStream_t)stream_;
+    const int HW = h * w;
+    if (ws_bytes < groupnorm_workspace_bytes(n, HW)) return LD_ERR_ARG;
+    *chunks = 0;
+    *applied = 0;
+    GemmParams p;
+    p.gn_part = part;
+    p.gn_P = gn_num_chunks(n, HW);
+    p.gn_HW = HW;
+    p.gn_ppb = (HW + p.gn_P - 1) / p.gn_P;
+    p.gn_part_done = chunks;
+    p.conv = 1;
+    p.ksize = ksize;
+    p.A = (const half_t*)x1; p.A2 = (const half_t*)x2; p.C1 = c1; p.C2 = c2;
+    p.Hs = p.Hv = p.Ho = h; p.Ws = p.Wv = p.Wo = w; p.stride = 1;
+    p.S1 = (const half_t*)s1; p.SC1 = sc1; p.S2 = (const half_t*)s2; p.SC2 = sc2;
+    p.K = ksize * ksize * (c1 + c2) + sc1 + sc2;
+    p.W = (const half_t*)wt; p.ldw = p.K;
+    p.M = n * HW; p.N = cout;
+    p.bias_n = (const half_t*)bias;
+    p.rowvec = (const half_t*)rowvec; p.rows_per_vec = HW; p.ldrv = cout;
+    p.R = (const half_t*)residual; p.ldr = cout;
+    p.C = (half_t*)y; p.ldc = cout;
+    p.partial = (float*)ws;
+    p.partial_bytes = ws_bytes;
+    if (offer) {
+        p.gnf_gamma = (const half_t*)gamma; p.gnf_beta = (const half_t*)beta; p.gnf_eps = eps; p.gnf_silu = silu;
+        p.gnf_y = (half_t*)yn; p.gnf_C2 = gn_c2; p.gnf_applied = applied;
+    }
+    if (const int st = gemm_op(p, stream); st != LD_OK) return st;
+    if (*applied) return LD_OK;
+    if (gn_c2 > 0)
+        return groupnorm_launch((const half_t*)y, cout, (const half_t*)gn_x2, gn_c2, n, HW, (const half_t*)gamma, (const half_t*)beta, eps, silu, (half_t*)yn, (float*)ws, stream);
+    if (*chunks > 0) return groupnorm_launch((const half_t*)y, cout, nullptr, 0, n, HW, (const half_t*)gamma, (const half_t*)beta, eps, silu, (half_t*)yn, part, stream, *chunks);
+    return groupnorm_launch((const half_t*)y, cout, nullptr, 0, n, HW, (const half_t*)gamma, (const half_t*)beta, eps, silu, (half_t*)yn, (float*)ws, stream);
+}
+
 size_t ld_op_groupnorm_conv_ws_bytes(int c1, int c2, int n, int h, int w, int cout) {
     op_begin();
     const size_t C = (size_t)c1 + c2, HW = (size_t)h * w;
diff --git a/lightdiffusion_amd/csrc/gemm.h b/lightdiffusion_amd/csrc/gemm.h
--- a/lightdiffusion_amd/csrc/gemm.h
+++ b/lightdiffusion_amd/csrc/gemm.h
@@ -57,10 +57,44 @@
     int c8_S = 0;
     const half_t* Wup = nullptr;
     int dbg = 0;
+    const half_t* gnf_gamma = nullptr;
+    const half_t* gnf_beta = nullptr;
+    float gnf_eps = 0.f;
+    int gnf_silu = 0;
+    half_t* gnf_y = nullptr;
+    int gnf_C2 = 0;
+    int* gnf_applied = nullptr;
+    int gnf_cb = 0, gnf_threads = 0;
 };
 
+#ifdef __HIPCC__
+__device__ __forceinline__ void epilogue_store8(const GemmParams& p, int z, int m, int n_out, int n_bias, float (&v)[8]) {
+    const bool hb = p.bias_n != nullptr && p.act != 2, hv = p.rowvec != nullptr, hr = p.R != nullptr;
+    const uint4 rb = hb ? ld16(p.bias_n + n_bias) : zero16();
+    const uint4 rv = hv ? ld16(p.rowvec + (long long)(m / p.rows_per_vec) * p.ldrv + n_out) : zero16();
+    const uint4 rr = hr ? ld16(p.R + (long long)z * p.sR + (long long)m * p.ldr + n_out) : zero16();
+    const float bm = p.bias_m != nullptr ? (float)p.bias_m[m] : 0.f;
+    float b[8], e[8], r[8];
+    unpack8(rb, b);
+    unpack8(rv, e);
+    unpack8(rr, r);
+#pragma unroll
+    for (int j = 0; j < 8; ++j) v[j] = v[j] + b[j] + bm + e[j];
+    if (p.act == 1) {
+#pragma unroll
+        for (int j = 0; j < 8; ++j) v[j] = silu_f(v[j]);
+    } else if (p.act == 3) {
+#pragma unroll
+        for (int j = 0; j < 8; ++j) v[j] = quick_gelu_f(v[j]);
+    }
+#pragma unroll
+    for (int j = 0; j < 8; ++j) v[j] += r[j];
+    st16(p.C + (long long)z * p.sC + (long long)m * p.ldc + n_out, pack8(v));
+}
+#endif
+
 enum GemmRoute { GR_NONE = 0, GR_CONV8, GR_CONV6, GR_GEMM7, GR_GEMM5, GR_GEMM3, GR_GEMM4, GR_UPCONV };
-enum GemmReduce { GRD_NONE = 0, GRD_PLAIN, GRD_GROUPNORM, GRD_UPCONV };
+enum GemmReduce { GRD_NONE = 0, GRD_PLAIN, GRD_GROUPNORM, GRD_UPCONV, GRD_GN_FINISH };
 struct GemmPlan {
     int status = LD_OK;
     int route = GR_NONE;
@@ -75,13 +109,16 @@
     int reduce = GRD_NONE;
     int stat_parts = 0;
     int gn_chunks = 0;
+    bool gn_applied = false;
+    int gnf_cb = 0, gnf_threads = 0;
     bool halo_tile = false;
     bool can_fuse_groupnorm = false;
     bool takes_skip_segment = false;
     const char* kernel = "";
 };
 GemmPlan gemm_plan(const GemmParams& p, bool gn_offer = false);
-int gemm_run(const GemmParams& p, const GemmPlan& plan, hipStream_t stream);
+enum { GEMM_CONTRACTION = 1, GEMM_SECOND_PASS = 2 };
+int gemm_run(const GemmParams& p, const GemmPlan& plan, hipStream_t stream, int phases = GEMM_CONTRACTION | GEMM_SECOND_PASS);
 inline int gemm_launch(const GemmParams& p, hipStream_t stream) { return gemm_run(p, gemm_plan(p), stream); }
 const char* gemm_last_kernel_name();
 
@@ -91,6 +128,9 @@
 size_t conv8_weight_bytes(int N, int Cin);
 int conv8_repack_launch(const half_t* w_okki, int N, int Cin, half_t* dst, hipStream_t stream);
 int upconv_reduce_launch(const GemmParams& p, hipStream_t stream);
+constexpr int GN_FINISH_MAXPIX = 6;
+static inline size_t gn_finish_lds_bytes(int P, int rows_par, int cb, int gpb) { return ((size_t)2 * P * rows_par * cb + (size_t)gpb * P * 2 + 2 * gpb) * sizeof(float); }
+int gn_splitk_finish_launch(const GemmParams& p, hipStream_t stream);
 #define LD_SYNC_INTS 1024
 
 static inline int gemm_pick_bn(int N) { return (N % 160 == 0) ? 160 : 128; }
diff --git a/lightdiffusion_amd/csrc/gemm.hip b/lightdiffusion_amd/csrc/gemm.hip
--- a/lightdiffusion_amd/csrc/gemm.hip
+++ b/lightdiffusion_amd/csrc/gemm.hip
@@ -11,30 +11,6 @@
 
 constexpr int BK = 64;
 constexpr int NT = 256;
-
-__device__ __forceinline__ void epilogue_store8(const GemmParams& p, int z, int m, int n_out, int n_bias, float (&v)[8]) {
-    const bool hb = p.bias_n != nullptr && p.act != 2, hv = p.rowvec != nullptr, hr = p.R != nullptr;
-    const uint4 rb = hb ? ld16(p.bias_n + n_bias) : zero16();
-    const uint4 rv = hv ? ld16(p.rowvec + (long long)(m / p.rows_per_vec) * p.ldrv + n_out) : zero16();
-    const uint4 rr = hr ? ld16(p.R + (long long)z * p.sR + (long long)m * p.ldr + n_out) : zero16();
-    const float bm = p.bias_m != nullptr ? (float)p.bias_m[m] : 0.f;
-    float b[8], e[8], r[8];
-    unpack8(rb, b);
-    unpack8(rv, e);
-    unpack8(rr, r);
-#pragma unroll
-    for (int j = 0; j < 8; ++j) v[j] = v[j] + b[j] + bm + e[j];
-    if (p.act == 1) {
-#pragma unroll
-        for (int j = 0; j < 8; ++j) v[j] = silu_f(v[j]);
-    } else if (p.act == 3) {
-#pragma unroll
-        for (int j = 0; j < 8; ++j) v[j] = quick_gelu_f(v[j]);
-    }
-#pragma unroll
-    for (int j = 0; j < 8; ++j) v[j] += r[j];
-    st16(p.C + (long long)z * p.sC + (long long)m * p.ldc + n_out, pack8(v));
-}
 
 template <int BM, int BN>
 struct EpiPre {
@@ -2237,7 +2213,7 @@
         case GR_GEMM4: s = "gemm4_kernel<" + tile + (pl.conv ? ",conv" : ",plain") + (pl.two_wg ? ",2wg>" : ">"); break;
         default: s = "gemm3_kernel<" + tile + (pl.conv ? ",conv" : ",plain") + (pl.deep ? ",deep>" : ">"); break;
     }
-    if (pl.reduce != GRD_NONE) s += pl.reduce == GRD_GROUPNORM ? "+splitk_reduce_gn_kernel" : pl.reduce == GRD_UPCONV ? "+upconv_reduce_kernel" : "+splitk_reduce_kernel";
+    if (pl.reduce != GRD_NONE && pl.reduce != GRD_GN_FINISH) s += pl.reduce == GRD_GROUPNORM ? "+splitk_reduce_gn_kernel" : pl.reduce == GRD_UPCONV ? "+upconv_reduce_kernel" : "+splitk_reduce_kernel";
     static std::mutex mu; static std::set<std::string> pool;
     std::lock_guard<std::mutex> lock(mu);
     const char* name = pool.insert(s).first->c_str();
@@ -2305,6 +2281,20 @@
                     p.ldc == p.N && (p.N / 4) % 8 == 0 && p.N / 32 <= 256;
     pl->reduce = gn ? GRD_GROUPNORM : GRD_PLAIN;
     if (gn) pl->gn_chunks = p.gn_P;
+    if (!gn || p.gnf_y == nullptr) return;
+    if (p.gnf_gamma == nullptr || p.gnf_beta == nullptr || p.gnf_C2 != 0 || p.act != 0 || p.bias_m != nullptr) return;
+    const int cpg = p.N / 32;
+    int cb = cpg;
+    while (cb % 8) cb += cpg;
+    if (cb > 80 || p.N % cb) return;
+    const int CHS = (p.N / 4) >> 3, rows_par = 256 / CHS, gpb = cb / cpg;
+    if (rows_par < 1 || p.gn_P > 32 || (p.gn_ppb + rows_par - 1) / rows_par > GN_FINISH_MAXPIX) return;
+    const int items = p.gn_P * rows_par * (cb >> 3), teams = p.gn_P * gpb * 32;
+    const int threads = ((items > teams ? items : teams) + 63) / 64 * 64;
+    if (threads > 1024 || gn_finish_lds_bytes(p.gn_P, rows_par, cb, gpb) > 64 * 1024) return;
+    pl->reduce = GRD_GN_FINISH;
+    pl->gn_applied = true;
+    pl->gnf_cb = cb; pl->gnf_threads = threads;
 }
 
 static bool upconv_plan(const GemmParams& p, GemmPlan* out) {
@@ -2558,18 +2548,26 @@
     return done(GR_GEMM3);
 }
 
-int gemm_run(const GemmParams& pin, const GemmPlan& pl, hipStream_t stream) {
-    t_last_kernel = "";
+int gemm_run(const GemmParams& pin, const GemmPlan& pl, hipStream_t stream, int phases) {
+    if (pl.reduce != GRD_GN_FINISH) {
+        if (!(phases & GEMM_CONTRACTION)) return LD_OK;
+        phases = GEMM_CONTRACTION | GEMM_SECOND_PASS;
+    }
+    if (phases & GEMM_CONTRACTION) t_last_kernel = "";
     if (pl.status != LD_OK) return pl.status;
     if (pl.gn != (pin.gn_scale != nullptr) || (pl.gn && pin.gn_shift == nullptr)) return LD_ERR_ARG;
     GemmParams p = pin;
     if (p.stat_parts_out != nullptr) *p.stat_parts_out = pl.stat_parts;
     if (p.gn_part_done != nullptr) *p.gn_part_done = pl.gn_chunks;
+    if (p.gnf_applied != nullptr) *p.gnf_applied = pl.gn_applied ? 1 : 0;
     if (p.conv && p.pad < 0) p.pad = p.ksize >> 1;
     if (p.n_valid <= 0 || p.n_valid > p.N) p.n_valid = p.N;
     const dim3 grid(pl.grid_x, 1, pl.grid_z);
-    t_last_kernel = pl.kernel;
-    switch (pl.route) {
+    if (phases & GEMM_CONTRACTION) t_last_kernel = pl.kernel;
+    const int route = (phases & GEMM_CONTRACTION) ? pl.route : GR_NONE;
+    if (route == GR_NONE) p.splitk = pl.splitk;
+    switch (route) {
+        case GR_NONE: break;
         case GR_CONV8:
             if (const int st = conv8_launch(p, pl.c8_S, stream); st != LD_OK) return st;
             break;
@@ -2627,7 +2625,11 @@
             else launch_cfg<64, 128>(p, pl, grid, stream);
             break;
     }
-    if (pl.reduce == GRD_GROUPNORM) {
+    if (!(phases & GEMM_SECOND_PASS)) return hipGetLastError() == hipSuccess ? LD_OK : LD_ERR_HIP;
+    if (pl.reduce == GRD_GN_FINISH) {
+        p.gnf_cb = pl.gnf_cb; p.gnf_threads = pl.gnf_threads;
+        if (const int st = gn_splitk_finish_launch(p, stream); st != LD_OK) return st;
+    } else if (pl.reduce == GRD_GROUPNORM) {
         hipLaunchKernelGGL(splitk_reduce_gn_kernel, dim3(p.gn_P, p.M / p.gn_HW, 4), dim3(256), 0, stream, p);
     } else if (pl.reduce == GRD_PLAIN) {
         const int out_n = p.act == 2 ? p.N / 2 : p.N;
diff --git a/lightdiffusion_amd/csrc/norm.hip b/lightdiffusion_amd/csrc/norm.hip
--- a/lightdiffusion_amd/csrc/norm.hip
+++ b/lightdiffusion_amd/csrc/norm.hip
@@ -210,6 +210,155 @@
         const float sc = rstd[g] * (float)a.gamma[cg];
         scale[(long long)n * C + cg] = sc;
         shift[(long long)n * C + cg] = (float)a.beta[cg] - mean[g] * sc;
+    }
+}
+
+template <int MAXPIX>
+__global__ __launch_bounds__(1024) void gn_splitk_finish_kernel(const GemmParams p) {
+    extern __shared__ float gnf_smem[];
+    const int C = p.N, cpg = C / 32;
+    const int CS = C / 4, CHS = CS >> 3, rows_par = 256 / CHS;
+    const int CB = p.gnf_cb, CHB = CB >> 3, gpb = CB / cpg, P = p.gn_P;
+    float* csum = gnf_smem;
+    float* csq = csum + P * rows_par * CB;
+    float* part = csq + P * rows_par * CB;
+    float* mean = part + gpb * P * 2;
+    float* rstd = mean + gpb;
+    const int nblk = C / CB;
+    int bx = blockIdx.x;
+    if ((nblk & 7) == 0) bx = (bx & 7) * (nblk >> 3) + (bx >> 3);
+    const int n = blockIdx.y, tid = threadIdx.x;
+    const int cb0 = bx * CB;
+    const int ccb = tid % CHB, prow = (tid / CHB) % rows_par, pc = tid / (CHB * rows_par);
+    const bool owner = pc < P;
+    const int c0 = cb0 + ccb * 8;
+    const int p_begin = pc * p.gn_ppb, p_end = min(p.gn_HW, p_begin + p.gn_ppb);
+    const long long slab_stride = (long long)p.M * p.N;
+    uint4 held[MAXPIX];
+    if (owner) {
+        float s[8], ss[8];
+#pragma unroll
+        for (int j = 0; j < 8; ++j) s[j] = ss[j] = 0.f;
+#pragma unroll
+        for (int u = 0; u < MAXPIX; ++u) {
+            const int pix = p_begin + prow + u * rows_par;
+            held[u] = zero16();
+            if (pix < p_end) {
+                const int m = n * p.gn_HW + pix;
+                const float* base = p.partial + (long long)m * p.N + c0;
+                float v[8];
+#pragma unroll
+                for (int j = 0; j < 8; ++j) v[j] = 0.f;
+                int sp = 0;
+                for (; sp + 4 <= p.splitk; sp += 4) {
+                    f32x4 x0[4], x1[4];
+#pragma unroll
+                    for (int q = 0; q < 4; ++q) {
+                        x0[q] = *reinterpret_cast<const f32x4*>(base + (sp + q) * slab_stride);
+                        x1[q] = *reinterpret_cast<const f32x4*>(base + (sp + q) * slab_stride + 4);
+                    }
+#pragma unroll
+                    for (int q = 0; q < 4; ++q)
+#pragma unroll
+                        for (int j = 0; j < 4; ++j) {
+                            v[j] += x0[q][j];
+                            v[4 + j] += x1[q][j];
+                        }
+                }
+                for (; sp < p.splitk; ++sp) {
+                    const f32x4 x0 = *reinterpret_cast<const f32x4*>(base + sp * slab_stride), x1 = *reinterpret_cast<const f32x4*>(base + sp * slab_stride + 4);
+#pragma unroll
+                    for (int j = 0; j < 4; ++j) {
+                        v[j] += x0[j];
+                        v[4 + j] += x1[j];
+                    }
+                }
+                epilogue_store8(p, 0, m, c0, c0, v);
+                held[u] = pack8(v);
+                float f[8];
+                unpack8(held[u], f);
+#pragma unroll
+                for (int j = 0; j < 8; ++j) {
+                    s[j] += f[j];
+                    ss[j] += f[j] * f[j];
+                }
+            }
+        }
+#pragma unroll
+        for (int j = 0; j < 8; ++j) {
+            csum[(pc * rows_par + prow) * CB + ccb * 8 + j] = s[j];
+            csq[(pc * rows_par + prow) * CB + ccb * 8 + j] = ss[j];
+        }
+    }
+    __syncthreads();
+    {
+        const int team = tid >> 5, sub = tid & 31;
+        const int tpc = team / gpb, gl = team - tpc * gpb;
+        const int cnt = tpc < P ? rows_par * cpg : 0;
+        float a = 0.f, b = 0.f;
+        for (int i = sub; i < cnt; i += 32) {
+            const int pr = i / cpg, c = gl * cpg + (i - pr * cpg);
+            a += csum[(tpc * rows_par + pr) * CB + c];
+            b += csq[(tpc * rows_par + pr) * CB + c];
+        }
+#pragma unroll
+        for (int o = 1; o < 32; o <<= 1) {
+            a += __shfl_xor(a, o, 64);
+            b += __shfl_xor(b, o, 64);
+        }
+        if (sub == 0 && tpc < P) {
+            float* o = p.gn_part + (((long long)n * P + tpc) * 32 + cb0 / cpg + gl) * 2;
+            o[0] = a;
+            o[1] = b;
+            part[(gl * P + tpc) * 2] = a;
+            part[(gl * P + tpc) * 2 + 1] = b;
+        }
+    }
+    __syncthreads();
+    {
+        const int gl = tid >> 5, sub = tid & 31;
+        float s = 0.f, ss = 0.f;
+        if (gl < gpb && sub < P) {
+            s += part[(gl * P + sub) * 2];
+            ss += part[(gl * P + sub) * 2 + 1];
+        }
+#pragma unroll
+        for (int o = 1; o < 32; o <<= 1) {
+            s += __shfl_xor(s, o, 64);
+            ss += __shfl_xor(ss, o, 64);
+        }
+        if (sub == 0 && gl < gpb) {
+            const float cnt = (float)cpg * (float)p.gn_HW;
+            const float mu = s / cnt;
+            const float var = fmaxf(ss / cnt - mu * mu, 0.f);
+            mean[gl] = mu;
+            rstd[gl] = rsqrtf(var + p.gnf_eps);
+        }
+    }
+    __syncthreads();
+    if (!owner) return;
+    float ga[8], be[8], sc[8], sh[8];
+    unpack8(ld16(p.gnf_gamma + c0), ga);
+    unpack8(ld16(p.gnf_beta + c0), be);
+#pragma unroll
+    for (int j = 0; j < 8; ++j) {
+        const int g = (ccb * 8 + j) / cpg;
+        sc[j] = rstd[g] * ga[j];
+        sh[j] = be[j] - mean[g] * sc[j];
+    }
+#pragma unroll
+    for (int u = 0; u < MAXPIX; ++u) {
+        const int pix = p_begin + prow + u * rows_par;
+        if (pix < p_end) {
+            float v[8];
+            unpack8(held[u], v);
+#pragma unroll
+            for (int j = 0; j < 8; ++j) {
+                v[j] = v[j] * sc[j] + sh[j];
+                if (p.gnf_silu) v[j] = silu_f(v[j]);
+            }
+            st16(p.gnf_y + ((long long)n * p.gn_HW + pix) * C + c0, pack8(v));
+        }
     }
 }
 
@@ -355,6 +504,15 @@
     return hipGetLastError() == hipSuccess ? LD_OK : LD_ERR_HIP;
 }
 
+int gn_splitk_finish_launch(const GemmParams& p, hipStream_t stream) {
+    if (p.partial == nullptr || p.gn_part == nullptr || p.gnf_y == nullptr || p.gnf_gamma == nullptr || p.gnf_beta == nullptr || p.C == nullptr) return LD_ERR_ARG;
+    if (p.gnf_cb <= 0 || p.gnf_threads <= 0 || p.gnf_threads > 1024 || p.N % p.gnf_cb || p.gn_HW <= 0 || p.M % p.gn_HW || p.splitk < 2) return LD_ERR_SHAPE;
+    const int cpg = p.N / 32, rows_par = 256 / ((p.N / 4) >> 3);
+    hipLaunchKernelGGL(gn_splitk_finish_kernel<GN_FINISH_MAXPIX>, dim3(p.N / p.gnf_cb, p.M / p.gn_HW), dim3(p.gnf_threads),
+                       gn_finish_lds_bytes(p.gn_P, rows_par, p.gnf_cb, p.gnf_cb / cpg), stream, p);
+    return hipGetLastError() == hipSuccess ? LD_OK : LD_ERR_HIP;
+}
+
 int layernorm_launch(const half_t* x, const half_t* gamma, const half_t* beta, half_t* y, int rows, int C, float eps,
                      hipStream_t stream) {
     if (x == nullptr || y == nullptr || gamma == nullptr || beta == nullptr) return LD_ERR_ARG;
diff --git a/lightdiffusion_amd/csrc/runtime.h b/lightdiffusion_amd/csrc/runtime.h
--- a/lightdiffusion_amd/csrc/runtime.h
+++ b/lightdiffusion_amd/csrc/runtime.h
@@ -222,6 +222,20 @@
         if (dry || status != LD_OK) return;
         t_begin(p.conv && p.ksize == 3 ? KC_CONV3 : KC_GEMM, fl, 1, p.conv ? (p.ksize == 3 ? "conv3" : "conv1") : (p.act == 2 ? "geglu" : "gemm"),
                 p.M, p.N, p.K, p.batch);
+        if (timing != nullptr && p.gnf_y != nullptr) {
+            const GemmPlan own = plan != nullptr ? *plan : gemm_plan(p);
+            if (own.gn_applied) {
+                note(gemm_run(p, own, stream, GEMM_CONTRACTION));
+                t_end(gemm_last_kernel_name());
+                t_begin(KC_GNORM, 0.0, 1, "groupnorm", p.M / p.gn_HW, p.gn_HW, p.N, p.gnf_silu);
+                note(gemm_run(p, own, stream, GEMM_SECOND_PASS));
+                t_end("gn_splitk_finish_kernel");
+                return;
+            }
+            note(gemm_run(p, own, stream));
+            t_end(gemm_last_kernel_name());
+            return;
+        }
         note(plan != nullptr ? gemm_run(p, *plan, stream) : gemm_launch(p, stream));
         t_end(gemm_last_kernel_name());
     }
@@ -241,8 +255,17 @@
         t_end(ready != nullptr ? "gn_apply_kernel" : "gn_stats_kernel+gn_apply_kernel");
         arena->release(m);
     }
-    void gn_silu_conv(GemmParams p, int n_img, int HW, const half_t* gamma, const half_t* beta, float eps, half_t* g, float* ready = nullptr, int ready_P = 0) {
+    void gn_silu_conv(GemmParams p, int n_img, int HW, const half_t* gamma, const half_t* beta, float eps, half_t* g, float* ready = nullptr, int ready_P = 0,
+                      const half_t* applied = nullptr) {
         with_scratch(p);
+        if (applied != nullptr) {
+            p.A = applied;
+            p.A2 = nullptr;
+            p.C1 = p.C1 + p.C2;
+            p.C2 = 0;
+            gemm(p);
+            return;
+        }
         if (ready_P <= 0) ready = nullptr;
         const GemmPlan fused = gemm_plan(p, true);
         if (fused.can_fuse_groupnorm) {
diff --git a/lightdiffusion_amd/csrc/unet.hip b/lightdiffusion_amd/csrc/unet.hip
--- a/lightdiffusion_amd/csrc/unet.hip
+++ b/lightdiffusion_amd/csrc/unet.hip
@@ -32,6 +32,15 @@
     int C, H, W;
     float* gn = nullptr;
     int gnP = 0;
+    const half_t* normed = nullptr;
+    const half_t* normed_by = nullptr;
+};
+struct NormOffer {
+    const half_t* gamma = nullptr;
+    const half_t* beta = nullptr;
+    float eps = 0.f;
+    int silu = 0;
+    int conv_cout = 0;
 };
 
 }
@@ -282,6 +291,21 @@
         p.gn_part_done = done;
     }
 
+    static void offer_norm(GemmParams& p, const half_t* gamma, const half_t* beta, float eps, int silu, half_t* y, int* applied) {
+        p.gnf_gamma = gamma; p.gnf_beta = beta; p.gnf_eps = eps; p.gnf_silu = silu; p.gnf_y = y; p.gnf_applied = applied;
+    }
+    bool conv_fuses_groupnorm(int cin, int cout, int H, int W) const {
+        GemmParams p;
+        p.conv = 1; p.ksize = 3;
+        half_t* const any = reinterpret_cast<half_t*>(u);
+        p.A = any; p.W = any; p.C = any;
+        p.C1 = cin;
+        p.Hs = H; p.Ws = W; p.Hv = H; p.Wv = W; p.Ho = H; p.Wo = W; p.stride = 1;
+        p.ldw = 9 * cin; p.M = n * H * W; p.N = cout; p.K = 9 * cin; p.ldc = cout;
+        ex.with_scratch(p);
+        return gemm_plan(p, true).can_fuse_groupnorm;
+    }
+
     half_t* conv3(const half_t* x1, int C1, const half_t* x2, int C2, int Hs, int Ws, int Hv, int Wv, int stride, int wslot, int bslot,
                   int cout, const half_t* rowvec, int ldrv, const half_t* R, half_t* out, int* Ho_, int* Wo_, int ksize = 3, float* stats = nullptr,
                   int* stats_done = nullptr, const half_t* wup = nullptr) {
@@ -318,13 +342,17 @@
         ex.gemm(p);
     }
 
-    Feat resblock(const ResW& r, const half_t* x1, int C1, const half_t* x2, int C2, int H, int W, float* in_stats = nullptr, int in_P = 0) {
+    Feat resblock(const ResW& r, const half_t* x1, int C1, const half_t* x2, int C2, int H, int W, float* in_stats = nullptr, int in_P = 0,
+                  const half_t* in_normed = nullptr, const NormOffer* next = nullptr) {
         Arena& ar = *ex.arena;
         const size_t M = (size_t)na() * H * W;
         half_t* out = ar.halfs(M * r.cout);
+        if (pair_pending || H * W > 1024) next = nullptr;
+        half_t* out_n = next != nullptr ? ar.halfs(M * r.cout) : nullptr;
+        int out_n_done = 0;
         float* gno = reinterpret_cast<float*>(ar.alloc(groupnorm_workspace_bytes(na(), H * W)));
         int gno_done = 0;
-        if (C2 != 0) in_stats = nullptr;
+        if (C2 != 0) in_stats = nullptr, in_normed = nullptr;
         const size_t mk = ar.mark();
         auto conv_params = [&](const half_t* a1, int c1, const half_t* a2, int c2, int wslot, int bslot, const half_t* rowvec, int ldrv, const half_t* R,
                                half_t* dst) {
@@ -355,13 +383,15 @@
         }
         float* gnp = reinterpret_cast<float*>(ar.alloc(groupnorm_workspace_bytes(na(), H * W)));
         int gnp_done = 0;
+        half_t* g2 = g1;
+        if (r.cout > r.cin) g2 = ar.halfs(M * r.cout);
+        int g2_done = 0;
         {
             GemmParams c1 = conv_params(x1, C1, x2, C2, r.c1_w, r.c1_b, emb_all + r.emb_off, u->emb_total, nullptr, h1);
             want_stats(c1, gnp, H * W, &gnp_done);
-            ex.gn_silu_conv(c1, n, H * W, P(r.gn1_g), P(r.gn1_b), 1e-5f, g1, in_stats, in_P);
-        }
-        half_t* g2 = g1;
-        if (r.cout > r.cin) g2 = ar.halfs(M * r.cout);
+            if (H * W <= 1024 && !conv_fuses_groupnorm(r.cout, r.cout, H, W)) offer_norm(c1, P(r.gn2_g), P(r.gn2_b), 1e-5f, 1, g2, &g2_done);
+            ex.gn_silu_conv(c1, n, H * W, P(r.gn1_g), P(r.gn1_b), 1e-5f, g1, in_stats, in_P, in_normed);
+        }
         {
             GemmParams c2 = conv_params(h1, r.cout, nullptr, 0, r.c2_w, r.c2_b, nullptr, 0, skip, out);
             if (fold_skip) {
@@ -373,13 +403,15 @@
                 c2.W8 = nullptr;
             }
             want_stats(c2, gno, H * W, &gno_done);
-            ex.gn_silu_conv(c2, n, H * W, P(r.gn2_g), P(r.gn2_b), 1e-5f, g2, gnp_done ? gnp : nullptr, gnp_done);
+            if (next != nullptr && !(next->conv_cout > 0 && conv_fuses_groupnorm(r.cout, next->conv_cout, H, W)))
+                offer_norm(c2, next->gamma, next->beta, next->eps, next->silu, out_n, &out_n_done);
+            ex.gn_silu_conv(c2, n, H * W, P(r.gn2_g), P(r.gn2_b), 1e-5f, g2, gnp_done ? gnp : nullptr, gnp_done, g2_done ? g2 : nullptr);
         }
         ar.release(mk);
-        return {out, r.cout, H, W, gno_done ? gno : nullptr, gno_done};
-    }
-
-    Feat transformer(const StW& s, const half_t* x, int H, int W, float* in_stats = nullptr, int in_P = 0) {
+        return {out, r.cout, H, W, gno_done ? gno : nullptr, gno_done, out_n_done ? out_n : nullptr, out_n_done ? next->gamma : nullptr};
+    }
+
+    Feat transformer(const StW& s, const half_t* x, int H, int W, float* in_stats = nullptr, int in_P = 0, const half_t* in_normed = nullptr) {
         Arena& ar = *ex.arena;
         const int C = s.c, L = H * W, heads = u->cfg.num_heads, d = C / heads;
         int M = n * L;
@@ -389,7 +421,8 @@
         int gno_done = 0;
         const size_t mk = ar.mark();
         half_t* g = ar.halfs(Ma * C);
-        ex.groupnorm(x, C, nullptr, 0, n, L, P(s.gn_g), P(s.gn_b), 1e-6f, 0, g, in_stats, in_P);
+        if (in_normed != nullptr) g = const_cast<half_t*>(in_normed);
+        else ex.groupnorm(x, C, nullptr, 0, n, L, P(s.gn_g), P(s.gn_b), 1e-6f, 0, g, in_stats, in_P);
         half_t* t = ar.halfs(Ma * C);
         half_t* qkv = ar.halfs(Ma * 3 * C);
         half_t* ao = ar.halfs(Ma * C);
@@ -590,16 +623,32 @@
     R.linear(semb, ted, u->res[0].emb_w, u->res[0].emb_b, nullptr, emb_all, n, u->emb_total, ted);
     R.emb_all = emb_all;
 
-    auto run_layers = [&](const std::vector<Layer>& layers, Feat f, const half_t* x2, int C2, int outH, int outW) -> Feat {
-        for (const Layer& L : layers) {
+    auto run_layers = [&](const std::vector<Layer>& layers, Feat f, const half_t* x2, int C2, int outH, int outW, const Layer* after = nullptr) -> Feat {
+        for (size_t li = 0; li < layers.size(); ++li) {
+            const Layer& L = layers[li];
             switch (L.kind) {
                 case L_RES: {
-                    f = R.resblock(u->res[L.idx], f.p, f.C, x2, C2, f.H, f.W, f.gn, f.gnP);
+                    const Layer* cons = li + 1 < layers.size() ? &layers[li + 1] : after;
+                    NormOffer no;
+                    if (cons != nullptr && cons->kind == L_ST) {
+                        const StW& st = u->st[cons->idx];
+                        no.gamma = R.P(st.gn_g); no.beta = R.P(st.gn_b); no.eps = 1e-6f; no.silu = 0;
+                    } else if (cons != nullptr && cons->kind == L_RES) {
+                        const ResW& rn = u->res[cons->idx];
+                        no.gamma = R.P(rn.gn1_g); no.beta = R.P(rn.gn1_b); no.eps = 1e-5f; no.silu = 1; no.conv_cout = rn.cout;
+                    }
+                    const ResW& rw = u->res[L.idx];
+                    const half_t* in_n = (C2 == 0 && f.normed != nullptr && f.normed_by == R.P(rw.gn1_g)) ? f.normed : nullptr;
+                    f = R.resblock(rw, f.p, f.C, x2, C2, f.H, f.W, f.gn, f.gnP, in_n, no.gamma != nullptr ? &no : nullptr);
                     x2 = nullptr;
                     C2 = 0;
                     break;
                 }
-                case L_ST: f = R.transformer(u->st[L.idx], f.p, f.H, f.W, f.gn, f.gnP); break;
+                case L_ST: {
+                    const StW& sw = u->st[L.idx];
+                    f = R.transformer(sw, f.p, f.H, f.W, f.gn, f.gnP, (f.normed != nullptr && f.normed_by == R.P(sw.gn_g)) ? f.normed : nullptr);
+                    break;
+                }
                 case L_DOWN: {
                     const ConvW& cw = u->convs[L.idx];
                     const int Ho = (f.H - 1) / 2 + 1, Wo = (f.W - 1) / 2 + 1;
@@ -612,7 +661,7 @@
                     float* gno = reinterpret_cast<float*>(ar.alloc(groupnorm_workspace_bytes(n, Ho * Wo)));
                     int gno_done = 0;
                     R.conv3(f.p, f.C, nullptr, 0, f.H, f.W, f.H, f.W, 2, cw.w, cw.b, cw.cout, nullptr, 0, nullptr, o, nullptr, nullptr, 3, gno, &gno_done);
-                    f = {o, cw.cout, Ho, Wo, gno_done ? gno : nullptr, gno_done};
+                    f = Feat{o, cw.cout, Ho, Wo, gno_done ? gno : nullptr, gno_done};
                     break;
                 }
                 case L_UP: {
@@ -621,7 +670,7 @@
                     half_t* o = ar.halfs((size_t)n * Hv * Wv * cw.cout);
                     const half_t* wup = (u->fold_base != nullptr && cw.f_up >= 0) ? reinterpret_cast<const half_t*>(u->fold_base + cw.f_up) : nullptr;
                     R.conv3(f.p, f.C, nullptr, 0, f.H, f.W, Hv, Wv, 1, cw.w, cw.b, cw.cout, nullptr, 0, nullptr, o, nullptr, nullptr, 3, nullptr, nullptr, wup);
-                    f = {o, cw.cout, Hv, Wv};
+                    f = Feat{o, cw.cout, Hv, Wv};
                     break;
                 }
                 default: break;
@@ -649,13 +698,15 @@
         hs.push_back(f);
     }
     for (size_t b = 1; b < u->in_blocks.size(); ++b) {
-        f = run_layers(u->in_blocks[b], f, nullptr, 0, 0, 0);
+        const Layer* after = b + 1 < u->in_blocks.size() ? &u->in_blocks[b + 1][0] : (u->mid_block.empty() ? nullptr : &u->mid_block[0]);
+        f = run_layers(u->in_blocks[b], f, nullptr, 0, 0, 0, after);
         if (R.pair_pending && b == 1) {
             R.dup(const_cast<half_t*>(f.p), (size_t)R.n * f.H * f.W * f.C * sizeof(half_t));
             R.pair_pending = false;
             R.n = n;
             f.gn = nullptr;
             f.gnP = 0;
+            f.normed = f.normed_by = nullptr;
         }
         hs.push_back(f);
     }
diff --git a/lightdiffusion_amd/ops.py b/lightdiffusion_amd/ops.py
--- a/lightdiffusion_amd/ops.py
+++ b/lightdiffusion_amd/ops.py
@@ -152,6 +152,29 @@
     if chunks.value == 0:
         return y, None
     return y, part[: n * chunks.value * 64].view(n, chunks.value, 32, 2)
+
+
+def conv2d_gn_finish(x: torch.Tensor, w_packed: torch.Tensor, bias: Optional[torch.Tensor], gamma: torch.Tensor, beta: torch.Tensor, eps: float,
+                     silu: bool = False, ksize: int = 3, x2: Optional[torch.Tensor] = None, rowvec: Optional[torch.Tensor] = None,
+                     residual: Optional[torch.Tensor] = None, s1: Optional[torch.Tensor] = None, s2: Optional[torch.Tensor] = None,
+                     gn_x2: Optional[torch.Tensor] = None, offer: bool = True):
+    import ctypes
+    n, h, w, c1 = x.shape
+    c2 = 0 if x2 is None else x2.shape[-1]
+    sc1 = 0 if s1 is None else s1.shape[-1]
+    sc2 = 0 if s2 is None else s2.shape[-1]
+    gc2 = 0 if gn_x2 is None else gn_x2.shape[-1]
+    cout = w_packed.shape[0]
+    y = torch.empty(n, h, w, cout, dtype=torch.float16, device=x.device)
+    yn = torch.empty(n, h, w, cout + gc2, dtype=torch.float16, device=x.device)
+    part = torch.zeros(lib().ld_op_conv_gn_partials_floats(n, h * w), dtype=torch.float32, device=x.device)
+    chunks, applied = ctypes.c_int(0), ctypes.c_int(0)
+    ws = _ws(192 << 20, x.device)
+    check(lib().ld_op_conv_gn_finish(_p(x), c1, _p(x2), c2, n, h, w, ksize, _p(w_packed), _p(bias), _p(rowvec), _p(residual), _p(s1), sc1, _p(s2), sc2,
+                                     _p(gamma), _p(beta), eps, int(silu), _p(gn_x2), gc2, _p(y), _p(yn), cout, _p(part), ctypes.byref(chunks),
+                                     ctypes.byref(applied), int(offer), _p(ws), ws.numel(), _stream()), "ld_op_conv_gn_finish")
+    p = None if chunks.value == 0 else part[: n * chunks.value * 64].view(n, chunks.value, 32, 2)
+    return y, yn, p, bool(applied.value)
 
 
 def group_norm_silu_conv2d(x: torch.Tensor, gamma: torch.Tensor, beta: torch.Tensor, eps: float, w_packed: torch.Tensor,
```

Measured after the change: 61.67 steps/s (median of 3 runs). Within noise of the previous version (+0.4%).
